# fabian-sp/GGLasso

Measured on AMD Instinct MI355X. Metric: ADMM iters/sec on (K=32,p=500) GGL at 1/2/4/8 GPUs; eigh HBM GB/s vs peak, higher is better.
Workload: dtype f64

## Files before the change

### gglasso_amd/_lib.py

```python
import ctypes
import os

import numpy as np

_HERE = os.path.dirname(os.path.abspath(__file__))
LIB_PATH = os.path.join(_HERE, "lib", "libggl_hip.so")
DEV_LIB_PATH = os.path.join(_HERE, "lib", "libggl_hip_dev.so")

REG_SGL, REG_GGL, REG_FGL = 0, 1, 2
EIG_AUTO, EIG_JACOBI, EIG_ROCSOLVER, EIG_NEWTON_SCHULZ = 0, 1, 2, 3
CTX_STREAM_GIVEN = 1 << 16
OPTIONS = {"speculate": 1, "spec_factor": 2, "ns_mode": 3, "ns_degrees": 4, "theta_flat": 5, "rank_eig": 6, "parts": 7,
           "parts_max_tiles": 8, "symm_variant": 9, "spin_wait": 10, "fused_bounds": 11, "pipeline": 12, "fused_start": 13, "parts_small": 14, "ns_tol": 15, "cw_warm": 16, "chain": 17, "rank_l0_coarse": 18, "isolate": 19, "rank_deflate": 20, "rank_l0_deflate": 21, "fused_cw": 22, "omega_lds": 23, "early_part": 24, "part_priority": 25, "fused_w": 26, "rank_cw": 27, "bound_side": 28, "lds_pinned": 29, "join_flag": 30, "cw_rider": 31, "copy_rider": 32, "reduce_rider": 33, "parts_bias": 34, "parts_order": 35, "download_threads": 36, "group_sched": 37}


def eig_flags(method=EIG_AUTO, ns_mode=0, ns_degrees=0):
    return int(method) | ((int(ns_mode) & 0x3) << 8) | ((int(ns_degrees) & 0xf) << 12)

JACOBI_MAX_P = 128
NS_MIN_P = 8
BUF_S, BUF_OMEGA, BUF_THETA, BUF_L, BUF_X, BUF_GROUPSQ, BUF_NORMS, BUF_OMEGA_PREV = range(8)
E_ARG, E_HIP, E_SOLVER, E_ALLOC, E_COMM = -1, -2, -3, -4, -5
PHASES = ("form_W", "eig_omega", "recon_omega", "theta", "eig_L", "recon_L", "dual", "reduce", "eig_omega2", "bound",
          "allreduce_groupsq", "allreduce_norms")

_dp = ctypes.POINTER(ctypes.c_double)
_vp = ctypes.c_void_p
_i = ctypes.c_int
_d = ctypes.c_double
_ubp = ctypes.POINTER(ctypes.c_ubyte)
_ip = ctypes.POINTER(ctypes.c_int)

_SIGNATURES = {
    "ggl_version": ([], _i),
    "ggl_last_error": ([], ctypes.c_char_p),
    "ggl_device_count": ([], _i),
    "ggl_theta_limits": ([ctypes.POINTER(_i)], _i),
    "ggl_ctx_create": ([_i, _i, _i, _i, _vp, ctypes.POINTER(_vp)], _i),
    "ggl_ctx_destroy": ([_vp], _i),
    "ggl_ctx_sync": ([_vp], _i),
    "ggl_device_ptr": ([_vp, _i], _vp),
    "ggl_ctx_set_option": ([_vp, _i, _d], _i),
    "ggl_ctx_get_option": ([_vp, _i, _dp], _i),
    "ggl_set_S": ([_vp, _dp], _i),
    "ggl_set_state": ([_vp, _dp, _dp, _dp, _dp], _i),
    "ggl_set_state_ex": ([_vp, _dp, _dp, _dp, _dp, ctypes.POINTER(_i)], _i),
# ... 40 lines not shown
    "ggl_ext_batch_step": ([_vp, _d, _dp, _dp, _i, _dp, _dp], _i),
    "ggl_objective": ([_vp, _d, _d, _i, _dp], _i),
    "ggl_kkt_residual": ([_vp, _d, _d, _d, _i, _i, _dp, _dp, _dp], _i),
    "ggl_profile_enable": ([_vp, _i], _i),
    "ggl_profile_read": ([_vp, _dp, ctypes.POINTER(ctypes.c_longlong), _i], _i),
    "ggl_dev_symm": ([_i, _i, _dp, _dp, _dp, _dp, _dp, _dp, _i], _i),
    "ggl_dev_symm_bench": ([_i, _i, _i, _i, _dp], _i),
    "ggl_lds_stats": ([_vp, ctypes.POINTER(ctypes.c_longlong)], _i),
    "ggl_group_stats": ([_vp, ctypes.POINTER(ctypes.c_longlong), _dp], _i),
    "ggl_spectral_bounds": ([_vp, _dp, _dp], _i),
    "ggl_pipeline_stats": ([_vp, ctypes.POINTER(ctypes.c_longlong)], _i),
    "ggl_trace_start": ([_vp, _i], _i),
    "ggl_trace_read": ([_vp, _dp, _i], _i),
    "ggl_dev_omega_lds": ([_i, _i, _dp, _dp, _dp, _dp, _dp, _d, _i, _dp, _dp, _i, _dp], _i),
    "ggl_dev_symm_bounds": ([_i, _i, _dp, _dp, _i, _dp, _dp, _dp, _dp], _i),
    "ggl_snapshot_k": ([_vp, _i], _i),
    "ggl_snapshot_from": ([_vp, _i, _vp, _i], _i),
    "ggl_selection_stats": ([_vp, _dp], _i),
    "ggl_threshold_scan": ([_vp, _dp, _i, _dp, ctypes.POINTER(_i)], _i),
    "ggl_selection_rank": ([_vp, _d, _dp], _i),
    "ggl_finalize_L": ([_vp, _i, ctypes.POINTER(_i)], _i),
    "ggl_failed_instances": ([_vp, ctypes.POINTER(_i)], _i),
    "ggl_failed_reason": ([_vp, _i, _dp], _i),
    "ggl_debug_poison": ([_i], _i),
    "ggl_set_odd_dl": ([_i], _i),
    "ggl_reset_instance": ([_vp, _i], _i),
    "ggl_ctx_create_subset": ([_vp, ctypes.POINTER(_i), _i, ctypes.POINTER(_vp)], _i),
    "ggl_get_snapshot_k": ([_vp, _i, _dp, _dp], _i),
    "ggl_get_snapshot_state_k": ([_vp, _i, _dp, _dp], _i),
    "ggl_dev_ns_schedule": ([_d, _i, _i, ctypes.POINTER(_i), _dp, ctypes.POINTER(_i)], _i),
    "ggl_dev_ns_schedule_tol": ([_d, _i, _d, _i, ctypes.POINTER(_i), _dp, ctypes.POINTER(_i)], _i),
    "ggl_dev_group_partition": ([ctypes.POINTER(_i), _i, _i, _i, ctypes.POINTER(_i)], _i),
    "ggl_dev_ns_units": ([_d, _i, _d], _i),
    "ggl_ns_stats": ([_vp, ctypes.POINTER(ctypes.c_longlong)], _i),
    "ggl_rank_stats": ([_vp, ctypes.POINTER(ctypes.c_longlong)], _i),
    "ggl_deflate_stats": ([_vp, ctypes.POINTER(ctypes.c_longlong)], _i),
    "ggl_finalize_stats": ([_vp, ctypes.POINTER(ctypes.c_longlong)], _i),
    "ggl_eig_info": ([_vp, ctypes.POINTER(_i)], _i),
    "ggl_last_dispatch": ([_vp, ctypes.POINTER(ctypes.c_longlong)], _i),
    "ggl_eigh_batched": ([_i, _i, _dp, _dp, _dp, _i], _i),
    "ggl_phiplus": ([_i, _i, _dp, _dp, _dp, _dp], _i),
    "ggl_prox_rank_norm": ([_i, _i, _dp, _dp, _dp, _dp], _i),
    "ggl_phiplus_matrix": ([_i, _i, _dp, _dp, _dp, _i], _i),
    "ggl_rank_matrix": ([_i, _i, _dp, _dp, _dp, _i], _i),
    "ggl_rank_matrix_ex": ([_i, _i, _dp, _dp, _dp, _i, _d, ctypes.POINTER(ctypes.c_longlong)], _i),
    "ggl_rank_matrix_deflate": ([_i, _i, _dp, _dp, _dp, _i, _d, ctypes.POINTER(ctypes.c_longlong)], _i),
    "ggl_prox_od_1norm": ([_i, _dp, _d, _dp, _dp], _i),
    "ggl_prox_p": ([_i, _i, _dp, _d, _d, _i, _dp], _i),
    "ggl_prox_tv": ([_i, _i, _dp, _d, _dp], _i),
    "ggl_prox_2norm": ([_i, _i, _dp, _d, _dp], _i),
    "ggl_prox_phi": ([_i, _i, _dp, _d, _d, _i, _dp], _i),
}

_DEV_SIGNATURES = {
    "ggl_dev_i8_stages": ([_i], _i),
    "ggl_dev_symm_i8": ([_i, _i, _i, _i, _dp, _dp, _d, _d, _dp, _i, _dp], _i),
    "ggl_dev_omega_i8": ([_i, _i, _dp, _dp, _dp, ctypes.POINTER(_i), _d, _dp, _i, _dp], _i),
    "ggl_dev_mfma_f64_peak": ([_dp], _i),
    "ggl_dev_symm_timeline": ([_i, _i, ctypes.POINTER(ctypes.c_longlong), _i, ctypes.POINTER(_i)], _i),
    "ggl_dev_chain_probe": ([_i, _i, _i, _i, _i, _i, _dp], _i),
    "ggl_dev_coissue_probe": ([_dp], _i),
    "ggl_dev_mfma_lds_probe": ([_dp], _i),
    "ggl_dev_chain_run": ([_i, _i, _i, _i, _dp], _i),
    "ggl_dev_switch_bench": ([_i, _i, _i, _i, _i, _dp], _i),
    "ggl_dev_vendor_bench": ([_i, _i, _i, _i, _dp], _i),
    "ggl_dev_fill_copy_probe": ([_i, _i, _i, _i, _i, ctypes.POINTER(ctypes.c_longlong)], _i),
# ... 79 lines not shown
```

### gglasso_amd/csrc/capi_batch.hip

```cpp
#include "capi_internal.hpp"

static int sgl_fused_finish(ggl_ctx* c, const double* rho, const double* lambda1, double* out_norms);

extern "C" int ggl_sgl_batch_step(ggl_ctx* c, const double* rho, const double* lambda1, int latent, const double* mu1,
                                  double* out_norms)
{
    ARGCHK(c && rho && lambda1 && out_norms, "ctx, rho, lambda1, out_norms");
    ARGCHK(!latent || mu1, "latent needs mu1");
    HIPCHK(hipSetDevice(c->device));
    DROP_PRE(c);
    return sgl_batch_step_impl(c, rho, lambda1, latent, mu1, out_norms);
}

static int sgl_fused_finish(ggl_ctx* c, const double* rho, const double* lambda1, double* out_norms)
{
    const int K = c->K;
    c->sgl_done = false;
    c->sgl_fused_calls += 1;
    c->norms_host = true;
    double* rows = c->norms_h;
    {
        const unsigned long long want = c->seq_wait;
        const volatile unsigned long long* sq = c->seq_h;
        const auto t0 = std::chrono::steady_clock::now();
// ... 443 lines not shown
    HIPCHK(hipSetDevice(c->device));
    DROP_PRE(c);
    const size_t pp = (size_t)c->p * c->p, off = (size_t)k * pp;
    double* ident[] = {c->S + off, c->Om[0] + off, c->Om[1] + off, c->Theta + off};
    double* zero[] = {c->L + off, c->X + off, c->W + off};
    for (double* z : zero) HIPCHK(hipMemsetAsync(z, 0, pp * sizeof(double), c->stream));
    for (double* a : ident) launch_set_identity(c->stream, a, 1, c->p);
    for (double* lam : c->Lam)
        if (lam) launch_set_identity(c->stream, lam + off, 1, c->p);
    if (c->X1) HIPCHK(hipMemsetAsync(c->X1 + off, 0, pp * sizeof(double), c->stream));
    HIPCHK(hipGetLastError());
    c->spec_have = false;
    c->cw_have = false;
    c->cwL_have = false;
    return GGL_OK;
}

extern "C" int ggl_ctx_create_subset(ggl_ctx* src, const int* idx, int m, ggl_ctx** out)
{
    ARGCHK(src && idx && out, "ctx, idx, out");
    ARGCHK(m >= 1 && m <= src->K, "1 <= m <= K");
    for (int i = 0; i < m; ++i) ARGCHK(idx[i] >= 0 && idx[i] < src->K, "instance index");
    HIPCHK(hipSetDevice(src->device));
    { int rc_ = drop_prelaunch(src); if (rc_) return rc_; }
    ggl_ctx* c = nullptr;
    int rc = ggl_ctx_create(src->device, m, src->p, src->flags & ~GGL_CTX_STREAM_GIVEN, nullptr, &c);
    if (rc) return rc;
    c->spec_enable = src->spec_enable; c->spec_factor = src->spec_factor; c->ns_force = src->ns_force;
    c->ns_degrees = src->ns_degrees; c->theta_flat = src->theta_flat; c->rank_eig = src->rank_eig;
    c->rank_ns = c->omega_ns && !c->rank_eig; c->ns_parts = src->ns_parts; c->parts_max_tiles = src->parts_max_tiles;
    c->symm_variant = src->symm_variant; c->spin_wait = src->spin_wait; c->fused_bounds = src->fused_bounds;
    c->pipeline = src->pipeline; c->fused_start = src->fused_start; c->parts_small = src->parts_small; c->download_threads = src->download_threads; c->ns_tol = src->ns_tol;
    c->cw_warm = src->cw_warm; c->rank_l0 = src->rank_l0; c->rank_l0_coarse = src->rank_l0_coarse;
    c->group_sched = src->group_sched;
    c->isolate = src->isolate; c->lds_omega = src->lds_omega; c->lds_waves = src->lds_waves; c->early_part = src->early_part; c->rank_deflate = src->rank_deflate; c->rank_l0_deflate = src->rank_l0_deflate;
    int* didx = nullptr;
    hipError_t e = hipMalloc(&didx, m * sizeof(int));
    if (e == hipSuccess) e = hipMemcpyAsync(didx, idx, m * sizeof(int), hipMemcpyHostToDevice, src->stream);
    if (e != hipSuccess) { ggl_ctx_destroy(c); return fail(GGL_E_HIP, "subset: %s", hipGetErrorString(e)); }
    const size_t pp = (size_t)src->p * src->p;
    const double* from[] = {src->S, src->Om[src->cur], src->Om[src->cur ^ 1], src->Theta, src->L, src->X};
    double* to[] = {c->S, c->Om[0], c->Om[1], c->Theta, c->L, c->X};
    for (int i = 0; i < 6; ++i) launch_copy_instances(src->stream, to[i], from[i], didx, m, pp, false);
    c->cur = 0;
    c->state_symmetric = src->state_symmetric;
    c->S_symmetric = src->S_symmetric;
    c->fused_w = src->fused_w;
#ifdef GGL_DEV
    c->parts_bias = src->parts_bias; c->parts_order = src->parts_order; c->chain_mode = src->chain_mode; c->fused_cw = src->fused_cw;
    c->rank_cw = src->rank_cw; c->bound_side = src->bound_side;
#endif
    c->lds_pinned = src->lds_pinned;
    c->join_flag = src->join_flag;
    c->cw_rider = src->cw_rider;
    c->copy_rider = src->copy_rider;
    c->red_rider = src->red_rider;
    c->step_latent = src->step_latent;
    c->nk_valid = false;
    if (src->l_ns && src->Ckeep && src->Ckeep_beta) {
        e = hipMalloc(&c->Ckeep_alloc, c->n * sizeof(double) + STACK_SLACK);
        if (e != hipSuccess) { (void)hipFree(didx); ggl_ctx_destroy(c); return fail(GGL_E_HIP, "subset: %s", hipGetErrorString(e)); }
        c->Ckeep = c->Ckeep_alloc;
        c->Ckeep_beta = (double*)malloc(m * sizeof(double));
        for (int i = 0; i < m; ++i) c->Ckeep_beta[i] = src->Ckeep_beta[idx[i]];
        launch_copy_instances(src->stream, c->Ckeep, src->Ckeep, didx, m, pp, false);
        c->l_ns = true;
    }
// ... 27 lines not shown
```

### gglasso_amd/csrc/capi_ctx.hip

```cpp
#include "capi_internal.hpp"

static thread_local char g_err[512] = "";

int fail(int code, const char* fmt, ...)
{
    va_list ap;
    va_start(ap, fmt);
    vsnprintf(g_err, sizeof(g_err), fmt, ap);
    va_end(ap);
    return code;
}

void prof_collect(ggl_ctx* c)
{
    if (!c->prof_on) return;
    for (int ph = 0; ph < GGL_NPHASE; ++ph) {
        if (!c->ev_used[ph]) continue;
        float ms = 0.f;
        if (hipEventElapsedTime(&ms, c->ev[ph][0], c->ev[ph][1]) == hipSuccess) {
            c->ph_ms[ph] += ms;
            c->ph_cnt[ph] += 1;
        }
        c->ev_used[ph] = false;
    }
// ... 294 lines not shown
{
    int rcd = drop_prelaunch(c);
    if (rcd) return rcd;
    switch (opt) {
        case GGL_OPT_SPECULATE: c->spec_enable = v != 0.0; break;
        case GGL_OPT_SPEC_FACTOR:
            if (!(v > 0.0)) return fail(GGL_E_ARG, "bad argument: GGL_OPT_SPEC_FACTOR must be positive");
            c->spec_factor = v;
            break;
        case GGL_OPT_NS_MODE:
            if (v != 0.0 && v != 1.0 && v != 2.0) return fail(GGL_E_ARG, "bad argument: GGL_OPT_NS_MODE is 0, 1 or 2");
            c->ns_force = (int)v;
            break;
        case GGL_OPT_NS_DEGREES: c->ns_degrees = v >= 9 ? 9 : (v >= 5 ? 5 : 3); break;
        case GGL_OPT_THETA_FLAT: c->theta_flat = (v == 2.0) ? 2 : (v != 0.0 ? 1 : 0); break;
        case GGL_OPT_RANK_EIG: c->rank_eig = v != 0.0; c->rank_ns = c->omega_ns && !c->rank_eig; break;
        case GGL_OPT_PARTS: c->ns_parts = std::min(std::max((int)v, 1), (int)ggl_ctx::MAX_PARTS); break;
        case GGL_OPT_PARTS_MAX_TILES: c->parts_max_tiles = (long)v; break;
        case GGL_OPT_SYMM_VARIANT:
            if (v >= 0 && !symm_variant_built((int)v))
                return fail(GGL_E_ARG, "bad argument: product-kernel variant not in this build");
            c->symm_variant = (int)v;
            break;
        case GGL_OPT_SPIN_WAIT: c->spin_wait = v != 0.0; break;
        case GGL_OPT_FUSED_BOUNDS: c->fused_bounds = v != 0.0; break;
        case GGL_OPT_PIPELINE: c->pipeline = v != 0.0; break;
        case GGL_OPT_FUSED_START: c->fused_start = v != 0.0; break;
        case GGL_OPT_PARTS_SMALL: c->parts_small = (int)v; break;
        case GGL_OPT_GROUP_SCHED:
            if (v != 0.0 && v != 1.0 && v != 2.0 && v != 3.0 && v != 12.0 && v != 13.0)
                return fail(GGL_E_ARG, "bad argument: GGL_OPT_GROUP_SCHED is 0, 1, 2, 3, 12 or 13");
            c->group_sched = (int)v;
            break;
#ifdef GGL_DEV
        case GGL_OPT_PARTS_BIAS: c->parts_bias = (int)v; break;
        case GGL_OPT_PARTS_ORDER: c->parts_order = (int)v; break;
        case GGL_OPT_CHAIN: c->chain_mode = (v == 2.0) ? 2 : (v != 0.0 ? 1 : 0); break;
        case GGL_OPT_FUSED_CW: c->fused_cw = v != 0.0; break;
        case GGL_OPT_RANK_CW: c->rank_cw = v != 0.0; break;
        case GGL_OPT_BOUND_SIDE: c->bound_side = (int)v; break;
#else
        case GGL_OPT_PARTS_BIAS: case GGL_OPT_PARTS_ORDER: case GGL_OPT_CHAIN: case GGL_OPT_FUSED_CW: case GGL_OPT_RANK_CW:
        case GGL_OPT_BOUND_SIDE: case GGL_OPT_PART_PRIORITY:
            if (v == 0.0) break;
            return fail(GGL_E_ARG, "bad argument: option %d is a measured-and-rejected alternative that only the development "
                        "library (libggl_hip_dev.so, python -m gglasso_amd.build --dev) carries", opt);
#endif
        case GGL_OPT_DOWNLOAD_THREADS: c->download_threads = std::min(std::max((int)v, 1), 64); break;
        case GGL_OPT_CW_WARM: c->cw_warm = v != 0.0; break;
        case GGL_OPT_ISOLATE: c->isolate = v != 0.0; break;
        case GGL_OPT_OMEGA_LDS: c->lds_omega = v != 0.0; c->lds_waves = (v == 4.0 || v == 8.0) ? (int)v : 0; break;
        case GGL_OPT_EARLY_PART: c->early_part = v != 0.0; break;
        case GGL_OPT_FUSED_W: c->fused_w = v != 0.0; break;
        case GGL_OPT_LDS_PINNED: c->lds_pinned = v != 0.0; break;
        case GGL_OPT_JOIN_FLAG: c->join_flag = v != 0.0; break;
        case GGL_OPT_CW_RIDER: c->cw_rider = (int)v; break;
        case GGL_OPT_COPY_RIDER: c->copy_rider = (int)v; break;
        case GGL_OPT_REDUCE_RIDER: c->red_rider = (int)v; break;
#ifdef GGL_DEV
        case GGL_OPT_PART_PRIORITY: {
            if (v != 0.0 && v != 1.0 && v != 2.0) return fail(GGL_E_ARG, "bad argument: GGL_OPT_PART_PRIORITY is 0, 1 or 2");
            if (!c->omega_ns || (int)v == c->part_priority) break;
            int lo = 0, hi = 0;
            HIPCHK(hipSetDevice(c->device));
            HIPCHK(hipDeviceGetStreamPriorityRange(&lo, &hi));
            HIPCHK(hipStreamSynchronize(c->stream));
// ... 25 lines not shown
        default: return fail(GGL_E_ARG, "bad argument: unknown ctx option %d", opt);
    }
    c->spec_have = false;
    c->cw_have = false;
    c->cwL_have = false;
    return GGL_OK;
}

extern "C" int ggl_ctx_set_option(ggl_ctx* c, int opt, double value)
{
    ARGCHK(c, "ctx");
    return set_option(c, opt, value);
}

extern "C" int ggl_ctx_get_option(ggl_ctx* c, int opt, double* value)
{
    ARGCHK(c && value, "ctx, value");
    switch (opt) {
        case GGL_OPT_SPECULATE: *value = c->spec_enable; break;
        case GGL_OPT_SPEC_FACTOR: *value = c->spec_factor; break;
        case GGL_OPT_NS_MODE: *value = c->ns_force; break;
        case GGL_OPT_NS_DEGREES: *value = c->ns_degrees; break;
        case GGL_OPT_THETA_FLAT: *value = c->theta_flat; break;
        case GGL_OPT_RANK_EIG: *value = c->rank_eig; break;
        case GGL_OPT_PARTS: *value = c->ns_parts; break;
        case GGL_OPT_PARTS_MAX_TILES: *value = (double)c->parts_max_tiles; break;
        case GGL_OPT_SYMM_VARIANT: *value = c->symm_variant; break;
        case GGL_OPT_SPIN_WAIT: *value = c->spin_wait; break;
        case GGL_OPT_FUSED_BOUNDS: *value = c->fused_bounds; break;
        case GGL_OPT_PIPELINE: *value = c->pipeline; break;
        case GGL_OPT_FUSED_START: *value = c->fused_start; break;
        case GGL_OPT_PARTS_SMALL: *value = c->parts_small; break;
        case GGL_OPT_GROUP_SCHED: *value = c->group_sched; break;
        case GGL_OPT_PARTS_BIAS: *value = c->parts_bias; break;
        case GGL_OPT_PARTS_ORDER: *value = c->parts_order; break;
        case GGL_OPT_DOWNLOAD_THREADS: *value = c->download_threads; break;
        case GGL_OPT_NS_TOL: *value = c->ns_tol; break;
        case GGL_OPT_CW_WARM: *value = c->cw_warm; break;
        case GGL_OPT_CHAIN: *value = c->chain_mode; break;
        case GGL_OPT_RANK_L0_COARSE: *value = c->rank_l0_coarse; break;
        case GGL_OPT_ISOLATE: *value = c->isolate; break;
        case GGL_OPT_FUSED_CW: *value = c->fused_cw; break;
        case GGL_OPT_OMEGA_LDS: *value = c->lds_omega ? (c->lds_waves ? c->lds_waves : 1) : 0; break;
        case GGL_OPT_EARLY_PART: *value = c->early_part; break;
        case GGL_OPT_FUSED_W: *value = c->fused_w; break;
        case GGL_OPT_RANK_CW: *value = c->rank_cw; break;
        case GGL_OPT_BOUND_SIDE: *value = c->bound_side; break;
        case GGL_OPT_LDS_PINNED: *value = c->lds_pinned; break;
        case GGL_OPT_JOIN_FLAG: *value = c->join_flag; break;
        case GGL_OPT_CW_RIDER: *value = c->cw_rider; break;
        case GGL_OPT_COPY_RIDER: *value = c->copy_rider; break;
        case GGL_OPT_REDUCE_RIDER: *value = c->red_rider; break;
        case GGL_OPT_PART_PRIORITY: *value = c->part_priority; break;
        case GGL_OPT_RANK_DEFLATE: *value = c->rank_deflate; break;
        case GGL_OPT_RANK_L0_DEFLATE: *value = c->rank_l0_deflate; break;
        default: return fail(GGL_E_ARG, "bad argument: unknown ctx option %d", opt);
    }
    return GGL_OK;
}

#ifdef GGL_DEV
static void dev_env_options(ggl_ctx* c)
{
    static const struct { const char* name; int opt; } tab[] = {
        {"GGL_SPECULATE", GGL_OPT_SPECULATE}, {"GGL_SPEC_FACTOR", GGL_OPT_SPEC_FACTOR}, {"GGL_NS_MODE", GGL_OPT_NS_MODE},
        {"GGL_NS_DEGREES", GGL_OPT_NS_DEGREES}, {"GGL_THETA_FLAT", GGL_OPT_THETA_FLAT}, {"GGL_RANK_EIG", GGL_OPT_RANK_EIG},
// ... 339 lines not shown
```

### gglasso_amd/csrc/capi_internal.hpp

```cpp
#pragma once
#include <hip/hip_runtime.h>
#include <rocblas/rocblas.h>
#include <rocsolver/rocsolver.h>

#include <algorithm>
#include <cmath>
#include <cstdarg>
#include <cstdio>
#include <cstring>
#include <numeric>
#include <atomic>
#include <thread>
#include <mutex>
#include <chrono>
#include <vector>

#include "../../include/ggl_hip.h"
#include "kernels.hpp"
#include "ggl_comm.hpp"

using namespace ggl;


#define HIPCHK(expr)                                                                                   \
// ... 74 lines not shown
    bool flags_dirty = false;
    int step_latent = 0;
    int ns_force = 0;
    bool use_syevj = false;
    static constexpr int MAX_PARTS = 4;
    hipStream_t streamx[MAX_PARTS - 1] = {};
    hipEvent_t ev_fork = nullptr, ev_join[MAX_PARTS - 1] = {};
    GGL_DEV_OPT(int, bound_side);
    bool join_flag = true;
    int red_rider = 2;
    long long red_rides = 0;
    RedRider red_pending;
    int copy_rider = 1;
    long long copy_rides = 0;
    std::vector<double> pre0_beta;
    int cw_rider = 1;
    long long cw_rides = 0;
    bool parts_serial = false;
    unsigned long long* join_words = nullptr;
    unsigned long long join_seq = 0;
    hipEvent_t ev_bfork[MAX_PARTS] = {}, ev_bjoin[MAX_PARTS] = {};
    bool pipeline = true, pre_valid = false, pre_spec_pending = false;
    bool last_step_hint = false;
    double* pre_beta = nullptr;
    long long pre_launched = 0, pre_dropped = 0;
    int download_threads = 8;
    GGL_DEV_OPT(int, parts_order);
    GGL_DEV_OPT(int, parts_bias);
    int group_sched = 1;
    long long group_steps = 0;
    long long group_changes = 0;
    int last_groups = 1, last_group_len[MAX_PARTS] = {}, last_group_units[MAX_PARTS] = {};
    double group_units_sum[MAX_PARTS] = {};
    int parts_small = 8;
    bool fused_start = true;
    bool fused_bounds = true;
    bool lds_omega = true;
    int lds_waves = 0;
    double* lds_tab = nullptr;
    int lds_ntab = 0, lds_tab_deg = -1;
    double lds_lnq = 0.0, lds_tab_tol = -1.0;
    long long lds_calls = 0, lds_misses = 0;
    int lds_cool = 0, lds_cool_next = 4;
    bool lds_last = false;
    GGL_DEV_OPT(bool, fused_cw);
    int theta_flat = 2;
    bool state_symmetric = true;
    bool S_symmetric = false;
    bool fused_w = true, wf_ready = false;
    double* wf_beta = nullptr;
    long long wf_written = 0, wf_used = 0;
    bool spec_enable = true, spec_have = false, spec_pending = false;
    double *spec_c = nullptr, *spec_beta = nullptr;
    double *cuse = nullptr, *cuse_h = nullptr;
    double *coef_hh[2] = {nullptr, nullptr}, *cuse_hh[2] = {nullptr, nullptr};
    int plan_par = 0;
    struct EarlyA {
        bool valid = false;
        NsPlan plans[4];
        double* fused[4] = {nullptr, nullptr, nullptr, nullptr};
        double* beta = nullptr;
        int nh = 0, Kh[4] = {}, k0h[4] = {};
        bool grouped = false;
        int var_parts = -1;
    } early;
    bool early_part = true;
// ... 169 lines not shown
```

### gglasso_amd/csrc/capi_omega.hip

```cpp
#include "capi_internal.hpp"

int eig_recon(ggl_ctx* c, double* A, double* out, double* Dv, int map, const double* betaK, int ph_eig,
                     int ph_recon)
{
    c->info_dirty = true;
    if (use_jacobi(c)) {
        if (ph_eig >= 0) PB(c, ph_eig);
        HIPCHK(launch_jacobi(c->stream, A, Dv, nullptr, out, map, betaK, c->info, c->K, c->p));
        if (ph_eig >= 0) PE(c, ph_eig);
        return GGL_OK;
    }
    if (ph_eig >= 0) PB(c, ph_eig);
    {
        int rcb = blas_handle(c, &c->blas);
        if (rcb) return rcb;
    }
    if (c->use_syevj) {
        rocblas_status sj = rocsolver_dsyevj_strided_batched(c->blas, rocblas_esort_none, rocblas_evect_original,
                                                             rocblas_fill_upper, c->p, A, c->p,
                                                             (rocblas_stride)c->p * c->p, 0.0, c->E, 100,
                                                             (rocblas_int*)c->sweeps, Dv, c->p, c->info, c->K);
        if (sj != rocblas_status_success) return fail(GGL_E_SOLVER, "rocsolver_dsyevj_strided_batched: status %d", (int)sj);
        if (ph_eig >= 0) PE(c, ph_eig);
        if (ph_recon >= 0) PB(c, ph_recon);
// ... 175 lines not shown
{
    c->lds_misses += 1;
    c->lds_cool = c->lds_cool_next;
    c->lds_cool_next = std::min(2 * c->lds_cool_next, 64);
    c->lds_last = false;
}

int trace_lane(const ggl_ctx* c, hipStream_t st)
{
    if (st == c->stream) return 0;
    for (int i = 0; i < ggl_ctx::MAX_PARTS - 1; ++i)
        if (st == c->streamx[i]) return i + 1;
    return -1;
}
void trace_mark(ggl_ctx* c, hipStream_t st, int tag)
{
    ggl_ctx::Trace& t = c->trace;
    if (!t.on || t.n >= t.cap) return;
    if (hipEventRecord(t.ev[t.n], st) != hipSuccess) return;
    t.tag[t.n] = tag;
    t.lane[t.n] = trace_lane(c, st);
    t.n += 1;
}
void trace_host(ggl_ctx* c, int tag)
{
    ggl_ctx::Trace& t = c->trace;
    if (!t.on || t.nhost >= t.cap) return;
    t.host_us[t.nhost] = std::chrono::duration<double, std::micro>(std::chrono::steady_clock::now() - t.t0).count();
    t.host_tag[t.nhost] = tag;
    t.nhost += 1;
}
void trace_symm_hook(hipStream_t st, int kind, void* arg) { trace_mark((ggl_ctx*)arg, st, 10 + kind); }

static int omega_groups(const ggl_ctx* c, const double* cb, const double* beta_h, int K, int* Kh, int* k0h, int* gunits)
{
    if (!c->group_sched || K < 2 || c->ns_force == 2 || c->chain_mode || c->comm) return 1;
    {
        const double I = 2.5e-14 * (double)c->p * c->p * c->p, F = 6.5e-6;
        if (c->group_sched < 10 && (double)K * 1e-7 > 0.01 * 7.0 * (F + K * I)) return 1;
    }
    std::vector<int> u(K);
    for (int k = 0; k < K; ++k) {
        double ck = cb[k] * (1.0 + 1e-10);
        if (!(ck > 0.0) || !std::isfinite(ck) || !(beta_h[k] > 0.0)) return 1;
        if (ck < 4.0 * beta_h[k]) ck = 4.0 * beta_h[k];
        u[k] = ns_units_query(std::sqrt(4.0 * beta_h[k] / ck), c->ns_degrees, c->ns_tol);
        if (u[k] < 0) return 1;
    }
    int len[ggl_ctx::MAX_PARTS];
    const bool force = c->group_sched >= 10;
    const int gmax = force ? c->group_sched - 10 : (c->group_sched >= 2 ? c->group_sched : 3);
    const int G = ns_group_partition(u.data(), K, force ? 20000 : c->p, std::min(gmax, (int)ggl_ctx::MAX_PARTS - 1), len);
    if (G <= 1) return 1;
    for (int g = 0, k0 = 0; g < G; ++g) {
        Kh[g] = len[g];
        k0h[g] = k0;
        gunits[g] = 0;
        for (int k = k0; k < k0 + len[g]; ++k) gunits[g] = std::max(gunits[g], u[k]);
        k0 += len[g];
    }
    return G;
}

static void note_groups(ggl_ctx* c, int G, const int* Kh, const NsPlan* plans)
{
    const int G_prev = c->last_groups;
// ... 10 lines not shown
    }
}

int omega_step(ggl_ctx* c, int latent, CopySegs* pending, bool allow_spec, bool only_spec)
{
    int rc;
    const double* beta = c->par;
    const int nxt = c->cur ^ 1;
    c->step_latent = latent;
    if (latent && !c->pre0_beta.empty()) std::fill(c->pre0_beta.begin(), c->pre0_beta.end(), std::nan(""));
    CopySegs first;
    if (pending) first = *pending;
    else if (c->par0_stale) first.add(c->par, c->par_h, 8 * (size_t)c->K * sizeof(double));
    c->par0_stale = false;
    if (c->omega_ns) {
        const int K = c->K;
        const bool want_A = c->early_request;
        c->early_request = false;
        bool w_ready = c->wf_ready && want_A && !latent;
        for (int k = 0; w_ready && k < K; ++k) w_ready = (c->par_h[k] == c->wf_beta[k]);
        c->wf_ready = false;
        bool resume = c->early.valid && allow_spec && !latent && !want_A && c->spec_enable;
        for (int k = 0; resume && k < K; ++k) resume = (c->par_h[k] == c->early.beta[k]);
        c->early.valid = false;
        if (!resume) {
            c->plan_par ^= 1;
            c->coef_h = c->coef_hh[c->plan_par];
            c->cuse_h = c->cuse_hh[c->plan_par];
        }
        double* pre = c->coef_h + (size_t)(NS_MAX_LAUNCHES - 2) * NS_SLOT(K);
        for (int k = 0; !resume && k < K; ++k) {
            double* o0 = pre + (size_t)k * NS_NCOEF;
            double* o1 = pre + NS_SLOT(K) + (size_t)k * NS_NCOEF;
            o0[0] = 4.0 * c->par_h[k]; o0[1] = 1.0; o0[2] = o0[3] = o0[4] = o0[5] = 0.0;
            o1[0] = 0.0; o1[1] = 1.0; o1[2] = o1[3] = o1[4] = o1[5] = 0.0;
        }
        double* pre_d = c->coef + (size_t)(NS_MAX_LAUNCHES - 2) * NS_SLOT(K);
        const long t64 = (c->p + 63) / 64;
        const long ntile = t64 * (t64 + 1) / 2 * K;
        int nh = (K >= 16 && ntile >= 600 && ntile <= c->parts_max_tiles) ? std::min(c->ns_parts, K / 8) : 1;
        if (nh == 1 && c->parts_small && K >= c->parts_small && K < 16 && c->p >= 384 && c->ns_parts >= 2) nh = 2;
        nh = std::max(nh, 1);
        bool spec = allow_spec && c->spec_enable && c->spec_have && !latent && c->spec_cool == 0;
        if (allow_spec && !only_spec && c->spec_cool > 0) c->spec_cool -= 1;
        for (int k = 0; spec && k < K; ++k) spec = (c->par_h[k] == c->spec_beta[k]);
        if (resume) spec = true;
        int Kh[ggl_ctx::MAX_PARTS], k0h[ggl_ctx::MAX_PARTS];
        bool grouped = false;
        int gunits[ggl_ctx::MAX_PARTS] = {};
        if (resume) {
            nh = c->early.nh;
            grouped = c->early.grouped;
            for (int h = 0; h < nh; ++h) { Kh[h] = c->early.Kh[h]; k0h[h] = c->early.k0h[h]; }
        } else {
            for (int h = 0, k0 = 0; h < nh; ++h) {
                Kh[h] = K / nh + (h < K % nh ? 1 : 0);
                if (nh == 2 && c->parts_bias && std::abs(c->parts_bias) < K / 2) Kh[h] += h == 0 ? c->parts_bias : -c->parts_bias;
                k0h[h] = k0;
                k0 += Kh[h];
            }
            if (spec && nh == 1) {
                std::vector<double> cb(K);
                for (int k = 0; k < K; ++k) cb[k] = c->spec_c[k] * c->spec_factor;
                const int G = omega_groups(c, cb.data(), c->par_h, K, Kh, k0h, gunits);
                if (G > 1) { nh = G; grouped = true; }
            }
        }
        const size_t pp = (size_t)c->p * c->p;
// ... 66 lines not shown
                if (as_spec) {
                    c->spec_pending = !fused;
                    c->cw_pending = false;
                    c->dvo_valid = false;
                    c->cur = nxt;
                    return GGL_OK;
                }
                HIPCHK(hipStreamSynchronize(c->stream));
                if (c->spec_flag_h[0] == 0) {
                    sanitize_bounds(c, c->bounds_h, c->par_h, 4.0);
                    for (int k = 0; k < K; ++k) { c->spec_c[k] = c->bounds_h[k]; c->spec_beta[k] = c->par_h[k]; }
                    c->spec_have = true;
                    c->lds_cool_next = 4;
                    c->dvo_valid = false;
                    c->cur = nxt;
                    return GGL_OK;
                }
                c->par0_stale = false;
                lds_missed(c);
                HIPCHK(hipMemsetAsync(c->spec_flag, 0, ggl_ctx::MAX_PARTS * sizeof(int), c->stream));
                for (int h = 0; h < ggl_ctx::MAX_PARTS; ++h) c->spec_flag_h[h] = 0;
            }
        }
#ifdef GGL_DEV
        if (spec && !want_A && !resume && c->chain_mode && c->fused_start && c->fused_bounds && (c->symm_variant < 0 || c->symm_variant == 17) &&
            chain_tile(K, c->p, c->chain_mode == 2) == 64) {
            if (!c->nsNX) HIPCHK(malloc_filled(&c->nsNX, 2 * c->n * sizeof(double) + STACK_SLACK, c->stream));
            if (!c->chain_cnt) HIPCHK(hipMalloc(&c->chain_cnt, (size_t)K * CHAIN_CNT_STRIDE * sizeof(unsigned)));
            for (int k = 0; k < K; ++k) c->cuse_h[k] = c->spec_c[k] * c->spec_factor;
            NsPlan& pl = plans[0];
            SymmOp ops[CHAIN_MAX_OPS];
            int nops = 0;
            const int bT = (c->p + 63) / 64;
            if (ns_plan(c->cuse_h, c->par_h, K, c->coef_h, start_base_h, &pl, c->ns_force, c->ns_degrees, c->ns_tol) == 0 &&
                !pl.stable) {
                double* f0 = nullptr;
                for (int k = 0; k < K; ++k)
                    f0 = ns_fused_start(pl, start_base_h + 5 * (size_t)k, c->nsYP[1], c->nsT, (size_t)K * pp,
                                        pre + NS_SLOT(K) + (size_t)k * NS_NCOEF + 3);
                if (f0)
                    nops = ns_chain_ops(pl, pre_d, pre_d + NS_SLOT(K), c->coef, c->W, c->nsYP[0], c->nsYP[1], c->nsNX, c->nsT,
                                        c->Om[nxt], K, c->p, 0, f0, c->rowpart, c->fropart, ops, CHAIN_MAX_OPS);
            }
            if (nops > 0) {
                CopySegs sg = first;
                sg.add(pre_d, pre, (size_t)K * NS_NCOEF * sizeof(double));
                sg.add(pre_d + NS_SLOT(K), pre + NS_SLOT(K), (size_t)K * NS_NCOEF * sizeof(double));
                sg.add(c->spec_flag, nullptr, 2 * sizeof(int));
                sg.add(c->spec_flag + ggl_ctx::MAX_PARTS - 1, nullptr, sizeof(int));
                c->spec_flag_h[0] = c->spec_flag_h[1] = c->spec_flag_h[ggl_ctx::MAX_PARTS - 1] = 0;
                const int nb_launch = pl.products - 2;
                if (nb_launch > 0) sg.add(c->coef, c->coef_h, (size_t)nb_launch * NS_SLOT(K) * sizeof(double));
                sg.add(c->cuse, c->cuse_h, (size_t)K * sizeof(double));
                if (c->info_dirty) sg.add(c->info, nullptr, K * sizeof(int));
                sg.add(c->chain_cnt, nullptr, (size_t)K * CHAIN_CNT_STRIDE * sizeof(unsigned));
                launch_copy_small(c->stream, sg);
                PB(c, GGL_PH_FORM_W);
                launch_form_W_sym(c->stream, c->W, c->Theta, nullptr, c->X, c->S, beta, K, c->p);
                PE(c, GGL_PH_FORM_W);
                PB(c, GGL_PH_EIG_OMEGA);
                ChainProg P;
                P.nops = nops; P.K = K; P.p = c->p; P.ntiles = bT * (bT + 1) / 2;
                P.begin[0] = 0;
                for (int i = 0; i < nops; ++i) { P.op[i] = ops[i]; P.begin[i + 1] = P.begin[i] + P.ntiles * (ops[i].pair ? 2 : 1); }
                if (launch_omega_chain(c->stream, P, c->chain_cnt, c->spec_flag + 1, c->spec_flag_h + 1) < 0)
                    return fail(GGL_E_HIP, "k_omega_chain: launch failed (%s)", hipGetErrorString(hipGetLastError()));
                launch_bound_rows(c->stream, c->rowpart, bT, K, c->p, c->nbrow, c->infpart);
                launch_cw_final(c->stream, c->nsYP[0] + c->n, c->nbrow, K, c->p, c->infpart, c->fropart, bT * (bT + 1) / 2,
                                c->cwmax, c->cwcnt, c->bounds_h, c->cuse, c->spec_flag, c->spec_flag_h, 0,
                                (c->cw_warm && c->cw_have) ? c->cwvec[c->cw_cur] : nullptr,
                                c->cw_warm ? c->cwvec[c->cw_cur ^ 1] : nullptr);
                PE(c, GGL_PH_EIG_OMEGA);
                HIPCHK(hipGetLastError());
                c->last_parts = 1;
                c->last_variant = 40;
                c->chain_calls += 1;
                c->ns_launches_total += pl.products;
                c->ns_units_frac += pl.units;
                c->ns_steps_frac += pl.steps;
                c->ns_units_total = (long long)(c->ns_units_frac + 0.5);
                c->ns_steps_total = (long long)(c->ns_steps_frac + 0.5);
                c->ns_calls += 1;
                c->spec_calls += 1;
                c->spec_pending = true;
                c->cw_pending = c->cw_warm;
                if (c->info_dirty) { memset(c->info_h, 0, K * sizeof(int)); c->info_dirty = false; }
                c->dvo_valid = false;
                c->cur = nxt;
                return GGL_OK;
            }
        }
#endif
        if (resume) {
            for (int h = 0; h < nh; ++h) { plans[h] = c->early.plans[h]; fused[h] = c->early.fused[h]; }
            c->early_used += 1;
        } else if (spec) {
            for (int k = 0; k < K; ++k) c->cuse_h[k] = c->spec_c[k] * c->spec_factor;
            sanitize_bounds(c, c->cuse_h, c->par_h, 4.0);
            for (int h = 0; spec && h < nh; ++h) {
                const int k0 = k0h[h];
                const int prc = ns_plan(c->cuse_h + k0, c->par_h + k0, Kh[h], c->coef_h + h * region,
                                        start_base_h + 5 * k0, &plans[h], c->ns_force, c->ns_degrees, c->ns_tol);
                spec = (prc == 0) && !plans[h].stable;
                for (int k = k0; spec && c->fused_start && k < k0 + Kh[h]; ++k) {
                    fused[h] = ns_fused_start(plans[h], start_base_h + 5 * (size_t)k, c->nsYP[1] + k0 * pp, c->nsT + k0 * pp,
                                              nh > 1 ? c->n : (size_t)K * pp, pre + NS_SLOT(K) + (size_t)k * NS_NCOEF + 3);
                }
            }
        }
        if (only_spec && !spec) return GGL_NOT_LAUNCHED;
        if (nh > 1 && !c->parts_probed) {
            rc = probe_part_streams(c);
            if (rc) return rc;
        }
        if (nh > 1 && !resume) {
            HIPCHK(hipEventRecord(c->ev_fork, c->stream));
            for (int h = 1; h < nh; ++h) HIPCHK(hipStreamWaitEvent(c->streamx[h - 1], c->ev_fork, 0));
        }
        for (int hh = 0; hh < nh; ++hh) {
            const int h = (c->parts_order && nh == 2 && c->prof_on == 0) ? nh - 1 - hh : hh;
            hipStream_t sh = h == 0 ? c->stream : c->streamx[h - 1];
            const int k0 = k0h[h];
            if (!want_A) {
                c->spec_flag_h[h] = 0;
                if (h == 0 && nh < ggl_ctx::MAX_PARTS) c->spec_flag_h[ggl_ctx::MAX_PARTS - 1] = 0;
            }
            double* Ap = c->nsYP[0] + k0 * pp;
            double* Bp = c->nsYP[0] + c->n + k0 * pp;
            const int btile = c->fused_bounds ? symm_bounds_tile(Kh[h], c->p, var_parts) : 0;
            const int bT = btile ? (c->p + btile - 1) / btile : 0;
            double* rowp = btile ? c->rowpart + (size_t)k0 * bT * c->p : nullptr;
            double* frop = btile ? c->fropart + (size_t)k0 * (bT * (bT + 1) / 2) : nullptr;
            if (!resume) {
            bool ride_copy = (c->copy_rider == 2 || (c->copy_rider == 1 && nh == 1)) && first.n == 0 && !latent && btile != 0 &&
                             !c->chain_mode && c->prof_on != 1;
            for (int k = k0; ride_copy && k < k0 + Kh[h]; ++k) ride_copy = (c->pre0_beta[k] == c->par_h[k]);
            CopySegs sg = first;
            if (!ride_copy) {
                sg.add(pre_d + NS_NCOEF * (size_t)k0, pre + NS_NCOEF * (size_t)k0, (size_t)Kh[h] * NS_NCOEF * sizeof(double));
// ... 11 lines not shown
                sg.add(c->cuse + k0, c->cuse_h + k0, (size_t)Kh[h] * sizeof(double));
                if (h == 0 && c->info_dirty) sg.add(c->info, nullptr, K * sizeof(int));
            }
            if (h == 0 && c->red_pending.nblk > 0) {
                if (w_ready && (c->red_rider == 2 || nh == 1)) {
                    symm_set_reduce_rider(c->red_pending);
                    c->red_rides += 1;
                } else {
                    launch_reduce_partials(sh, c->red_pending.partials, 1, c->red_pending.nblk, c->red_pending.nv, c->red_pending.out,
                                           c->red_pending.seq, c->red_pending.seq_val);
                    trace_mark(c, sh, 21);
                }
                c->red_pending = RedRider{};
            }
            if (ride_copy) {
                symm_set_copy_rider(sg);
                c->copy_rides += 1;
            } else {
                launch_copy_small(sh, sg);
                trace_mark(c, sh, 1);
            }
            if (h == 0) PB(c, GGL_PH_FORM_W);
            if (!w_ready) {
                launch_form_W_sym(sh, c->W + k0 * pp, c->Theta + k0 * pp, latent ? c->L + k0 * pp : nullptr, c->X + k0 * pp,
                                  c->S + k0 * pp, beta + k0, Kh[h], c->p);
                trace_mark(c, sh, 2);
            } else if (h == 0) c->wf_used += 1;
            const bool early_ev = want_A && h == 0 && c->prof_on == 2;
            if (early_ev) {
                c->ev_early_par ^= 1;
                (void)hipEventRecord(c->ev_early[c->ev_early_par][0], c->stream);
            } else if (h == 0 && !want_A) { PE(c, GGL_PH_FORM_W); PB(c, GGL_PH_EIG_OMEGA); }
            ns_prepare(sh, pre_d + NS_NCOEF * (size_t)k0, pre_d + NS_SLOT(K) + NS_NCOEF * (size_t)k0, c->W + k0 * pp, Ap, Bp, Kh[h], c->p,
                       var_parts, spec ? fused[h] : nullptr, rowp, frop);
            symm_flush_rider(sh);
            if (early_ev) {
                (void)hipEventRecord(c->ev_early[c->ev_early_par][1], c->stream);
                c->ev_early_used[c->ev_early_par] = true;
            }
            }
            if (want_A) continue;
            if (resume && h == 0) PB(c, GGL_PH_EIG_OMEGA);
            hipStream_t sb = sh;
            hipEvent_t bfree = nullptr;
            const int side_slot = nh + h - 1;
            const bool side_on = c->bound_side == 1 || (c->bound_side == 2 && nh > 1 && K >= 16);
            if (side_on && spec && btile && !c->fused_cw && side_slot < ggl_ctx::MAX_PARTS - 1 && c->streamx[side_slot]) {
                if (!c->ev_bfork[h]) {
                    HIPCHK(hipEventCreateWithFlags(&c->ev_bfork[h], hipEventDisableTiming));
                    HIPCHK(hipEventCreateWithFlags(&c->ev_bjoin[h], hipEventDisableTiming));
                }
                sb = c->streamx[side_slot];
                HIPCHK(hipEventRecord(c->ev_bfork[h], sh));
                HIPCHK(hipStreamWaitEvent(sb, c->ev_bfork[h], 0));
                bfree = c->ev_bjoin[h];
            }
            const bool ride = c->cw_rider && spec && btile && !c->fused_cw && sb == sh && c->cw_warm && c->cw_have;
            if (ride) {
                CwRider r;
                r.B = Bp; r.rowpart = rowp; r.fropart = frop;
                r.dprev = c->cwvec[c->cw_cur] + (size_t)k0 * c->p;
                r.dnext = c->cwvec[c->cw_cur ^ 1] + (size_t)k0 * c->p;
                r.d_out = c->nbrow + (size_t)k0 * c->p;
                r.cwmax = c->cwmax + k0; r.cnt = c->cwcnt + k0; r.out = c->bounds_h + k0; r.cuse = c->cuse + k0;
                r.flag = c->spec_flag; r.flag_host = c->spec_flag_h; r.flag_slot = h;
                r.T = bT; r.ntile = bT * (bT + 1) / 2; r.p = c->p; r.K = Kh[h]; r.nbx = (c->p + 15) / 16;
                symm_set_rider(r);
// ... 4 lines not shown
                if (c->fused_cw) {
                    launch_bound_cw(sh, Bp, rowp, bT, Kh[h], c->p, c->nbrow + (size_t)k0 * c->p, frop, bT * (bT + 1) / 2,
                                    c->cwmax + k0, c->cwcnt + k0, c->bounds_h + k0, spec ? c->cuse + k0 : nullptr,
                                    spec ? c->spec_flag : nullptr, spec ? c->spec_flag_h : nullptr, h,
                                    (c->cw_warm && c->cw_have) ? c->cwvec[c->cw_cur] + (size_t)k0 * c->p : nullptr,
                                    c->cw_warm ? c->cwvec[c->cw_cur ^ 1] + (size_t)k0 * c->p : nullptr);
                } else {
                const int nib = bound_rows_blocks(c->p);
                launch_bound_rows(sb, rowp, bT, Kh[h], c->p, c->nbrow + (size_t)k0 * c->p, c->infpart + (size_t)k0 * nib);
                trace_mark(c, sb, 3);
                launch_cw_final(sb, Bp, c->nbrow + (size_t)k0 * c->p, Kh[h], c->p, c->infpart + (size_t)k0 * nib, frop,
                                bT * (bT + 1) / 2, c->cwmax + k0, c->cwcnt + k0, c->bounds_h + k0, spec ? c->cuse + k0 : nullptr,
                                spec ? c->spec_flag : nullptr, spec ? c->spec_flag_h : nullptr, h,
                                (c->cw_warm && c->cw_have) ? c->cwvec[c->cw_cur] + (size_t)k0 * c->p : nullptr,
                                c->cw_warm ? c->cwvec[c->cw_cur ^ 1] + (size_t)k0 * c->p : nullptr);
                trace_mark(c, sb, 4);
                }
                cw_written = c->cw_warm;
            } else {
                double* nb2 = c->nbpart + 2 * (size_t)k0 * nbb;
                double* nbc = c->nbpart + 2 * (size_t)K * nbb + (size_t)k0 * nbb;
                launch_norm_bounds(sh, Bp, Kh[h], c->p, nb2, c->nbrow + (size_t)k0 * c->p);
                launch_cw_bounds(sh, Bp, c->nbrow + (size_t)k0 * c->p, Kh[h], c->p, nbc);
                launch_bound_final(sh, nb2, nbc, nbb, Kh[h], c->bounds_h + k0, 0, spec ? c->cuse + k0 : nullptr,
                                   spec ? c->spec_flag + h : nullptr, spec ? c->spec_flag_h + h : nullptr);
            }
            if (bfree) HIPCHK(hipEventRecord(bfree, sb));
            if (spec) {
                ns_run(sh, plans[h], c->coef + h * region, start_base_d + 5 * k0, c->W + k0 * pp, c->nsYP[0] + k0 * pp,
                       c->nsYP[1] + k0 * pp, c->nsT + k0 * pp, c->Om[nxt] + k0 * pp, Kh[h], c->p,
                       var_parts, nh > 1 ? c->n : 0, fused[h] != nullptr, bfree);
                symm_flush_rider(sh);
                c->ns_launches_total += plans[h].products;
                const double frac = (double)Kh[h] / K;
                c->ns_units_frac += frac * plans[h].units;
                c->ns_steps_frac += frac * plans[h].steps;
            }
            if (h == 0 && !spec) PE(c, GGL_PH_EIG_OMEGA);
        }
        HIPCHK(hipGetLastError());
        if (want_A) {
            for (int h = 0; h < nh; ++h) { c->early.plans[h] = plans[h]; c->early.fused[h] = fused[h]; c->early.Kh[h] = Kh[h]; c->early.k0h[h] = k0h[h]; }
            c->early.nh = nh;
            c->early.grouped = grouped;
            c->early.var_parts = var_parts;
            memcpy(c->early.beta, c->par_h, K * sizeof(double));
            c->early.valid = true;
            c->early_launched += 1;
            return GGL_OK;
        }
        if (spec) {
            if (nh > 1 && c->join_flag && !c->parts_serial) {
                c->join_seq += 1;
                for (int h = 1; h < nh; ++h) launch_set_flag(c->streamx[h - 1], c->join_words + h, c->join_seq);
                launch_wait_flags(c->stream, c->join_words + 1, nh - 1, c->join_seq, c->spec_flag, c->spec_flag_h, 0, 200.0);
                HIPCHK(hipGetLastError());
            } else {
                for (int h = 1; h < nh; ++h) {
                    HIPCHK(hipEventRecord(c->ev_join[h - 1], c->streamx[h - 1]));
                    HIPCHK(hipStreamWaitEvent(c->stream, c->ev_join[h - 1], 0));
                }
            }
            PE(c, GGL_PH_EIG_OMEGA);
            c->ns_units_total = (long long)(c->ns_units_frac + 0.5);
            c->ns_steps_total = (long long)(c->ns_steps_frac + 0.5);
            c->ns_calls += 1;
            c->spec_calls += 1;
            note_groups(c, grouped ? nh : 1, Kh, plans);
            c->spec_pending = true;
            c->cw_pending = cw_written;
            if (c->info_dirty) { memset(c->info_h, 0, K * sizeof(int)); c->info_dirty = false; }
            c->dvo_valid = false;
            c->cur = nxt;
            return GGL_OK;
        }
        for (int h = 0; h < nh; ++h) HIPCHK(hipStreamSynchronize(h == 0 ? c->stream : c->streamx[h - 1]));
        sanitize_bounds(c, c->bounds_h, c->par_h, 4.0);
        for (int k = 0; k < K; ++k) { c->spec_c[k] = c->bounds_h[k]; c->spec_beta[k] = c->par_h[k]; }
        c->spec_have = true;
        if (cw_written) { c->cw_cur ^= 1; c->cw_have = true; }
        bool any_stable = false;
        size_t region_b = region;
        int var_b = var_parts;
        if (nh == 1) {
            const int G = omega_groups(c, c->bounds_h, c->par_h, K, Kh, k0h, gunits);
            if (G > 1) {
                nh = G;
                grouped = true;
                region_b = (size_t)(NS_MAX_LAUNCHES - 4) / nh * NS_SLOT(K);
                var_b = var_grouped;
                if (!c->parts_probed) {
                    rc = probe_part_streams(c);
                    if (rc) return rc;
                }
            }
        }
        for (int h = 0; h < nh; ++h) {
            const int k0 = k0h[h];
            const int prc = ns_plan(c->bounds_h + k0, c->par_h + k0, Kh[h], c->coef_h + h * region_b, start_base_h + 5 * k0,
                                    &plans[h], c->ns_force, c->ns_degrees, c->ns_tol);
            if (prc == -1) return fail(GGL_E_SOLVER, "Newton-Schulz Omega-step: non-finite W (diverged iterate?)");
            if (prc == -2) {
                c->ns_eigh_fallbacks += 1;
                rc = eig_recon(c, c->W, c->Om[nxt], c->DvO, MAP_PHIPLUS, beta, -1, GGL_PH_RECON_OMEGA);
                if (rc) return rc;
                c->dvo_valid = true;
                c->cur = nxt;
                return GGL_OK;
            }
            any_stable = any_stable || plans[h].stable;
        }
        if (nh > 1 && any_stable) {
            const int prc = ns_plan(c->bounds_h, c->par_h, K, c->coef_h, start_base_h, &plans[0], c->ns_force, c->ns_degrees, c->ns_tol);
            if (prc != 0) return fail(GGL_E_SOLVER, "Newton-Schulz Omega-step: plan failed (%d)", prc);
        }
        const int nrun = (nh > 1 && !any_stable) ? nh : 1;
        if (nrun == 1) { Kh[0] = K; k0h[0] = 0; }
        c->last_parts = nrun;
        c->last_variant = symm_effective_variant((nrun > 1 && var_b >= 0) ? var_b
                          : (c->symm_variant >= 0 ? c->symm_variant : symm_auto_variant(Kh[0], c->p)), c->p);
        note_groups(c, (grouped && nrun > 1) ? nrun : 1, Kh, plans);
        PB(c, GGL_PH_EIG_OMEGA2);
        for (int h = 0; h < nrun; ++h) {
            const int Kr = Kh[h], k0 = k0h[h];
            hipStream_t sh = h == 0 ? c->stream : c->streamx[h - 1];
            CopySegs up;
            up.add(start_base_d + 5 * (size_t)k0, start_base_h + 5 * (size_t)k0, (size_t)Kr * 5 * sizeof(double));
            const int nb_launch = plans[h].products - 2;
            if (nb_launch > 0)
                up.add(c->coef + h * region_b, c->coef_h + h * region_b, (size_t)nb_launch * NS_SLOT(Kr) * sizeof(double));
            if (h == 0 && c->info_dirty) up.add(c->info, nullptr, K * sizeof(int));
            launch_copy_small(sh, up);
            ns_run(sh, plans[h], c->coef + h * region_b, start_base_d + 5 * k0,
                   c->W + k0 * pp, c->nsYP[0] + k0 * pp, c->nsYP[1] + k0 * pp, c->nsT + k0 * pp, c->Om[nxt] + k0 * pp, Kr,
                   c->p,
                   nrun > 1 ? var_b : c->symm_variant, nrun > 1 ? c->n : 0);
            c->ns_stable_calls += plans[h].stable ? 1 : 0;
            c->ns_launches_total += plans[h].products;
            const double frac = (double)Kr / K;
            c->ns_units_frac += frac * plans[h].units;
            c->ns_steps_frac += frac * plans[h].steps;
        }
        for (int h = 1; h < nrun; ++h) {
            HIPCHK(hipEventRecord(c->ev_join[h - 1], c->streamx[h - 1]));
            HIPCHK(hipStreamWaitEvent(c->stream, c->ev_join[h - 1], 0));
        }
        PE(c, GGL_PH_EIG_OMEGA2);
        HIPCHK(hipGetLastError());
        c->ns_units_total = (long long)(c->ns_units_frac + 0.5);
        c->ns_steps_total = (long long)(c->ns_steps_frac + 0.5);
        c->ns_calls += 1;
        c->dvo_valid = false;
        if (c->info_dirty) { memset(c->info_h, 0, K * sizeof(int)); c->info_dirty = false; }
        c->cur = nxt;
        return GGL_OK;
    }
    if (only_spec) return GGL_NOT_LAUNCHED;
    launch_copy_small(c->stream, first);
    PB(c, GGL_PH_FORM_W);
    launch_form_W(c->stream, c->W, c->Theta, latent ? c->L : nullptr, c->X, c->S, beta, c->K, c->p);
    PE(c, GGL_PH_FORM_W);
    HIPCHK(hipGetLastError());
    rc = eig_recon(c, c->W, c->Om[nxt], c->DvO, MAP_PHIPLUS, beta, GGL_PH_EIG_OMEGA, GGL_PH_RECON_OMEGA);
    if (rc) return rc;
    c->dvo_valid = true;
    c->cur = nxt;
    return GGL_OK;
}

extern "C" int ggl_step_group_partial(ggl_ctx* c, double rho, double lambda1)
{
// ... 336 lines not shown
```

### gglasso_amd/csrc/capi_ops.hip

```cpp
#include "capi_internal.hpp"

static int eig_common(int K, int p, const double* A, const double* beta, double* D, double* Q, double* out, int map,
                      int eig_method)
{
    ARGCHK(K >= 1 && p >= 1 && A, "K, p, A");
    ARGCHK(eig_method != GGL_EIG_JACOBI || jacobi_fits(p), "GGL_EIG_JACOBI needs p <= GGL_JACOBI_MAX_P");
    const bool jac = (eig_method == GGL_EIG_JACOBI) || (eig_method == GGL_EIG_AUTO && jacobi_fits(p));
    const size_t n = (size_t)K * p * p, kp = (size_t)K * p;
    DevBuf dA, dD, dR, dO, dB, dE, dS;
    int* dinfo = nullptr;
    HIPCHK(dA.alloc(n));
    HIPCHK(dD.alloc(kp));
    HIPCHK(dB.alloc(K));
    HIPCHK(hipMalloc(&dinfo, K * sizeof(int)));
    struct InfoFree { int* p; ~InfoFree() { (void)hipFree(p); } } infofree{dinfo};
    UP(dA.p, A, n);
    if (beta) UP(dB.p, beta, K);
    if (out) HIPCHK(dO.alloc(n));
    std::vector<int> info(K);
    if (jac) {
        if (Q) HIPCHK(dR.alloc(n));
        HIPCHK(launch_jacobi(nullptr, dA.p, dD.p, dR.p, dO.p, map, beta ? dB.p : nullptr, dinfo, K, p));
        HIPCHK(hipDeviceSynchronize());
        HIPCHK(hipMemcpy(info.data(), dinfo, K * sizeof(int), hipMemcpyDeviceToHost));
// ... 686 lines not shown
    HIPCHK(dC.alloc(n));
    HIPCHK(dcoef.alloc(coef.size()));
    HIPCHK(dT.alloc((size_t)nb * 5));
    UP(dA.p, h.data(), n);
    UP(dB.p, h.data(), n);
    UP(dcoef.p, coef.data(), coef.size());
    HIPCHK(hipMemset(dT.p, 0, (size_t)nb * 5 * sizeof(double)));
    for (int i = 0; i < 3; ++i) launch_symm(nullptr, dA.p, dB.p, dC.p, nullptr, nullptr, dcoef.p, K, p, 0);
    launch_symm(nullptr, dA.p, dB.p, dC.p, nullptr, nullptr, dcoef.p, K, p, 10, dT.p);
    HIPCHK(hipGetLastError());
    HIPCHK(hipDeviceSynchronize());
    HIPCHK(hipMemcpy(out, dT.p, (size_t)nb * 5 * sizeof(long long), hipMemcpyDeviceToHost));
    *nblocks_out = nb;
    return GGL_OK;
}

#endif

extern "C" int ggl_dev_ns_schedule(double l, int degrees, int max_steps, int* deg_out, double* coef_out, int* units_out)
{
    ARGCHK(deg_out && coef_out && units_out, "output pointers");
    ARGCHK(l > 0.0 && l <= 1.0, "l must be in (0,1]");
    const int n = ns_schedule_query(l, degrees, max_steps, deg_out, coef_out, units_out);
    if (n < 0) return fail(GGL_E_ARG, "no schedule within %d steps", max_steps);
    return n;
}

extern "C" int ggl_dev_group_partition(const int* units, int K, int p, int max_groups, int* len_out)
{
    ARGCHK(units && len_out && K >= 1 && p >= 1 && max_groups >= 1 && max_groups <= 3, "units, len_out, K, p, 1 <= max_groups <= 3");
    return ns_group_partition(units, K, p, max_groups, len_out);
}
extern "C" int ggl_dev_ns_units(double l, int degrees, double tol) { return ns_units_query(l, degrees, tol); }

extern "C" int ggl_dev_ns_schedule_tol(double l, int degrees, double tol, int max_steps, int* deg_out, double* coef_out,
                                       int* units_out)
{
    ARGCHK(deg_out && coef_out && units_out, "output pointers");
    ARGCHK(l > 0.0 && l <= 1.0, "l must be in (0,1]");
    ARGCHK(tol >= 0.0 && tol <= 1e-6, "tol in [0, 1e-6]");
    const int n = ns_schedule_query(l, degrees, max_steps, deg_out, coef_out, units_out, std::max(tol, NS_TOL_EXACT));
    if (n < 0) return fail(GGL_E_ARG, "no schedule within %d steps", max_steps);
    return n;
}

#ifdef GGL_DEV
extern "C" int ggl_dev_coissue_probe(double* out12)
{
    ARGCHK(out12, "out");
    DevBuf d;
    HIPCHK(d.alloc((size_t)512 * 512));
    coissue_probe(nullptr, d.p, out12);
    HIPCHK(hipGetLastError());
    return GGL_OK;
}

extern "C" int ggl_dev_mfma_lds_probe(double* out6)
{
    ARGCHK(out6, "out");
    DevBuf d;
    HIPCHK(d.alloc((size_t)2048 * 256));
    mfma_lds_probe(nullptr, d.p, out6);
    HIPCHK(hipGetLastError());
    return GGL_OK;
}

// ... 221 lines not shown
```

### gglasso_amd/csrc/capi_stats.hip

```cpp
#include "capi_internal.hpp"

extern "C" int ggl_scale_X(ggl_ctx* c, double factor)
{
    ARGCHK(c, "ctx");
    HIPCHK(hipSetDevice(c->device));
    DROP_PRE(c);
    launch_scale(c->stream, c->X, factor, c->n);
    HIPCHK(hipGetLastError());
    return GGL_OK;
}

extern "C" int ggl_profile_enable(ggl_ctx* c, int on)
{
    ARGCHK(c, "ctx");
    HIPCHK(hipSetDevice(c->device));
    if (on && !c->ev[0][0]) {
        for (int ph = 0; ph < GGL_NPHASE; ++ph)
            for (int e = 0; e < 2; ++e) HIPCHK(hipEventCreate(&c->ev[ph][e]));
        for (int q = 0; q < 2; ++q)
            for (int e = 0; e < 2; ++e) HIPCHK(hipEventCreate(&c->ev_early[q][e]));
    }
    c->prof_on = (on == 2) ? 2 : (on != 0 ? 1 : 0);
    return GGL_OK;
}

extern "C" int ggl_ns_stats(ggl_ctx* c, long long out[16])
{
    ARGCHK(c && out, "ctx, out");
    long long lds[4] = {0, 0, 0, 0};
    if (c->lds_calls) { int rc_ = ggl_lds_stats(c, lds); if (rc_) return rc_; }
    out[0] = c->ns_calls;
    out[1] = c->ns_steps_total + (lds[3] + c->K / 2) / c->K;
    out[2] = c->ns_stable_calls;
    out[3] = c->ns_units_total + (lds[2] + c->K / 2) / c->K;
    out[4] = c->ns_launches_total;
    out[5] = c->rank_calls;
    out[6] = c->rank_retries;
    out[7] = c->rank_fallbacks;
    out[8] = c->rank_launches;
    out[9] = c->spec_calls;
    out[10] = c->spec_misses;
    out[11] = c->spin_timeouts;
    out[12] = c->last_parts;
    out[13] = c->last_variant;
    out[14] = c->ns_eigh_fallbacks;
    out[15] = c->pre_dropped;
    return GGL_OK;
}

extern "C" int ggl_group_stats(ggl_ctx* c, long long out[11], double* units_sum)
{
    ARGCHK(c && out, "ctx, out");
    out[10] = c->group_changes;
    out[0] = c->group_steps;
    out[1] = c->last_groups;
    for (int g = 0; g < 4; ++g) {
        out[2 + g] = c->last_groups > 1 ? c->last_group_len[g] : 0;
        out[6 + g] = c->last_groups > 1 ? c->last_group_units[g] : 0;
        if (units_sum) units_sum[g] = c->group_units_sum[g];
    }
    return GGL_OK;
}

extern "C" int ggl_spectral_bounds(ggl_ctx* c, double* c_out, double* beta_out)
{
    ARGCHK(c && c_out && beta_out, "ctx, c_out, beta_out");
    if (!c->omega_ns || !c->spec_have) return 0;
    for (int k = 0; k < c->K; ++k) { c_out[k] = c->spec_c[k]; beta_out[k] = c->spec_beta[k]; }
    return 1;
}

extern "C" int ggl_lds_stats(ggl_ctx* c, long long out[4])
{
    ARGCHK(c && out, "ctx, out");
    out[0] = c->lds_calls;
    out[1] = c->lds_misses;
    out[2] = out[3] = 0;
    if (c->lds_tab) {
        HIPCHK(hipSetDevice(c->device));
        unsigned long long cnt[2] = {0, 0};
        HIPCHK(hipStreamSynchronize(c->stream));
        HIPCHK(hipMemcpy(cnt, c->lds_tab + (size_t)OMEGA_LDS_MAXTAB * OMEGA_LDS_ENT, sizeof(cnt), hipMemcpyDeviceToHost));
// ... 126 lines not shown
```

### gglasso_amd/csrc/gemm_sym.hip

```cpp
#include <algorithm>
#include <initializer_list>
#include <mutex>
#include <unordered_map>
#include <type_traits>

#include "common.hpp"
#include "kernels.hpp"

namespace ggl {

typedef double v4d __attribute__((ext_vector_type(4)));

__device__ __forceinline__ double c2val(double dC, double v, double dE, double e) { return __builtin_fma(dE, e, dC * v); }

template <int BM, int BK, int WM, int WN, bool LM>
struct SymCfg {
    static constexpr int NWR = BM / WM, NWC = BM / WN, NW = NWR * NWC, NT = NW * 64;
    static constexpr int TI = WM / 16, TJ = WN / 16;
    static constexpr int LDS_LD = BM + 16;
    static constexpr int SLAB = BK * LDS_LD;
    static constexpr int CLD = BM + 1;
    static constexpr int LDS_DOUBLES = (!LM || 2 * SLAB > BM * CLD) ? 2 * SLAB : BM * CLD;
    static constexpr int LPT = (BK * BM) / NT;
    static_assert((BK * BM) % NT == 0, "slab must divide evenly over the threads");
    static_assert(NT % BM == 0, "a row of the slab must be covered by whole thread rows");
};

constexpr int sym_nt(int BM, int WM, int WN) { return (BM / WM) * (BM / WN) * 64; }

static constexpr int NXCD = 8;
__host__ __device__ inline int xcd_share(int K) { return (K == 1 || K == 2 || K == 4) ? NXCD / K : 0; }
__host__ __device__ inline int xcd_grid_small(int ntiles, int K)
{
    const int g = xcd_share(K);
    return g ? NXCD * ((ntiles + g - 1) / g) : NXCD * ((ntiles * K + NXCD - 1) / NXCD);
}
__host__ __device__ inline int xcd_grid(int ntiles, int K)
{
    if (K < NXCD) return xcd_grid_small(ntiles, K);
    const int r = K % NXCD;
    return NXCD * (K / NXCD) * ntiles + (r ? xcd_grid_small(ntiles, r) : 0);
}
__device__ __forceinline__ bool decode_block_small(int ntiles, int K, int& k, int& tile, int L)
{
    const int g = xcd_share(K);
    if (g) {
        const int xcd = L % NXCD, slot = L / NXCD;
        k = xcd / g;
        tile = slot * g + xcd % g;
        return tile < ntiles;
    }
    k = L / ntiles;
    tile = L % ntiles;
    return k < K;
}
__device__ __forceinline__ bool decode_block_xcd(int ntiles, int K, int& k, int& tile, int L)
{
    if (K < NXCD) return decode_block_small(ntiles, K, k, tile, L);
    const int nfull = NXCD * (K / NXCD) * ntiles;
    if (L < nfull) {
        const int xcd = L % NXCD, slot = L / NXCD;
        k = (slot / ntiles) * NXCD + xcd;
        tile = slot % ntiles;
        return true;
    }
    const bool ok = decode_block_small(ntiles, K % NXCD, k, tile, L - nfull);
    k += (K / NXCD) * NXCD;
    return ok;
}
__device__ __forceinline__ bool decode_block_xcd(int ntiles, int K, int& k, int& tile)
{
    return decode_block_xcd(ntiles, K, k, tile, (int)blockIdx.x);
}

template <int BM, int BK, int WM, int WN, bool LM, int ABL = 0>
__global__ __launch_bounds__(sym_nt(BM, WM, WN)) void k_symm_tn(
    const double* __restrict__ A, const double* __restrict__ B, double* __restrict__ C, double* __restrict__ C2,
    const double* __restrict__ E, const double* __restrict__ coef, int K, int p, const double* __restrict__ A1,
    const double* __restrict__ B1, double* __restrict__ C1, int K1, double* __restrict__ maxdev)
{
    using Cfg = SymCfg<BM, BK, WM, WN, LM>;
    __shared__ __attribute__((aligned(16))) double smem[Cfg::LDS_DOUBLES];
    double* As = smem;
    double* Bs = smem + Cfg::SLAB;
    const int T = (p + BM - 1) / BM;
    int k, b;
    if (!decode_block_xcd(T * (T + 1) / 2, K + K1, k, b)) return;
    const bool second = k >= K;
    const int kk = second ? k - K : k;
    int I = 0;
    while (b >= T - I) { b -= T - I; ++I; }
    const int J = I + b;
    const int I0 = I * BM, J0 = J * BM;
    const int tid = threadIdx.x, lane = tid & 63, wave = tid >> 6;
    const int wr = (wave / Cfg::NWC) * WM, wc = (wave % Cfg::NWC) * WN;
    const size_t pp = (size_t)p * p;
    const double* Ak = (second ? A1 : A) + (size_t)kk * pp;
    const double* Bk = (second ? B1 : B) + (size_t)kk * pp;

#ifdef GGL_DEV
    long long t_start = 0, t_loop = 0, t_loop_end = 0;
    if (ABL == 3) t_start = clock64();
#endif

    v4d acc[Cfg::TI][Cfg::TJ];
#pragma unroll
    for (int i = 0; i < Cfg::TI; ++i)
#pragma unroll
        for (int j = 0; j < Cfg::TJ; ++j) acc[i][j] = (v4d){0.0, 0.0, 0.0, 0.0};

    constexpr int RSTEP = Cfg::NT / BM;
    constexpr int NST = 1;
// ... 43 lines not shown
                    acc[i][j] = __builtin_amdgcn_mfma_f64_16x16x4f64(af[kk][i], bf[kk][j], acc[i][j], 0, 0, 0);
                }
        }
    };

    const bool dead_wave = (I == J) && (wr >= wc + WN);
#pragma unroll
    for (int s = 0; s < NST; ++s) fetch(s * BK, ra[s], rb[s]);
#ifdef GGL_DEV
    if (ABL == 3) t_loop = clock64();
#endif
    for (int m0 = 0; m0 < p; m0 += NST * BK) {
#pragma unroll
        for (int s = 0; s < NST; ++s) {
            const int ms = m0 + s * BK;
            if (ms < p) {
                if (ABL != 4) stage(ms, ra[s], rb[s]);
                if (ABL != 4 && ABL != 5) __syncthreads();
                fetch(ms + NST * BK, ra[s], rb[s]);
                if (!dead_wave) compute(min(BK / 4, (p - ms + 3) / 4));
                if (ABL != 4 && ABL != 5) __syncthreads();
            }
        }
    }

#ifdef GGL_DEV
    if (ABL == 3) t_loop_end = clock64();
#endif
    const double cI = coef[k * NS_NCOEF + 0], cAcc = coef[k * NS_NCOEF + 1], cE = coef[k * NS_NCOEF + 2];
    const double dI = coef[k * NS_NCOEF + 3], dC = coef[k * NS_NCOEF + 4], dE = coef[k * NS_NCOEF + 5];
    double* Ck = (second ? C1 : C) + (size_t)kk * pp;
    double* C2k = (C2 && !second) ? C2 + (size_t)kk * pp : nullptr;
    const double* Ek = (E && !second) ? E + (size_t)kk * pp : nullptr;
#pragma unroll
    for (int ti = 0; ti < Cfg::TI; ++ti)
#pragma unroll
        for (int tj = 0; tj < Cfg::TJ; ++tj)
#pragma unroll
            for (int r = 0; r < 4; ++r) {
                const int row = wr + ti * 16 + (lane >> 4) + 4 * r;
                const int col = wc + tj * 16 + (lane & 15);
                const int gi = I0 + row, gj = J0 + col;
                double v = cAcc * acc[ti][tj][r];
                const bool in = gi < p && gj < p;
                if (in && (I != J || gi <= gj)) {
                    if (gi == gj) v += cI;
                    const double e0 = Ek ? Ek[(size_t)gi * p + gj] : 0.0;
                    v += cE * e0;
                    Ck[(size_t)gi * p + gj] = v;
                    if (C2k) C2k[(size_t)gi * p + gj] = c2val(dC, v, dE, e0) + (gi == gj ? dI : 0.0);
                    if ((I == J && gi != gj) || (!LM && I != J)) {
                        Ck[(size_t)gj * p + gi] = v;
                        if (C2k) C2k[(size_t)gj * p + gi] = c2val(dC, v, dE, e0);
                    }
                }
                if (LM && I != J) smem[row * Cfg::CLD + col] = v;
            }
    if (maxdev && ABL != 3) {
        double dev = 0.0;
#pragma unroll
        for (int ti = 0; ti < Cfg::TI; ++ti)
#pragma unroll
            for (int tj = 0; tj < Cfg::TJ; ++tj)
#pragma unroll
                for (int r = 0; r < 4; ++r) {
                    const int gi = I0 + wr + ti * 16 + (lane >> 4) + 4 * r;
                    const int gj = J0 + wc + tj * 16 + (lane & 15);
                    if (gi < p && gj < p && (I != J || gi <= gj)) {
                        double v = cAcc * acc[ti][tj][r] + (gi == gj ? cI - 1.0 : 0.0);
                        if (Ek) v += cE * Ek[(size_t)gi * p + gj];
                        dev = fmax(dev, fabs(v));
                    }
                }
        dev = wave_max(dev);
        if (lane == 0 && dev > 0.0)
            atomicMax(reinterpret_cast<unsigned long long*>(maxdev + k), (unsigned long long)__double_as_longlong(dev));
    }
    if (LM && I != J) {
        __syncthreads();
        for (int e = tid; e < BM * BM; e += Cfg::NT) {
            const int a = e / BM, c = e % BM;
            if (J0 + a < p && I0 + c < p) {
                const double v = smem[c * Cfg::CLD + a];
                Ck[(size_t)(J0 + a) * p + I0 + c] = v;
                if (C2k) {
                    const double e0 = (dE != 0.0 && Ek) ? Ek[(size_t)(J0 + a) * p + I0 + c] : 0.0;
                    C2k[(size_t)(J0 + a) * p + I0 + c] = c2val(dC, v, dE, e0);
                }
            }
        }
    }
#ifdef GGL_DEV
    if (ABL == 3 && tid == 0) {
        asm volatile("s_waitcnt vmcnt(0)" ::: "memory");
        long long* tl = reinterpret_cast<long long*>(maxdev) + (size_t)blockIdx.x * 5;
        unsigned xcc = 0;
        asm volatile("s_getreg_b32 %0, hwreg(HW_REG_XCC_ID)" : "=s"(xcc));
        tl[0] = t_start; tl[1] = t_loop; tl[2] = t_loop_end; tl[3] = clock64(); tl[4] = (long long)xcc;
    }
#endif
}

template <int BM, int BK, int WM, int WN, bool LM>
static void launch_cfg(hipStream_t st, const double* A, const double* B, double* C, double* C2, const double* E,
                       const double* coef, int K, int p, const double* A1 = nullptr, const double* B1 = nullptr,
                       double* C1 = nullptr, int K1 = 0, double* maxdev = nullptr)
{
    using Cfg = SymCfg<BM, BK, WM, WN, LM>;
    const int T = (p + BM - 1) / BM;
    hipLaunchKernelGGL((k_symm_tn<BM, BK, WM, WN, LM>), dim3(xcd_grid(T * (T + 1) / 2, K + K1)), dim3(Cfg::NT), 0, st, A,
                       B, C, C2, E, coef, K, p, A1, B1, C1, K1, maxdev);
}

typedef __attribute__((address_space(1))) const void* gptr_t;
typedef __attribute__((address_space(3))) void* lptr_t;

template <int N> __device__ __forceinline__ void wait_vmcnt()
{
    static_assert(N >= 0 && N <= 63, "vmcnt range");
    if constexpr (N == 0) asm volatile("s_waitcnt vmcnt(0)" ::: "memory");
    else if constexpr (N == 2) asm volatile("s_waitcnt vmcnt(2)" ::: "memory");
    else if constexpr (N == 4) asm volatile("s_waitcnt vmcnt(4)" ::: "memory");
    else if constexpr (N == 6) asm volatile("s_waitcnt vmcnt(6)" ::: "memory");
    else if constexpr (N == 8) asm volatile("s_waitcnt vmcnt(8)" ::: "memory");
    else if constexpr (N == 12) asm volatile("s_waitcnt vmcnt(12)" ::: "memory");
    else if constexpr (N == 16) asm volatile("s_waitcnt vmcnt(16)" ::: "memory");
    else if constexpr (N == 24) asm volatile("s_waitcnt vmcnt(24)" ::: "memory");
    else static_assert(N == 0, "add the immediate");
}

template <int AUX> __device__ __forceinline__ double ld_pol(const double* p)
{
    if constexpr (AUX == 0) return *p;
    else return __hip_atomic_load(p, __ATOMIC_RELAXED, __HIP_MEMORY_SCOPE_AGENT);
}

template <int BK, int NSTG, int ABL, int BM, int NW, int AUX = 0>
__device__ __forceinline__ void symm_dl_tile(const double* __restrict__ A, const double* __restrict__ B,
                                             double* __restrict__ C, double* __restrict__ C2,
                                             const double* __restrict__ E, const double* __restrict__ coef, int K,
                                             int p, const double* __restrict__ A1, const double* __restrict__ B1,
                                             double* __restrict__ C1, int K1, double* __restrict__ maxdev,
                                             double* __restrict__ rowpart, double* __restrict__ fropart, int k, int b,
                                             double* smem)
{
    constexpr int NT = NW * 64;
    constexpr int WM = BM / (NW / 2), WN = BM / 2, TI = WM / 16, TJ = WN / 16;
    constexpr int RPI = 128 / BM;
    constexpr int LPR = 64 / RPI;
    constexpr int SLAB = BK * BM;
    constexpr int IPW = BK / (NW * RPI);
    constexpr int RPW = BK / NW;
    static_assert(NW == 4 || NW == 8, "waves per workgroup");
    static_assert(TI >= 1 && TJ >= 1, "wave tile");
    static_assert(BM == 64 || BM == 32, "tile edge");
    static_assert(IPW >= 1, "k-slab too shallow for this tile");
    static_assert(NSTG * 2 * SLAB >= BM * BM, "the mirror tile reuses the slab storage");
    const int T = (p + BM - 1) / BM;
    const int blockTile = b;
    const bool second = k >= K;
    const int kk = second ? k - K : k;
    int I = 0;
    while (b >= T - I) { b -= T - I; ++I; }
    const int J = I + b;
    const int I0 = I * BM, J0 = J * BM;
    const int tid = threadIdx.x, lane = tid & 63;
    const int wave = __builtin_amdgcn_readfirstlane(tid >> 6);
    const int wr = (wave >> 1) * WM, wc = (wave & 1) * WN;
    const size_t pp = (size_t)p * p;
    const double* Ak = (second ? A1 : A) + (size_t)kk * pp;
    const double* Bk = (second ? B1 : B) + (size_t)kk * pp;

    v4d acc[TI][TJ];
// ... 120 lines not shown
            __builtin_amdgcn_s_setprio(0);
#endif
        }
    };
    auto stages = [&](const int s0, auto... bufs) {
        (void)std::initializer_list<int>{((s0 + (int)decltype(bufs)::value < S) ? (slab(s0 + (int)decltype(bufs)::value, bufs), 0) : 0)...};
    };
    static_assert(NSTG == 2 || NSTG == 3 || NSTG == 4 || NSTG == 6, "stage counts with an unrolled slab loop");
    for (int s0 = 0; s0 < S; s0 += NSTG) {
        if constexpr (NSTG == 2) stages(s0, std::integral_constant<int, 0>{}, std::integral_constant<int, 1>{});
        else if constexpr (NSTG == 3) stages(s0, std::integral_constant<int, 0>{}, std::integral_constant<int, 1>{}, std::integral_constant<int, 2>{});
        else if constexpr (NSTG == 4) stages(s0, std::integral_constant<int, 0>{}, std::integral_constant<int, 1>{}, std::integral_constant<int, 2>{}, std::integral_constant<int, 3>{});
        else stages(s0, std::integral_constant<int, 0>{}, std::integral_constant<int, 1>{}, std::integral_constant<int, 2>{}, std::integral_constant<int, 3>{}, std::integral_constant<int, 4>{}, std::integral_constant<int, 5>{});
    }
    __syncthreads();
#if defined(GGL_EXP_SETPRIO) && GGL_EXP_SETPRIO == 2
    __builtin_amdgcn_s_setprio(2);
#endif
    if (ABL == 4) {
        double keepalive = 0.0;
#pragma unroll
        for (int i = 0; i < TI; ++i)
#pragma unroll
            for (int j = 0; j < TJ; ++j) keepalive += acc[i][j][0] + acc[i][j][1] + acc[i][j][2] + acc[i][j][3];
        if (keepalive == 1234.5678) C[0] = keepalive;
        return;
    }

    const double cI = coef[k * NS_NCOEF + 0], cAcc = coef[k * NS_NCOEF + 1], cE = coef[k * NS_NCOEF + 2];
    const double dI = coef[k * NS_NCOEF + 3], dC = coef[k * NS_NCOEF + 4], dE = coef[k * NS_NCOEF + 5];
    double* Ck = (second ? C1 : C) + (size_t)kk * pp;
    double* C2k = (C2 && !second) ? C2 + (size_t)kk * pp : nullptr;
    const double* Ek = (E && !second) ? E + (size_t)kk * pp : nullptr;
    double dev = 0.0;
    const bool wide = (I != J) && ABL != 1;
    if (wide) {
#pragma unroll
        for (int ti = 0; ti < TI; ++ti)
#pragma unroll
            for (int tj = 0; tj < TJ; ++tj)
#pragma unroll
                for (int r = 0; r < 4; ++r) {
                    const int row = wr + ti * 16 + (lane >> 4) + 4 * r;
                    const int col = wc + tj * 16 + (lane & 15);
                    smem[row * BM + (col ^ row)] = cAcc * acc[ti][tj][r];
                }
        __syncthreads();
        auto ld2 = [](const double* q) { return *reinterpret_cast<const double2*>(q); };
        auto lde2 = [&](const double* q) {
            if constexpr (AUX == 0) return *reinterpret_cast<const double2*>(q);
            else { double2 e; e.x = ld_pol<AUX>(q); e.y = ld_pol<AUX>(q + 1); return e; }
        };
        for (int e2 = tid; e2 < BM * BM / 2; e2 += NT) {
            const int row = e2 / (BM / 2), c2 = (e2 % (BM / 2)) * 2;
            const int gi = I0 + row, gj = J0 + c2;
            double2 t = ld2(smem + row * BM + ((c2 ^ row) & ~1));
            if (row & 1) { const double h = t.x; t.x = t.y; t.y = h; }
            if (gi < p && gj + 1 < p) {
                double2 e = {0.0, 0.0};
                if (Ek) e = lde2(Ek + (size_t)gi * p + gj);
                double2 v;
                v.x = t.x + cE * e.x;
                v.y = t.y + cE * e.y;
                dev = fmax(dev, fmax(fabs(v.x), fabs(v.y)));
                *reinterpret_cast<double2*>(Ck + (size_t)gi * p + gj) = v;
                if (C2k) {
                    double2 w;
                    w.x = c2val(dC, v.x, dE, e.x);
                    w.y = c2val(dC, v.y, dE, e.y);
                    *reinterpret_cast<double2*>(C2k + (size_t)gi * p + gj) = w;
                }
                if (rowpart) {
                    if (row & 1) { const double h = v.x; v.x = v.y; v.y = h; }
                    *reinterpret_cast<double2*>(smem + row * BM + ((c2 ^ row) & ~1)) = v;
                }
            } else if (gi < p && gj < p) {
                const double e0 = Ek ? ld_pol<AUX>(Ek + (size_t)gi * p + gj) : 0.0;
                const double v0 = t.x + cE * e0;
                dev = fmax(dev, fabs(v0));
                Ck[(size_t)gi * p + gj] = v0;
                if (C2k) C2k[(size_t)gi * p + gj] = c2val(dC, v0, dE, e0);
                if (rowpart) {
                    double2 v = {v0, 0.0};
                    if (row & 1) { v.x = 0.0; v.y = v0; }
                    *reinterpret_cast<double2*>(smem + row * BM + ((c2 ^ row) & ~1)) = v;
                }
            } else if (rowpart) {
                *reinterpret_cast<double2*>(smem + row * BM + ((c2 ^ row) & ~1)) = double2{0.0, 0.0};
            }
        }
    } else {
    if (REBAL && I == J && rowpart && ABL != 1) {
        for (int e = tid; e < 6 * 256; e += NT) {
            const int blk = e >> 8, br = (blk < 1) ? 1 : (blk < 3 ? 2 : 3), bc = blk - (br == 1 ? 0 : (br == 2 ? 1 : 3));
            const int row = br * 16 + ((e >> 4) & 15), col = bc * 16 + (e & 15);
            smem[row * BM + (col ^ row)] = 0.0;
        }
    }
#pragma unroll
    for (int ti = 0; ti < TI; ++ti)
#pragma unroll
        for (int tj = 0; tj < TJ; ++tj) {
            if (REBAL && ((ti != tj && tj == 0 && nval <= 3) || ((ti | tj) != 0 && nval <= 1))) continue;
#pragma unroll
            for (int r = 0; r < 4; ++r) {
                const int row = rbk[ti] + (lane >> 4) + 4 * r;
                const int col = cbk[tj] + (lane & 15);
                const int gi = I0 + row, gj = J0 + col;
                double v = cAcc * acc[ti][tj][r];
                const bool keep = gi < p && gj < p && (I != J || gi <= gj);
                if (keep) {
                    if (gi == gj) v += cI;
                    const double e0 = Ek ? ld_pol<AUX>(Ek + (size_t)gi * p + gj) : 0.0;
                    v += cE * e0;
                    dev = fmax(dev, fabs(v - (gi == gj ? 1.0 : 0.0)));
                    Ck[(size_t)gi * p + gj] = v;
                    if (C2k) C2k[(size_t)gi * p + gj] = c2val(dC, v, dE, e0) + (gi == gj ? dI : 0.0);
                    if (I == J && gi != gj) {
                        Ck[(size_t)gj * p + gi] = v;
                        if (C2k) C2k[(size_t)gj * p + gi] = c2val(dC, v, dE, e0);
                    }
                }
                if ((I != J || rowpart) && ABL != 1) smem[row * BM + (col ^ row)] = (rowpart && !keep) ? 0.0 : v;
            }
        }
    }
    if (maxdev) {
        dev = wave_max(dev);
        if (lane == 0 && dev > 0.0)
            atomicMax(reinterpret_cast<unsigned long long*>(maxdev + k), (unsigned long long)__double_as_longlong(dev));
    }
    if (((I != J && !wide) || rowpart) && ABL != 1) __syncthreads();
    if (rowpart && ABL != 1 && tid < 2 * BM) {
        const int t = tid & (BM - 1);
        const bool second = tid >= BM;
        const size_t slot_stride = (size_t)p;
        double rs = 0.0, sq = 0.0;
        if (!second) {
#pragma unroll 8
            for (int c = 0; c < BM; ++c) { const double x = smem[t * BM + (c ^ t)]; rs += fabs(x); sq += x * x; }
        }
        if (second || I == J) {
            double cs = 0.0;
#pragma unroll 8
            for (int r = 0; r < BM; ++r) cs += fabs(smem[r * BM + (t ^ r)]);
            if (I == J) {
                if (!second) {
                    const double dg = smem[t * BM];
                    rs = (rs + cs) - fabs(dg);
                    sq = 2.0 * sq - dg * dg;
                }
            } else {
                rs = cs;
            }
        } else {
            sq *= 2.0;
        }
        if (I != J || !second) {
            const int T2 = (p + BM - 1) / BM;
            const int slot = second ? I : J, gi = (second ? J0 : I0) + t;
            if (gi < p) rowpart[((size_t)k * T2 + slot) * slot_stride + gi] = rs;
        }
        if (tid < 64) {
            sq = wave_sum((tid < BM) ? sq : 0.0);
            if (tid == 0) fropart[(size_t)k * (T * (T + 1) / 2) + blockTile] = sq;
        }
    }
    if (wide) {
        auto lde2 = [&](const double* q) {
            if constexpr (AUX == 0) return *reinterpret_cast<const double2*>(q);
            else { double2 e; e.x = ld_pol<AUX>(q); e.y = ld_pol<AUX>(q + 1); return e; }
        };
        for (int e2 = tid; e2 < BM * BM / 2; e2 += NT) {
            const int a = e2 / (BM / 2), c2 = (e2 % (BM / 2)) * 2;
            if (J0 + a < p && I0 + c2 + 1 < p) {
                double2 v;
                v.x = smem[c2 * BM + (a ^ c2)];
                v.y = smem[(c2 + 1) * BM + (a ^ (c2 + 1))];
                double2 e = {0.0, 0.0};
                const bool need_e = Ek && (!rowpart || (C2k && dE != 0.0));
                if (need_e) e = lde2(Ek + (size_t)(J0 + a) * p + I0 + c2);
                if (!rowpart) { v.x += cE * e.x; v.y += cE * e.y; }
                *reinterpret_cast<double2*>(Ck + (size_t)(J0 + a) * p + I0 + c2) = v;
                if (C2k) {
                    double2 w;
                    w.x = c2val(dC, v.x, dE, e.x);
                    w.y = c2val(dC, v.y, dE, e.y);
                    *reinterpret_cast<double2*>(C2k + (size_t)(J0 + a) * p + I0 + c2) = w;
                }
            } else if (J0 + a < p && I0 + c2 < p) {
                double v0 = smem[c2 * BM + (a ^ c2)];
                const bool need_e = Ek && (!rowpart || (C2k && dE != 0.0));
                const double e0 = need_e ? ld_pol<AUX>(Ek + (size_t)(J0 + a) * p + I0 + c2) : 0.0;
                if (!rowpart) v0 += cE * e0;
                Ck[(size_t)(J0 + a) * p + I0 + c2] = v0;
                if (C2k) C2k[(size_t)(J0 + a) * p + I0 + c2] = c2val(dC, v0, dE, e0);
            }
        }
    }
}

__device__ __forceinline__ void cw_rider_body(const CwRider& r, int idx, double* sh)
{
    const int k = idx / r.nbx, bx = idx - k * r.nbx;
    if (k >= r.K) return;
    const int p = r.p;
    const int lane = threadIdx.x & 63, wave = threadIdx.x >> 6;
    double mxd = 0.0;
    for (int j = threadIdx.x; j < p; j += 256) {
        const double* rp = r.rowpart + (size_t)k * r.T * p + j;
        double v = 0.0;
        for (int s2 = 0; s2 < r.T; ++s2) v += rp[(size_t)s2 * p];
        mxd = fmax(mxd, v);
        if (bx == 0 && r.d_out) r.d_out[(size_t)k * p + j] = v;
    }
    mxd = wave_max(mxd);
    if (lane == 0) sh[wave] = mxd;
    __syncthreads();
    const double inf0 = fmax(fmax(sh[0], sh[1]), fmax(sh[2], sh[3]));
    __syncthreads();
    const double scale = 1.0 / inf0;
    const double* dk = r.dprev + (size_t)k * p;
    const int r0 = bx * 16 + wave * 4;
    const double* w = r.B + (size_t)k * p * p;
    double a[4] = {0.0, 0.0, 0.0, 0.0};
    size_t ro[4];
    bool ok[4];
#pragma unroll
    for (int q = 0; q < 4; ++q) {
// ... 79 lines not shown
#pragma unroll
                for (int v = 0; v < 8; ++v)
                    if (v < nv) acc[v] += t[u][v];
            }
        }
    }
#pragma unroll
    for (int v = 0; v < 8; ++v) {
        if (v < nv) {
            const double s = wave_sum(acc[v]);
            if (lane == 0) sh[wid][v] = s;
        }
    }
    __syncthreads();
    if ((int)threadIdx.x <= nv) {
        const double s = (int)threadIdx.x == nv ? (double)r.seq_val
                                                : (sh[0][threadIdx.x] + sh[1][threadIdx.x]) + (sh[2][threadIdx.x] + sh[3][threadIdx.x]);
        __hip_atomic_store(r.out + threadIdx.x, s, __ATOMIC_RELAXED, __HIP_MEMORY_SCOPE_SYSTEM);
        asm volatile("s_waitcnt vmcnt(0)" ::: "memory");
    }
    __syncthreads();
    if (threadIdx.x == 0) __hip_atomic_store(r.seq, r.seq_val, __ATOMIC_RELAXED, __HIP_MEMORY_SCOPE_SYSTEM);
}

__global__ __launch_bounds__(256) void k_cw_rider(const CwRider rider)
{
    __shared__ __attribute__((aligned(16))) double sh[8 + 256];
    cw_rider_body(rider, (int)blockIdx.x, sh);
}

template <int BK, int NSTG, int ABL = 0, int BM = 64, int NW = 4>
__global__ __launch_bounds__(NW * 64) void k_symm_dl(const double* __restrict__ A, const double* __restrict__ B,
                                                 double* __restrict__ C, double* __restrict__ C2,
                                                 const double* __restrict__ E, const double* __restrict__ coef, int K,
                                                 int p, const double* __restrict__ A1, const double* __restrict__ B1,
                                                 double* __restrict__ C1, int K1, double* __restrict__ maxdev,
                                                 double* __restrict__ rowpart, double* __restrict__ fropart, const CwRider rider,
                                                 const CopySegs cps, const RedRider red)
{
    __shared__ __attribute__((aligned(16))) double smem[NSTG * 2 * BK * BM];
    const int T = (p + BM - 1) / BM;
    int bid = (int)blockIdx.x;
    if constexpr (NW == 4) {
        if (red.nblk > 0) {
            if (bid < NXCD) {
                if (bid == 0) red_rider_body(red, smem);
                return;
            }
            bid -= NXCD;
        }
        const int base = xcd_grid(T * (T + 1) / 2, K + K1);
        if (bid >= base) {
            const int idx = bid - base, ncw = rider.K * rider.nbx;
            if (idx < ncw) cw_rider_body(rider, idx, smem);
            else {
                int blk = idx - ncw;
                for (int sgi = 0; sgi < cps.n; ++sgi) {
                    const int nb = (int)((cps.words[sgi] + 1023u) / 1024u);
                    if (blk < nb) {
                        unsigned* d = (unsigned*)cps.dst[sgi];
                        const unsigned* src = (const unsigned*)cps.src[sgi];
                        const unsigned i0 = (unsigned)blk * 1024u + threadIdx.x;
#pragma unroll
                        for (int e = 0; e < 4; ++e) {
                            const unsigned i = i0 + 256u * e;
                            if (i < cps.words[sgi]) d[i] = src ? src[i] : 0u;
                        }
                        break;
                    }
                    blk -= nb;
                }
            }
            return;
        }
    }
    int k, b;
    if (!decode_block_xcd(T * (T + 1) / 2, K + K1, k, b, bid)) return;
    symm_dl_tile<BK, NSTG, ABL, BM, NW>(A, B, C, C2, E, coef, K, p, A1, B1, C1, K1, maxdev, rowpart, fropart, k, b, smem);
}

#ifdef GGL_DEV
template <int SPLIT> __device__ __forceinline__ bool sk_decode(int ntiles, int K, int L, int& k, int& tile, int& part)
{
    auto small = [&](int Ks, int Ls) {
        const int g = xcd_share(Ks);
        if (g) {
            const int xcd = Ls % NXCD, slot = Ls / NXCD;
            k = xcd / g;
            tile = (slot / SPLIT) * g + xcd % g;
            part = slot % SPLIT;
            return tile < ntiles;
        }
        const int u = Ls % (ntiles * SPLIT);
        k = Ls / (ntiles * SPLIT);
        tile = u / SPLIT;
        part = u % SPLIT;
        return k < Ks;
    };
    if (K < NXCD) return small(K, L);
    const int nfull = NXCD * (K / NXCD) * ntiles * SPLIT;
    if (L < nfull) {
        const int xcd = L % NXCD, slot = L / NXCD, u = slot % (ntiles * SPLIT);
        k = (slot / (ntiles * SPLIT)) * NXCD + xcd;
        tile = u / SPLIT;
        part = u % SPLIT;
        return true;
    }
    const bool ok = small(K % NXCD, L - nfull);
    k += (K / NXCD) * NXCD;
    return ok;
}
// ... 292 lines not shown
                    ++s;
                }
                sh_step[i] = (unsigned char)s;
            }
            sh_job[0] = jk; sh_job[1] = js; sh_job[2] = jb;
        }
        __syncthreads();
        const int jk = __builtin_amdgcn_readfirstlane(sh_job[0]);
        const int js = __builtin_amdgcn_readfirstlane(sh_job[1]);
        int jb = __builtin_amdgcn_readfirstlane(sh_job[2]);
        __syncthreads();
#ifdef GGL_DEV
        if (jk == -2 && P.prof && threadIdx.x == 0) {
            long long* o = P.prof + (size_t)blockIdx.x * 8;
            o[0] = t_claim; o[1] = t_idle; o[2] = t_tile; o[3] = n_tile; o[4] = t_first; o[5] = wall_clock64(); o[6] = x; o[7] = clock64() - c_first;
        }
#endif
        if (jk == -2) return;
        if (jk == -1) {
            for (unsigned q = 0; q < backoff; ++q) __builtin_amdgcn_s_sleep(8);
            backoff = min(backoff * 2u, 64u);
#ifdef GGL_DEV
            { const long long t = wall_clock64(); t_idle += t - t_prev; t_prev = t; }
#endif
            continue;
        }
        backoff = 4;
#ifdef GGL_DEV
        { const long long t = wall_clock64(); t_claim += t - t_prev; t_prev = t; }
#endif
        const SymmOp& o = P.op[js];
        int kk = jk;
        if (o.pair && jb >= P.ntiles) { kk = P.K + jk; jb -= P.ntiles; }
        symm_dl_tile<BK, NSTG, 0, BM, 4, AUX>(o.A, o.B, o.C, o.C2, o.E, o.coef, P.K, P.p, o.A1, o.B1, o.C1, o.pair ? P.K : 0,
                                               nullptr, o.rowpart, o.fropart, kk, jb, smem);
        asm volatile("s_waitcnt vmcnt(0)" ::: "memory");
        __syncthreads();
        if (threadIdx.x == 0)
            __hip_atomic_fetch_add(state + (size_t)jk * CHAIN_CNT_STRIDE, 1u, __ATOMIC_RELAXED, __HIP_MEMORY_SCOPE_WORKGROUP);
#ifdef GGL_DEV
        { const long long t = wall_clock64(); t_tile += t - t_prev; t_prev = t; n_tile += 1; }
#endif
    }
}

__global__ __launch_bounds__(64) void k_chain_check(const unsigned* __restrict__ state, int K, unsigned total,
                                                    int* __restrict__ flag, int* __restrict__ flag_h)
{
    bool bad = false;
    for (int k = threadIdx.x; k < K; k += 64) bad = bad || (state[(size_t)k * CHAIN_CNT_STRIDE] != total);
    if (__any(bad) && threadIdx.x == 0) { *flag = 1; *flag_h = 1; }
}

int chain_tile(int K, int p, bool force)
{
    if ((p & 1) != 0 || K < NXCD || K > NXCD * CHAIN_MAX_INST) return 0;
    const long T = (p + 63) / 64;
    return (force || T * (T + 1) / 2 * K >= 1100) ? 64 : 0;
}

int launch_omega_chain(hipStream_t st, const ChainProg& P, unsigned* state, int* flag, int* flag_h, int aux)
{
    static int slots = 0;
    if (!slots) {
        int dev = 0, per_cu = 0;
        hipDeviceProp_t prop;
        if (hipGetDevice(&dev) != hipSuccess || hipGetDeviceProperties(&prop, dev) != hipSuccess) return -1;
// ... 40 lines not shown
        long spins = 0;
        while (__hip_atomic_load(bar, __ATOMIC_RELAXED, __HIP_MEMORY_SCOPE_AGENT) < phase * NXCD) {
            __builtin_amdgcn_s_sleep(1);
            if (++spins > (1L << 22)) {
                __hip_atomic_store(bar + 1, 1u, __ATOMIC_RELAXED, __HIP_MEMORY_SCOPE_AGENT);
                break;
            }
        }
        __builtin_amdgcn_fence(__ATOMIC_ACQUIRE, "agent");
    }
    __syncthreads();
}

template <int BK, int NSTG, int BM>
__global__ __launch_bounds__(256) void k_symm_chain_probe(double* X0, double* X1, const double* coef, int K, int p,
                                                          int nprod, unsigned* bar, unsigned* err, int two_level)
{
    __shared__ __attribute__((aligned(16))) double smem[NSTG * 2 * BK * BM];
    const int T = (p + BM - 1) / BM, ntiles = T * (T + 1) / 2;
    const int total = xcd_grid(ntiles, K);
    unsigned xcd = blockIdx.x % NXCD;
    if (two_level) {
        unsigned xcc;
        asm volatile("s_getreg_b32 %0, hwreg(HW_REG_XCC_ID)" : "=s"(xcc));
        if ((xcc & 0xf) != xcd && threadIdx.x == 0)
            __hip_atomic_store(err, 2u, __ATOMIC_RELAXED, __HIP_MEMORY_SCOPE_AGENT);
    }
    for (int j = 0; j < nprod; ++j) {
        const double* src = (j & 1) ? X1 : X0;
        double* dst = (j & 1) ? X0 : X1;
        for (int L = blockIdx.x; L < total; L += gridDim.x) {
            int k, b;
            if (decode_block_xcd(ntiles, K, k, b, L))
                symm_dl_tile<BK, NSTG, 0, BM, 4>(src, src, dst, nullptr, nullptr, coef, K, p, nullptr, nullptr, nullptr, 0,
                                                 nullptr, nullptr, nullptr, k, b, smem);
            __syncthreads();
        }
        if (j + 1 < nprod) {
            if (two_level) grid_barrier_xcd(bar, (unsigned)(j + 1), gridDim.x / NXCD, xcd);
            else grid_barrier(bar, (unsigned)(j + 1) * gridDim.x, err);
        }
    }
}

int launch_chain_probe(hipStream_t st, double* X0, double* X1, const double* coef, int K, int p, int nprod, int variant,
                       unsigned* bar, unsigned* err, int two_level)
{
    const void* fn = nullptr;
    int BM = 64;
    if (variant == 16) fn = (const void*)k_symm_chain_probe<16, 2, 64>;
    else if (variant == 17) fn = (const void*)k_symm_chain_probe<16, 3, 64>;
    else if (variant == 20) { fn = (const void*)k_symm_chain_probe<32, 2, 32>; BM = 32; }
    else return 0;
    int per_cu = 0, dev = 0;
    hipDeviceProp_t prop;
    if (hipGetDevice(&dev) != hipSuccess || hipGetDeviceProperties(&prop, dev) != hipSuccess) return -1;
    if (hipOccupancyMaxActiveBlocksPerMultiprocessor(&per_cu, fn, 256, 0) != hipSuccess || per_cu < 1) return -1;
    const int T = (p + BM - 1) / BM;
    const int total = xcd_grid(T * (T + 1) / 2, K);
    if (per_cu > 4) per_cu = 4;
    int grid = per_cu * prop.multiProcessorCount;
    if (grid > total) grid = total;
    grid -= grid % NXCD;
    if (grid < NXCD) return -1;
    void* args[] = {&X0, &X1, &coef, &K, &p, &nprod, &bar, &err, &two_level};
    if (hipLaunchCooperativeKernel(fn, dim3(grid), dim3(256), args, 0, st) != hipSuccess) return -1;
    return grid;
}
#endif

static thread_local CwRider g_rider;
static thread_local CopySegs g_copy_rider;
static thread_local RedRider g_red_rider;
void symm_set_reduce_rider(const RedRider& r) { g_red_rider = r; }
void symm_set_rider(const CwRider& r) { g_rider = r; }
void symm_set_copy_rider(const CopySegs& sg) { g_copy_rider = sg; }
void symm_flush_rider(hipStream_t st)
{
    if (g_red_rider.nblk > 0) {
        launch_reduce_partials(st, g_red_rider.partials, 1, g_red_rider.nblk, g_red_rider.nv, g_red_rider.out, g_red_rider.seq,
                               g_red_rider.seq_val);
        g_red_rider = RedRider{};
    }
    if (g_copy_rider.n > 0) {
        launch_copy_small(st, g_copy_rider);
        g_copy_rider = CopySegs{};
    }
    if (g_rider.K <= 0) return;
    hipLaunchKernelGGL(k_cw_rider, dim3(g_rider.K * g_rider.nbx), dim3(256), 0, st, g_rider);
    g_rider = CwRider{};
}

static void launch_dl(hipStream_t st, const double* A, const double* B, double* C, double* C2, const double* E,
                      const double* coef, int K, int p, const double* A1, const double* B1, double* C1, int K1,
                      double* maxdev, int dl_cfg = 0, double* rowpart = nullptr, double* fropart = nullptr)
{
    const bool eight = dl_cfg == 6 || dl_cfg == 7;
    const CwRider rider = (g_rider.K > 0 && !eight) ? g_rider : CwRider{};
    if (rider.K > 0) g_rider = CwRider{};
    const CopySegs cps = (g_copy_rider.n > 0 && !eight) ? g_copy_rider : CopySegs{};
    if (cps.n > 0) g_copy_rider = CopySegs{};
    const RedRider red = (g_red_rider.nblk > 0 && !eight) ? g_red_rider : RedRider{};
    if (red.nblk > 0) g_red_rider = RedRider{};
    int ncopy = red.nblk > 0 ? NXCD : 0;
    for (int i = 0; i < cps.n; ++i) ncopy += (int)((cps.words[i] + 1023u) / 1024u);
    const int nride = rider.K * rider.nbx + ncopy;
#define GGL_DL(...) hipLaunchKernelGGL((k_symm_dl<__VA_ARGS__>), grid, dim3(256), 0, st, A, B, C, C2, E, coef, K, p, A1, B1, C1, K1, maxdev, rowpart, fropart, rider, cps, red)
    if (dl_cfg == 4 || (dl_cfg >= 8 && dl_cfg <= 13) || (dl_cfg >= 18 && dl_cfg <= 21)) {
        const int T32 = (p + 31) / 32;
        const dim3 grid(xcd_grid(T32 * (T32 + 1) / 2, K + K1) + nride);
        if (dl_cfg == 4) GGL_DL(32, 2, 0, 32);
#ifdef GGL_DEV
        else if (dl_cfg == 8) GGL_DL(16, 4, 0, 32);
        else if (dl_cfg == 9) GGL_DL(32, 3, 0, 32);
        else if (dl_cfg == 10) GGL_DL(16, 6, 0, 32);
        else if (dl_cfg == 11) GGL_DL(32, 4, 0, 32);
        else if (dl_cfg == 12) GGL_DL(16, 2, 0, 32);
        else if (dl_cfg == 13) GGL_DL(16, 3, 0, 32);
        else if (dl_cfg == 18) GGL_DL(32, 2, 2, 32);
        else if (dl_cfg == 19) GGL_DL(32, 2, 3, 32);
        else if (dl_cfg == 20) GGL_DL(32, 2, 4, 32);
        else if (dl_cfg == 21) GGL_DL(32, 2, 5, 32);
#endif
        return;
    }
    const int T = (p + 63) / 64;
    const dim3 grid(xcd_grid(T * (T + 1) / 2, K + K1) + nride);
#ifdef GGL_DEV
    if (dl_cfg == 6 || dl_cfg == 7) {
#define GGL_DL8(...) hipLaunchKernelGGL((k_symm_dl<__VA_ARGS__>), grid, dim3(512), 0, st, A, B, C, C2, E, coef, K, p, A1, B1, C1, K1, maxdev, rowpart, fropart, rider, cps, red)
        if (dl_cfg == 6) GGL_DL8(16, 4, 0, 64, 8);
        else GGL_DL8(32, 3, 0, 64, 8);
#undef GGL_DL8
        return;
    }
#endif
    if (dl_cfg == 1) GGL_DL(16, 3);
#ifdef GGL_DEV
    else if (dl_cfg == 2) GGL_DL(16, 4);
    else if (dl_cfg == 3) GGL_DL(32, 2);
    else if (dl_cfg == 5) GGL_DL(16, 2, 1);
    else if (dl_cfg == 14) GGL_DL(16, 3, 2);
    else if (dl_cfg == 15) GGL_DL(16, 3, 3);
    else if (dl_cfg == 16) GGL_DL(16, 3, 4);
    else if (dl_cfg == 17) GGL_DL(16, 3, 5);
    else if (dl_cfg == 22) GGL_DL(8, 4);
    else if (dl_cfg == 23) GGL_DL(8, 6);
#endif
    else GGL_DL(16, 2);
#undef GGL_DL
}

template <int BM, int BK, int WM, int WN>
__global__ __launch_bounds__(sym_nt(BM, WM, WN)) void k_gemm_nt_right(const double* __restrict__ A,
                                                                      const double* __restrict__ T,
                                                                      double* __restrict__ C,
                                                                      const double* __restrict__ scal, int nbatch, int K, int p)
{
    constexpr int NWC = BM / WN, NT = sym_nt(BM, WM, WN), TI = WM / 16, TJ = WN / 16;
    constexpr int LDA = BK + 2;
    constexpr int LDB = BM + 16;
    __shared__ __attribute__((aligned(16))) double smem[BM * LDA + BK * LDB];
    double* As = smem;
// ... 294 lines not shown
    SymmHookAtExit hook{st, 1};
    if (variant < 0) variant = symm_auto_variant(2 * K, p);
    if (variant >= 41 && variant <= 50) variant = 20;
    switch (variant) {
        case 16: case 17: case 18: case 19: case 20: case 22: case 23: case 24: case 25: case 26: case 27: case 28: case 29: case 30: case 31: case 32: case 33: case 34: case 35: case 36: case 37: case 38: case 39:
            if (symm_dl_serves(p)) {
                launch_dl(st, A, B, C, nullptr, nullptr, coef2K, K, p, A1, B1, C1, K, nullptr, variant - 16);
                break;
            }
            if (variant == 20 || variant >= 24) launch_cfg<32, 32, 16, 16, true>(st, A, B, C, nullptr, nullptr, coef2K, K, p, A1, B1, C1, K);
            else launch_cfg<64, 16, 32, 32, true>(st, A, B, C, nullptr, nullptr, coef2K, K, p, A1, B1, C1, K);
            break;
        case 9: launch_cfg<32, 32, 16, 16, true>(st, A, B, C, nullptr, nullptr, coef2K, K, p, A1, B1, C1, K); break;
#ifdef GGL_DEV
        case 1: launch_cfg<64, 32, 32, 32, true>(st, A, B, C, nullptr, nullptr, coef2K, K, p, A1, B1, C1, K); break;
        case 3: launch_cfg<128, 16, 32, 64, false>(st, A, B, C, nullptr, nullptr, coef2K, K, p, A1, B1, C1, K); break;
        case 4: launch_cfg<64, 16, 32, 32, false>(st, A, B, C, nullptr, nullptr, coef2K, K, p, A1, B1, C1, K); break;
        case 8: launch_cfg<32, 16, 16, 16, true>(st, A, B, C, nullptr, nullptr, coef2K, K, p, A1, B1, C1, K); break;
#endif
        default: launch_cfg<64, 16, 32, 32, true>(st, A, B, C, nullptr, nullptr, coef2K, K, p, A1, B1, C1, K); break;
    }
}

int symm_bounds_tile(int K, int p, int variant)
{
    if (variant < 0) variant = symm_auto_variant(K, p);
    if (!symm_dl_serves(p)) return 0;
    if (variant == 20 || (variant >= 24 && variant <= 29) || (variant >= 34 && variant <= 37) || (variant >= 41 && variant <= 50)) return 32;
    if ((variant >= 16 && variant <= 19) || variant == 22 || variant == 23 || (variant >= 30 && variant <= 33) || variant == 38 || variant == 39) return 64;
    return 0;
}

void launch_symm(hipStream_t st, const double* A, const double* B, double* C, double* C2, const double* E,
                 const double* coef, int K, int p, int variant, double* maxdev, double* rowpart, double* fropart)
{
    SymmHookAtExit hook{st, 0};
    if (variant < 0) variant = symm_auto_variant(K, p);
#define GGL_TN(BM, BK, WM, WN, LM) \
    launch_cfg<BM, BK, WM, WN, LM>(st, A, B, C, C2, E, coef, K, p, nullptr, nullptr, nullptr, 0, maxdev)
#ifdef GGL_DEV
    if (variant >= 41 && variant <= 50) {
        if ((p & 1) == 0 && p >= 2) { launch_sk(st, A, B, C, C2, E, coef, K, p, maxdev, rowpart, fropart, variant); return; }
        variant = 9;
    }
#endif
    switch (variant) {
        case 16: case 17: case 18: case 19: case 20: case 21: case 22: case 23: case 24: case 25: case 26: case 27: case 28: case 29: case 30: case 31: case 32: case 33: case 34: case 35: case 36: case 37: case 38: case 39:
            if (symm_dl_serves(p)) {
                launch_dl(st, A, B, C, C2, E, coef, K, p, nullptr, nullptr, nullptr, 0, maxdev, variant - 16, rowpart, fropart);
                break;
            }
            if (variant == 20 || variant >= 24) GGL_TN(32, 32, 16, 16, true);
            else GGL_TN(64, 16, 32, 32, true);
            break;
        case 9: GGL_TN(32, 32, 16, 16, true); break;
#ifdef GGL_DEV
        case 1: GGL_TN(64, 32, 32, 32, true); break;
        case 2: GGL_TN(128, 16, 64, 64, false); break;
        case 3: GGL_TN(128, 16, 32, 64, false); break;
        case 4: GGL_TN(64, 16, 32, 32, false); break;
        case 5: GGL_TN(128, 32, 64, 64, false); break;
        case 8: GGL_TN(32, 16, 16, 16, true); break;
        case 11: GGL_TN(64, 16, 16, 32, true); break;
        case 12: GGL_TN(64, 32, 16, 32, true); break;
        case 13: GGL_TN(64, 16, 32, 16, true); break;
        case 6: case 7: case 10: case 14: case 15: {
            const int T = (p + 63) / 64;
            const dim3 grid(xcd_grid(T * (T + 1) / 2, K));
            double* md = (variant == 10) ? maxdev : nullptr;
#define GGL_ABL(N) hipLaunchKernelGGL((k_symm_tn<64, 16, 32, 32, true, N>), grid, dim3(256), 0, st, A, B, C, C2, E, coef, K, p, nullptr, nullptr, nullptr, 0, md)
            if (variant == 6) GGL_ABL(1); else if (variant == 7) GGL_ABL(2); else if (variant == 10) GGL_ABL(3);
            else if (variant == 14) GGL_ABL(4); else GGL_ABL(5);
#undef GGL_ABL
            break;
        }
#endif
        default: GGL_TN(64, 16, 32, 32, true); break;
    }
#undef GGL_TN
}

}
```

### gglasso_amd/csrc/kernels.hpp

```cpp
#pragma once
#include <hip/hip_runtime.h>
#include <stddef.h>

#define GGL_NNORM 5

namespace ggl {

enum EigMap {
    MAP_PHIPLUS = 0,
    MAP_RANK = 1,
    MAP_IDENT = 2
};

int elementwise_blocks(int p);
void launch_form_W(hipStream_t st, double* W, const double* Theta, const double* L, const double* X,
                   const double* S, const double* betaK, int K, int p);
void launch_theta_sgl(hipStream_t st, double* Theta, double* X, double* C, const double* Omega,
                      const double* OmegaPrev, const double* L, const double* l1K,
                      const double* mask, const double* invrhoK, int latent, double* partials, int K, int p, const int* skip = nullptr,
                      const int* pk = nullptr, size_t mask_stride = 0);
void launch_dual_update(hipStream_t st, double* X, const double* Omega, const double* OmegaPrev,
                        const double* Theta, const double* L, double* partials, int K, int p);
void launch_reduce_partials(hipStream_t st, const double* partials, int K, int nblk, int nv, double* out,
                            unsigned long long* seq = nullptr, unsigned long long seq_val = 0, unsigned* arrive = nullptr);
// ... 122 lines not shown
    int nS1 = 0, nS2 = 0;
    size_t sstride1 = 0, sstride2 = 0;
    int* flag = nullptr;
    int K = 0, p = 0, P = 0;
};
bool launch_symm_i8_op(hipStream_t st, const I8Op& op, int SA, int SB, int dmax);
static constexpr int I8_NSLICES = 59;
static constexpr int I8_MAXPROD = 8;
struct I8Omega {
    int K = 0, p = 0, P = 0;
    size_t sl = 0;
    int8_t* slab = nullptr;
    double *par = nullptr, *par_h = nullptr;
    double *wscale = nullptr, *wscale_h = nullptr;
    int* flag = nullptr;
};
struct I8Cfg { int s_full = 7, s_f2 = 4, s_gf2 = 3, s_ye = 5, d_ye = 4; };
struct I8Bufs { const double* W; double *Ap, *Bp, *Y1, *F, *F2, *Om; };
struct I8Prog {
    struct Prod { I8Op op; int SA, SB, dmax; } prod[I8_MAXPROD];
    int nprod = 0, units = 0, k0 = 0, Kp = 0, S_W = 7;
};
int i8_omega_alloc(I8Omega* w, int K, int p);
void i8_omega_free(I8Omega* w);
int i8_omega_plan(I8Omega* w, const double* cuse_h, const double* beta_h, int k0, int Kp, double tol, int degrees,
                  const I8Cfg& cfg, const I8Bufs& bufs, I8Prog* prog);
bool i8_omega_run(hipStream_t st, I8Omega* w, const I8Prog& prog, const double* W);
hipError_t launch_jacobi(hipStream_t st, const double* A, double* D, double* R, double* out, int map,
                         const double* betaK, int* info, int K, int p);

void launch_recon(hipStream_t st, double* out, const double* R, const double* D, const double* betaK,
                  int map, int K, int p, double* scale_work);

static constexpr int NS_NCOEF = 6;
int symm_variants();
bool symm_variant_built(int v);
bool symm_dl_serves(int p);
void symm_set_odd_dl(bool on);
int symm_effective_variant(int variant, int p);
int symm_auto_variant(int nprod, int p);
void launch_symm(hipStream_t st, const double* A, const double* B, double* C, double* C2, const double* E,
                 const double* coef, int K, int p, int variant, double* maxdev = nullptr, double* rowpart = nullptr,
                 double* fropart = nullptr);
int symm_bounds_tile(int K, int p, int variant);
void symm_release_workspace(hipStream_t st);

struct SymmOp {
    const double *A, *B, *E, *A1, *B1;
    double *C, *C2, *C1;
    const double* coef;
    double *rowpart, *fropart;
    int pair, pad_;
};
static constexpr int CHAIN_MAX_OPS = 16;
struct ChainProg {
    int nops, K, p, ntiles;
    int begin[CHAIN_MAX_OPS + 1];
    SymmOp op[CHAIN_MAX_OPS];
    long long* prof = nullptr;
};
int chain_tile(int K, int p, bool force = false);
static constexpr int CHAIN_CNT_STRIDE = 32;
static constexpr int CHAIN_MAX_INST = 64;
static_assert(CHAIN_MAX_OPS + 1 <= CHAIN_CNT_STRIDE, "one line holds the completion word and the ticket words");
int launch_omega_chain(hipStream_t st, const ChainProg& P, unsigned* state, int* flag, int* flag_h, int aux = 16);

#ifdef GGL_DEV
int launch_chain_probe(hipStream_t st, double* X0, double* X1, const double* coef, int K, int p, int nprod, int variant,
                       unsigned* bar, unsigned* err, int two_level);
#endif
#ifdef GGL_DEV
void coissue_probe(hipStream_t st, double* scratch, double* out);
void mfma_lds_probe(hipStream_t st, double* scratch, double* out);
#endif
double mfma_f64_peak_tflops(hipStream_t st, double* scratch, int blocks, int iters, int nacc);
double mfma_valu_mix_tflops(hipStream_t st, double* scratch, int blocks, int iters, int nv);
void launch_gemm_right(hipStream_t st, const double* A, const double* T, double* C, const double* scal,
                       int nbatch, int K, int p, int variant);


struct CwRider {
// ... 7 lines not shown
    unsigned* cnt = nullptr;
    double* out = nullptr;
    const double* cuse = nullptr;
    int* flag = nullptr;
    int* flag_host = nullptr;
    int flag_slot = 0;
    int T = 0, ntile = 0, p = 0, K = 0;
    int nbx = 0;
};
void symm_set_copy_rider(const CopySegs& sg);
struct RedRider {
    const double* partials = nullptr;
    double* out = nullptr;
    unsigned long long* seq = nullptr;
    unsigned long long seq_val = 0;
    int nblk = 0, nv = 0;
};
void symm_set_reduce_rider(const RedRider& r);
void symm_set_rider(const CwRider& r);
void symm_flush_rider(hipStream_t st);
void symm_set_launch_hook(void (*fn)(hipStream_t, int, void*), void* arg);
void launch_symm_pair(hipStream_t st, const double* A, const double* B, double* C, const double* A1, const double* B1,
                      double* C1, const double* coef2K, int K, int p, int variant);

static constexpr double NS_TOL_EXACT = 4e-16;
static constexpr double NS_TOL_DEFAULT = 2e-12;
static constexpr int NS_MAX_STEPS = 24;
static constexpr int NS_RANK_MAX_STEPS = 40;
static constexpr int NS_MAX_LAUNCHES = 2 * NS_RANK_MAX_STEPS + 1 + 3;
static inline size_t NS_SLOT(int K) { return (size_t)K * 2 * NS_NCOEF; }
static constexpr double NS_SYM_KAPPA_MAX = 300.0;
static constexpr double NS_KAPPA_LIMIT = 1e12;
struct NsPlan {
    int steps = 0; int products = 0; bool stable = false; double kappa = 0.0; int units = 0;
    double check = 5e-5;
    unsigned char deg[NS_RANK_MAX_STEPS] = {};
};
int form_W_tiles(int p);
void launch_form_W_sym(hipStream_t st, double* W, const double* Theta, const double* L, const double* X,
                       const double* S, const double* betaK, int K, int p);
int ns_plan(const double* cbound_h, const double* beta_h, int K, double* coef_h, double* start_h, NsPlan* plan,
            int force_mode, int degrees = 9, double tol = NS_TOL_EXACT);
int ns_schedule_query(double l, int degrees, int max_steps, int* deg, double* coef, int* units, double tol = NS_TOL_EXACT);
int ns_units_query(double l, int degrees, double tol);
int ns_group_partition(const int* units, int K, int p, int max_groups, int* len_out);
void ns_prepare(hipStream_t st, const double* pre0_d, const double* pre1_d, const double* W, double* Ap, double* Bp,
                int K, int p, int variant, double* start2 = nullptr, double* rowpart = nullptr, double* fropart = nullptr);
void ns_run(hipStream_t st, const NsPlan& plan, const double* coef_d, const double* start_d, const double* W,
            double* AB, double* YP, double* Tb, double* out, int K, int p, int variant, size_t pstride = 0,
            bool fused_start = false, hipEvent_t bprime_free = nullptr);
int ns_chain_ops(const NsPlan& plan, const double* pre0_d, const double* pre1_d, const double* coef_d, const double* W,
                 double* AB, double* YP, double* NX, double* Tb, double* out, int K, int p, size_t pstride, double* start2,
                 double* rowpart, double* fropart, SymmOp* ops, int max_ops);
double* ns_fused_start(const NsPlan& plan, const double* start_hk, double* YP, double* Tb, size_t n1, double out3[3]);

int norm_bounds_blocks(int p);
void launch_norm_bounds(hipStream_t st, const double* W, int K, int p, double* part, double* rowsum = nullptr);
void launch_cw_bounds(hipStream_t st, const double* W, const double* rowsum, int K, int p, double* part);
void launch_bound_final(hipStream_t st, const double* part2, const double* cwpart, int nbb, int K, double* out, int mode,
                        const double* cuse = nullptr, int* flag = nullptr, int* flag_host = nullptr);
int bound_rows_blocks(int p);
void launch_bound_rows(hipStream_t st, const double* rowpart, int T, int K, int p, double* d, double* infpart);
void launch_bound_cw(hipStream_t st, const double* B, const double* rowpart, int T, int K, int p, double* d_out,
                     const double* fropart, int ntile, unsigned long long* cwmax, unsigned* cnt, double* out,
                     const double* cuse, int* flag, int* flag_host, int flag_slot, const double* dprev, double* dnext);
void launch_cw_final(hipStream_t st, const double* B, const double* d, int K, int p, const double* infpart,
                     const double* fropart, int ntile, unsigned long long* cwmax, unsigned* cnt, double* out,
                     const double* cuse, int* flag, int* flag_host, int flag_slot, const double* dprev = nullptr,
                     double* dnext = nullptr);
int rank_ns_plan(const double* cnorm_h, const double* mu_h, int K, double l0, double* coef_h, NsPlan* plan,
                 int degrees = 9);
double rank_ns_image(double l0, int degrees, double x);
double rank_trace_tolerance(double l0, int p);
int rank_ns_plan_continue(const double* mu_h, int m, double lp, double* coef_h, NsPlan* plan, int degrees, size_t slot);
void rank_ns_steps(hipStream_t st, const NsPlan& plan, const double* coef_d, const double* C, double* X, double* Xn, double* Tb,
                   double* P2, double* out, double* maxdev, int K, int p, int variant, size_t cs);
void rank_ns_run(hipStream_t st, const NsPlan& plan, const double* coef_d, const double* C, double* Xa, double* Xb,
                 double* Tb, double* P2, double* out, double* maxdev, int K, int p, int variant, size_t cslot = 0,
                 bool t0_ready = false);
void launch_bound_sqrt_inf_fro(hipStream_t st, const double* infpart, int ninf, const double* fropart, int ntile, int K,
                               double* out);
void launch_rank_t0(hipStream_t st, double* P, const double* C, const double* coef_d, int K, int p);

}
```

### gglasso_amd/csrc/newton_schulz.hip

```cpp
#include <cmath>
#include <vector>
#include <unordered_map>

#include <functional>
#include "common.hpp"
#include "kernels.hpp"

namespace ggl {

static constexpr int FT = 32, FTY = 8, FQ = FT / FTY;

template <bool HAS_L>
__global__ __launch_bounds__(256) void k_form_W_sym(double* __restrict__ W, const double* __restrict__ Theta,
                                                    const double* __restrict__ L, const double* __restrict__ X,
                                                    const double* __restrict__ S, const double* __restrict__ betaK,
                                                    int p)
{
    __shared__ double tile[FT][FT + 1];
    const int k = blockIdx.y;
    const int T = (p + FT - 1) / FT;
    int I = 0, b = blockIdx.x;
    while (b >= T - I) { b -= T - I; ++I; }
    const int J = I + b;
    const int I0 = I * FT, J0 = J * FT;
// ... 294 lines not shown
        NsKey q = q0;
        int d = bd;
        bool done = false;
        for (int i = 0; i < NS_RANK_MAX_STEPS; ++i) {
            const NsStep& s = step(q, d);
            best.deg[i] = (unsigned char)d;
            best.st[i] = s;
            best.n = i + 1;
            if (converged(s)) { done = true; break; }
            q = ns_quantise(s.lnew);
            d = best_from(q, i + 1).d;
        }
        if (!done) best.cost = 1 << 30;
        return plans.emplace(q0.key, best).first->second;
    }
};

static const NsSeq& ns_mixed_schedule(double l, int degrees, double tol)
{
    static thread_local NsPlanner planners[3] = {{3, 0}, {5, 0}, {9, 0}};
    NsPlanner& pl = planners[degrees >= 9 ? 2 : (degrees >= 5 ? 1 : 0)];
    pl.set_tol(std::fmin(std::fmax(tol, NS_TOL_EXACT), 1e-6));
    return pl.plan(l);
}

static const NsSeq& ns_sign_schedule(double l, int degrees, double tol = NS_TOL_EXACT)
{
    static thread_local NsPlanner planners[3] = {{3, 1}, {5, 1}, {9, 1}};
    NsPlanner& pl = planners[degrees >= 9 ? 2 : (degrees >= 5 ? 1 : 0)];
    pl.set_tol(std::fmin(std::fmax(tol, NS_TOL_EXACT), 1e-6));
    return pl.plan(l);
}

int ns_schedule_query(double l, int degrees, int max_steps, int* deg, double* coef, int* units, double tol)
{
    if (!(l > 0.0) || !(l <= 1.0)) return -1;
    const NsSeq& sq = (degrees >= 100) ? ns_sign_schedule(l, degrees - 100, tol) : ns_mixed_schedule(l, degrees, tol);
    if (sq.n < 1 || sq.n > max_steps || sq.cost >= (1 << 29)) return -1;
    for (int i = 0; i < sq.n; ++i) {
        deg[i] = sq.deg[i];
        for (int j = 0; j < 5; ++j) coef[6 * i + j] = sq.st[i].t[j];
        coef[6 * i + 5] = sq.st[i].lnew;
    }
    *units = (degrees >= 100) ? sq.cost : 2 + sq.cost;
    return sq.n;
}

int ns_units_query(double l, int degrees, double tol)
{
    if (!(l > 0.0) || !(l <= 1.0) || 1.0 / (l * l) > NS_SYM_KAPPA_MAX) return -1;
    const NsSeq& sq = ns_mixed_schedule(l, degrees, tol);
    if (sq.n < 1 || sq.n > NS_MAX_STEPS || sq.cost >= (1 << 29)) return -1;
    return 2 + sq.cost;
}

int ns_group_partition(const int* units, int K, int p, int max_groups, int* len_out)
{
    len_out[0] = K;
    if (K < 2 || max_groups < 2) return 1;
    int umin = units[0], umax = units[0];
    for (int k = 1; k < K; ++k) { umin = std::min(umin, units[k]); umax = std::max(umax, units[k]); }
    if (umin <= 0 || umin == umax) return 1;
    const double I = 2.5e-14 * (double)p * p * p, F = 6.5e-6;
    if (3.0 * K * K * 4e-9 > 0.02 * umax * (F + K * I)) return 1;
    const int G = std::min(max_groups, 3);
    const double INF = 1e300;
// ... 17 lines not shown
        if (best[(size_t)g * (K + 1) + K] < best[(size_t)gbest * (K + 1) + K]) gbest = g;
    if (gbest == 1 || !(best[(size_t)gbest * (K + 1) + K] <= 0.94 * whole)) return 1;
    int j = K;
    for (int g = gbest; g >= 1; --g) {
        const int i = from[(size_t)g * (K + 1) + j];
        len_out[g - 1] = j - i;
        j = i;
    }
    return gbest;
}

__global__ __launch_bounds__(256) void k_ns_start(double* __restrict__ Y1, double* __restrict__ Z1,
                                                  const double* __restrict__ Ap, const double* __restrict__ Bp,
                                                  const double* __restrict__ W, const double* __restrict__ st, int p,
                                                  int mode)
{
    const int k = blockIdx.y;
    const size_t pp = (size_t)p * p, base = (size_t)k * pp;
    const double y1a = st[k * 5 + 0], y1b = st[k * 5 + 1], z1i = st[k * 5 + 2], z1a = st[k * 5 + 3], h = st[k * 5 + 4];
    size_t i = (size_t)blockIdx.x * 1024 + threadIdx.x;
#pragma unroll
    for (int e = 0; e < 4; ++e, i += 256) {
        if (i < pp) {
            const double a = Ap[base + i], b2 = Bp[base + i];
            const int r = (int)(i / p), c = (int)(i - (size_t)r * p);
            if (mode == 2) {
                Z1[base + i] = __builtin_fma(z1a, a, y1b * b2) + (r == c ? z1i : 0.0);
                continue;
            }
            if (mode == 3) {
                Y1[base + i] = __builtin_fma(y1a, a, y1b * b2) + (r == c ? z1i : 0.0);
                continue;
            }
            const double y = y1a * a + y1b * b2;
            if (mode == 1) {
                Y1[base + i] = 0.5 * W[base + i] + h * y;
            } else {
                Y1[base + i] = y;
                Z1[base + i] = z1a * a + (r == c ? z1i : 0.0);
            }
        }
    }
}

static void launch_ns_start(hipStream_t st, double* Y1, double* Z1, const double* Ap, const double* Bp, const double* W,
                            const double* stt, int K, int p, int mode)
{
    dim3 grid((unsigned)(((size_t)p * p + 1023) / 1024), K);
    hipLaunchKernelGGL(k_ns_start, grid, dim3(256), 0, st, Y1, Z1, Ap, Bp, W, stt, p, mode);
}

int ns_plan(const double* cbound_h, const double* beta_h, int K, double* coef_h, double* start_h, NsPlan* plan,
            int force_mode, int degrees, double tol)
{
    std::vector<double> c(K);
    double kappa = 1.0;
    for (int k = 0; k < K; ++k) {
        c[k] = cbound_h[k] * (1.0 + 1e-10);
        if (!(c[k] > 0.0) || !std::isfinite(c[k]) || !(beta_h[k] > 0.0)) return -1;
        if (c[k] < 4.0 * beta_h[k]) c[k] = 4.0 * beta_h[k];
        kappa = std::fmax(kappa, c[k] / (4.0 * beta_h[k]));
    }
    const bool stable = (force_mode == 2) || (force_mode == 0 && kappa > NS_SYM_KAPPA_MAX);
    if (kappa > NS_KAPPA_LIMIT) return -2;
    const double lmin = 1.0 / std::sqrt(kappa);
    plan->stable = stable;
    plan->kappa = kappa;
    auto put = [&](int g, int k, double cI, double cAcc, double cE, double dI = 0.0, double dC = 0.0, double dE = 0.0) {
        double* o = coef_h + (size_t)g * NS_SLOT(K) + (size_t)k * NS_NCOEF;
        o[0] = cI; o[1] = cAcc; o[2] = cE; o[3] = dI; o[4] = dC; o[5] = dE;
    };
    if (!stable) {
        const NsSeq& sq = ns_mixed_schedule(lmin, degrees, tol);
        if (sq.n < 1 || sq.n > NS_MAX_STEPS || sq.cost >= (1 << 29)) return -2;
        const int n = sq.n;
        plan->steps = n;
        plan->units = 2 + sq.cost;
        int g = 0;
        for (int it = 0; it < n; ++it) plan->deg[it] = sq.deg[it];
        for (int k = 0; k < K; ++k) {
            const double ck = c[k], sc = std::sqrt(ck);
            double* s = start_h + (size_t)k * 5;
            const double* t = sq.st[0].t;
            g = 0;
            if (sq.deg[0] == 3) {
                s[0] = t[0] / ck; s[1] = t[1] / (ck * ck); s[2] = t[0]; s[3] = t[1] / ck; s[4] = 0.5 * sc;
            } else {
                if (sq.deg[0] == 5) {
                    s[0] = 0.0; s[1] = t[2] / (ck * ck); s[2] = t[0]; s[3] = t[1] / ck; s[4] = 0.0;
                } else {
                    s[0] = t[3] / ck; s[1] = t[4] / (ck * ck); s[2] = t[2]; s[3] = 0.0; s[4] = 0.0;
                    put(g++, k, t[0], 1.0 / (ck * ck), t[1] / ck);
                }
                if (n == 1) put(g++, k, 0.0, 0.5 * sc / ck, 0.5);
                else put(g++, k, 0.0, 1.0 / ck, 0.0);
            }
            for (int it = 1; it < n; ++it) {
                t = sq.st[it].t;
                if (sq.deg[it] == 3) {
                    put(g++, k, t[0], t[1], 0.0);
                } else if (sq.deg[it] == 5) {
                    put(g++, k, 0.0, 1.0, 0.0);
                    put(g++, k, t[0], t[2], t[1]);
                } else {
// ... 20 lines not shown
        n = std::max(n, (int)al[k].size());
    }
    plan->steps = n;
    plan->products = 2 + 2 * (n - 1);
    plan->units = (n == 1) ? 2 : 5 * n - 6;
    for (int it = 0; it < n && it < NS_MAX_STEPS; ++it) plan->deg[it] = 3;
    for (int k = 0; k < K; ++k) {
        auto a_of = [&](int it) { return it < (int)al[k].size() ? al[k][it] : 1.0; };
        const double sc = std::sqrt(c[k]);
        double a = a_of(0);
        double* s = start_h + (size_t)k * 5;
        s[0] = 1.5 * a / c[k];
        s[1] = -0.5 * a * a * a / (c[k] * c[k]);
        s[2] = 1.5 * a;
        s[3] = -0.5 * a * a * a / c[k];
        s[4] = 0.5 * sc;
        int g = 0;
        for (int it = 1; it < n; ++it) {
            a = a_of(it);
            put(g++, k, 1.5, -0.5 * a * a, 0.0);
            if (it == n - 1) put(g++, k, 0.0, 0.5 * sc * a, 0.5);
            else {
                double* o = coef_h + (size_t)g * NS_SLOT(K);
                o[k] = a;
                o[K + k] = a;
                ++g;
            }
        }
    }
    return 0;
}

void ns_prepare(hipStream_t st, const double* pre0_d, const double* pre1_d, const double* W, double* Ap, double* Bp, int K,
                int p, int variant, double* start2, double* rowpart, double* fropart)
{
    launch_symm(st, W, W, Ap, nullptr, nullptr, pre0_d, K, p, variant);
    symm_flush_rider(st);
    launch_symm(st, Ap, Ap, Bp, start2, start2 ? Ap : nullptr, pre1_d, K, p, variant, nullptr, rowpart, fropart);
}

double* ns_fused_start(const NsPlan& plan, const double* start_hk, double* YP, double* Tb, size_t n1, double out3[3])
{
    if (plan.stable || plan.deg[0] < 5) return nullptr;
    if (plan.deg[0] == 5) { out3[0] = start_hk[2]; out3[1] = start_hk[1]; out3[2] = start_hk[3]; return YP + n1; }
    out3[0] = start_hk[2]; out3[1] = start_hk[1]; out3[2] = start_hk[0];
    return Tb;
}

void ns_run(hipStream_t st, const NsPlan& plan, const double* coef_d, const double* start_d, const double* W,
            double* AB, double* YP, double* Tb, double* out, int K, int p, int variant, size_t pstride, bool fused_start,
            hipEvent_t bprime_free)
{
    bool bwaited = bprime_free == nullptr;
    const double* bprime = AB + (pstride ? pstride : (size_t)K * p * p);
    auto before_write = [&](const double* o1, const double* o2) {
        if (!bwaited && (o1 == bprime || o2 == bprime)) { (void)hipStreamWaitEvent(st, bprime_free, 0); bwaited = true; }
    };
    struct AtExit { std::function<void()> f; ~AtExit() { f(); } } at_exit{[&]() { before_write(bprime, nullptr); }};
    const size_t cs = NS_SLOT(K), n1 = pstride ? pstride : (size_t)K * p * p;
    const int n = plan.steps;
    int g = 0;
    double *cur = YP, *nxt = AB;
    if (plan.deg[0] >= 5 && !plan.stable) {
        if (plan.deg[0] == 5) {
            if (!fused_start)
                launch_ns_start(st, nullptr, YP + n1, AB, AB + n1, W, start_d, K, p, 2);
        } else {
            if (!fused_start)
                launch_ns_start(st, Tb, nullptr, AB, AB + n1, W, start_d, K, p, 3);
            launch_symm(st, Tb, AB + n1, YP + n1, nullptr, AB, coef_d + cs * g++, K, p, variant);
        }
        if (n == 1) {
            launch_symm(st, AB, YP + n1, out, nullptr, W, coef_d + cs * g++, K, p, variant);
            return;
        }
        launch_symm(st, AB, YP + n1, YP, nullptr, nullptr, coef_d + cs * g++, K, p, variant);
    } else {
        if (n == 1) {
            launch_ns_start(st, out, nullptr, AB, AB + n1, W, start_d, K, p, 1);
            return;
        }
        launch_ns_start(st, YP, YP + n1, AB, AB + n1, W, start_d, K, p, 0);
    }
    for (int it = 1; it < n; ++it) {
        if (plan.deg[it] == 5 && !plan.stable) {
            launch_symm(st, cur + n1, cur, nxt, nullptr, nullptr, coef_d + cs * g++, K, p, variant);
            launch_symm(st, nxt, nxt, Tb, nullptr, nxt, coef_d + cs * g++, K, p, variant);
        } else if (plan.deg[it] == 9 && !plan.stable) {
            launch_symm(st, cur + n1, cur, out, nullptr, nullptr, coef_d + cs * g++, K, p, variant);
            before_write(nxt, nxt + n1);
            launch_symm(st, out, out, nxt, nxt + n1, out, coef_d + cs * g++, K, p, variant);
            launch_symm(st, nxt, nxt + n1, Tb, nullptr, out, coef_d + cs * g++, K, p, variant);
        } else {
            launch_symm(st, cur + n1, cur, Tb, nullptr, nullptr, coef_d + cs * g++, K, p, variant);
        }
        if (it == n - 1) {
            launch_symm(st, cur, Tb, out, nullptr, W, coef_d + cs * g++, K, p, variant);
        } else if (plan.stable) {
            before_write(nxt + n1, nullptr);
            launch_gemm_right(st, cur, Tb, nxt, coef_d + cs * g++, 2 * K, K, p, 0);
            std::swap(cur, nxt);
        } else {
            before_write(nxt, nxt + n1);
            launch_symm_pair(st, cur, Tb, nxt, Tb, cur + n1, nxt + n1, coef_d + cs * g++, K, p, variant);
            std::swap(cur, nxt);
        }
    }
}

#ifdef GGL_DEV
int ns_chain_ops(const NsPlan& plan, const double* pre0_d, const double* pre1_d, const double* coef_d, const double* W,
                 double* AB, double* YP, double* NX, double* Tb, double* out, int K, int p, size_t pstride, double* start2,
                 double* rowpart, double* fropart, SymmOp* ops, int max_ops)
{
    if (plan.stable || plan.deg[0] < 5 || !start2) return 0;
    const size_t cs = NS_SLOT(K), n1 = pstride ? pstride : (size_t)K * p * p;
    const int n = plan.steps;
    int no = 0, g = 0;
    bool ok = true;
    auto add = [&](const double* A, const double* B, double* C, double* C2, const double* E, const double* coef,
                   double* rp = nullptr, double* fp = nullptr) -> SymmOp* {
        if (no >= max_ops) { ok = false; return nullptr; }
        SymmOp& o = ops[no++];
        o = SymmOp{};
        o.A = A; o.B = B; o.C = C; o.C2 = C2; o.E = E; o.coef = coef; o.rowpart = rp; o.fropart = fp;
        return &o;
    };
    double* Ap = AB;
    double* Bp = AB + n1;
    add(W, W, Ap, nullptr, nullptr, pre0_d);
    add(Ap, Ap, Bp, start2, Ap, pre1_d, rowpart, fropart);
    double *cur = YP, *nxt = NX;
    if (plan.deg[0] == 9) add(Tb, Bp, YP + n1, nullptr, Ap, coef_d + cs * g++);
    if (n == 1) {
        add(Ap, YP + n1, out, nullptr, W, coef_d + cs * g++);
        return ok ? no : 0;
    }
    add(Ap, YP + n1, YP, nullptr, nullptr, coef_d + cs * g++);
    for (int it = 1; it < n; ++it) {
        if (plan.deg[it] == 5) {
            add(cur + n1, cur, nxt, nullptr, nullptr, coef_d + cs * g++);
            add(nxt, nxt, Tb, nullptr, nxt, coef_d + cs * g++);
        } else if (plan.deg[it] == 9) {
            add(cur + n1, cur, out, nullptr, nullptr, coef_d + cs * g++);
            add(out, out, nxt, nxt + n1, out, coef_d + cs * g++);
            add(nxt, nxt + n1, Tb, nullptr, out, coef_d + cs * g++);
        } else {
            add(cur + n1, cur, Tb, nullptr, nullptr, coef_d + cs * g++);
        }
        if (it == n - 1) {
            add(cur, Tb, out, nullptr, W, coef_d + cs * g++);
        } else {
            SymmOp* o = add(cur, Tb, nxt, nullptr, nullptr, coef_d + cs * g++);
            if (o) { o->A1 = Tb; o->B1 = cur + n1; o->C1 = nxt + n1; o->pair = 1; }
            std::swap(cur, nxt);
        }
    }
    return ok ? no : 0;
}
#endif

__global__ __launch_bounds__(256) void k_norm_bounds(const double* __restrict__ W, int p, double* __restrict__ part,
// ... 535 lines not shown
```

### gglasso_amd/solver.py

```python
import math
import time
import warnings

import numpy as np

from . import _lib
from ._lib import as_c, check, ptr

_REG = {"SGL": _lib.REG_SGL, "GGL": _lib.REG_GGL, "FGL": _lib.REG_FGL}


ENGINE_OPTIONS = {}


RANK_REL_TOL = 1e-9


def latent_rank(L, rel_tol=0.0):
    a = np.abs(np.linalg.eigvalsh(L))
    return int(np.count_nonzero(a > a.max() * max(rel_tol, L.shape[0] * np.finfo(np.float64).eps)))


def _host_period(A, K=None, p=None):
    if K is not None:
# ... 357 lines not shown
                raise RuntimeError(f"ggl_ext_admm_step: unexpected return code {rc} (speculative step rejected twice)")
            check(rc)
        return self._norms

    def ext_kkt(self, rho, lambda1K, lambda2, latent, mu1):
        out = np.zeros(1)
        check(self.lib.ggl_ext_kkt_residual(self.h, rho, ptr(lambda1K), lambda2, int(latent), ptr(mu1), ptr(out)))
        return float(out[0])

    def state(self):
        shape = (self.K, self.p, self.p)
        Om, Th, L, X = (np.empty(shape) for _ in range(4))
        check(self.lib.ggl_get_state(self.h, ptr(Om), ptr(Th), ptr(L), ptr(X)))
        return {'Omega': Om, 'Theta': Th, 'L': L, 'X': X}

    def profile(self, on=1):
        check(self.lib.ggl_profile_enable(self.h, int(on)))

    def profile_read(self, reset=True):
        import ctypes
        ms = np.zeros(len(_lib.PHASES))
        cnt = (ctypes.c_longlong * len(_lib.PHASES))()
        check(self.lib.ggl_profile_read(self.h, ptr(ms), cnt, int(reset)))
        return {name: (float(ms[i]), int(cnt[i])) for i, name in enumerate(_lib.PHASES)}

    def ns_stats(self):
        import ctypes
        out = (ctypes.c_longlong * 16)()
        check(self.lib.ggl_ns_stats(self.h, out))
        return dict(zip(("calls", "steps", "stable_calls", "units", "launches", "rank_calls", "rank_retries",
                         "rank_fallbacks", "rank_launches", "spec_calls", "spec_misses", "spin_timeouts", "last_parts",
                         "last_variant", "eigh_fallbacks", "pre_dropped"), (int(v) for v in out)))

    def rank_stats(self):
        import ctypes
        out = (ctypes.c_longlong * 4)()
        check(self.lib.ggl_rank_stats(self.h, out))
        st = dict(zip(("calls", "continued_calls", "continued_instances", "eigh_fallbacks"), (int(v) for v in out)))
        d = (ctypes.c_longlong * 2)()
        check(self.lib.ggl_deflate_stats(self.h, d))
        st["deflated_calls"], st["deflated_instances"] = int(d[0]), int(d[1])
        return st

    def group_stats(self):
        import ctypes
        out = (ctypes.c_longlong * 11)()
        us = np.zeros(4)
        check(self.lib.ggl_group_stats(self.h, out, ptr(us)))
        g = int(out[1])
        return {'steps': int(out[0]), 'groups': g, 'changes': int(out[10]), 'len': [int(out[2 + i]) for i in range(g)] if g > 1 else [],
                'units': [int(out[6 + i]) for i in range(g)] if g > 1 else [], 'units_sum': us.tolist()}

    def spectral_bounds(self):
        cb, be = np.zeros(self.K), np.zeros(self.K)
        if check(self.lib.ggl_spectral_bounds(self.h, ptr(cb), ptr(be))) == 0:
            return None
        return cb, be

    def lds_stats(self):
        import ctypes
        out = (ctypes.c_longlong * 4)()
        check(self.lib.ggl_lds_stats(self.h, out))
        return dict(zip(("calls", "misses", "products", "steps"), (int(v) for v in out)))

    def pipeline_stats(self):
        import ctypes
# ... 347 lines not shown
```

### include/ggl_hip.h

```cpp
#ifndef GGL_HIP_H
#define GGL_HIP_H

#ifdef __cplusplus
extern "C" {
#endif

#define GGL_VERSION 300

#define GGL_OK 0
#define GGL_E_ARG (-1)
#define GGL_E_HIP (-2)
#define GGL_E_SOLVER (-3)
#define GGL_E_ALLOC (-4)
#define GGL_E_COMM (-5)

#define GGL_REG_SGL 0
#define GGL_REG_GGL 1
#define GGL_REG_FGL 2

#define GGL_EIG_AUTO 0
#define GGL_EIG_JACOBI 1
#define GGL_EIG_ROCSOLVER 2
#define GGL_EIG_NEWTON_SCHULZ 3
#define GGL_JACOBI_MAX_P 128
// ... 26 lines not shown
#define GGL_OPT_SPEC_FACTOR 2
#define GGL_OPT_NS_MODE 3
#define GGL_OPT_NS_DEGREES 4
#define GGL_OPT_THETA_FLAT 5
#define GGL_OPT_RANK_EIG 6
#define GGL_OPT_PARTS 7
#define GGL_OPT_PARTS_MAX_TILES 8
#define GGL_OPT_SYMM_VARIANT 9
#define GGL_OPT_SPIN_WAIT 10
#define GGL_OPT_FUSED_BOUNDS 11
#define GGL_OPT_PIPELINE 12
#define GGL_OPT_FUSED_START 13
#define GGL_OPT_PARTS_SMALL 14
#define GGL_OPT_NS_TOL 15
#define GGL_OPT_CW_WARM 16
#define GGL_OPT_CHAIN 17
#define GGL_OPT_RANK_DEFLATE 20
#define GGL_OPT_RANK_L0_DEFLATE 21
#define GGL_OPT_FUSED_CW 22
#define GGL_OPT_OMEGA_LDS 23
#define GGL_OPT_EARLY_PART 24
#define GGL_OPT_FUSED_W 26
#define GGL_OPT_RANK_CW 27
#define GGL_OPT_BOUND_SIDE 28
#define GGL_OPT_LDS_PINNED 29
#define GGL_OPT_JOIN_FLAG 30
#define GGL_OPT_CW_RIDER 31
#define GGL_OPT_COPY_RIDER 32
#define GGL_OPT_REDUCE_RIDER 33
#define GGL_OPT_PARTS_BIAS 34
#define GGL_OPT_PARTS_ORDER 35
#define GGL_OPT_DOWNLOAD_THREADS 36
#define GGL_OPT_GROUP_SCHED 37
#define GGL_OPT_PART_PRIORITY 25
#define GGL_OPT_ISOLATE 19
#define GGL_OPT_RANK_L0_COARSE 18
int ggl_ctx_set_option(ggl_ctx *ctx, int option, double value);
int ggl_ctx_get_option(ggl_ctx *ctx, int option, double *value);

int ggl_set_S(ggl_ctx *ctx, const double *S_host);
int ggl_set_state(ggl_ctx *ctx, const double *Omega, const double *Theta, const double *L,
                  const double *X);
int ggl_set_S_ex(ggl_ctx *ctx, const double *S_host, int period);
int ggl_set_state_ex(ggl_ctx *ctx, const double *Omega, const double *Theta, const double *L, const double *X,
                     const int *periods);
int ggl_get_state(ggl_ctx *ctx, double *Omega, double *Theta, double *L, double *X);
int ggl_state_snapshot(ggl_ctx *ctx, int restore);
int ggl_set_lambda1_mask(ggl_ctx *ctx, const double *lam_pp_host);

int ggl_admm_step(ggl_ctx *ctx, double rho, double lambda1, double lambda2, int reg, int latent,
                  const double *mu1, const double *nk, double out_norms[5]);
int ggl_hint_last_step(ggl_ctx *ctx);

int ggl_step_omega(ggl_ctx *ctx, double rho, int latent, const double *nk);
int ggl_step_group_partial(ggl_ctx *ctx, double rho, double lambda1);
int ggl_step_omega_spec(ggl_ctx *ctx, double rho, int latent, const double *nk);
int ggl_step_finish(ggl_ctx *ctx, double rho, double lambda1, double lambda2, int reg, int latent,
                    const double *mu1, int groupsq_ready, double out_norms[5]);
int ggl_norms_read(ggl_ctx *ctx, double out_norms[5]);

int ggl_comm_unique_id(char id_out[128]);
int ggl_comm_init(ggl_ctx *ctx, int rank, int nranks, const char id[128]);
int ggl_comm_destroy(ggl_ctx *ctx);
int ggl_comm_count(ggl_ctx *ctx, int *nranks_out);
int ggl_allreduce_groupsq(ggl_ctx *ctx);
int ggl_allreduce_norms(ggl_ctx *ctx);
// ... 51 lines not shown
int ggl_selection_rank(ggl_ctx *ctx, double rel_tol, double *out);
int ggl_finalize_L(ggl_ctx *ctx, int which, int *rank_out);
int ggl_debug_poison(int on);
int ggl_set_odd_dl(int on);
int ggl_failed_instances(ggl_ctx *ctx, int *out);
int ggl_failed_reason(ggl_ctx *ctx, int k, double out[2]);
int ggl_reset_instance(ggl_ctx *ctx, int k);
int ggl_ctx_create_subset(ggl_ctx *src, const int *idx, int m, ggl_ctx **out);
int ggl_get_snapshot_k(ggl_ctx *ctx, int k, double *Theta, double *L);
int ggl_get_snapshot_state_k(ggl_ctx *ctx, int k, double *Omega, double *X);
int ggl_objective(ggl_ctx *ctx, double lambda1, double lambda2, int reg, double out[3]);

int ggl_kkt_residual(ggl_ctx *ctx, double rho, double lambda1, double lambda2, int reg, int latent,
                     const double *mu1, const double *nk, double *out);

#define GGL_PH_FORM_W 0
#define GGL_PH_EIG_OMEGA 1
#define GGL_PH_RECON_OMEGA 2
#define GGL_PH_THETA 3
#define GGL_PH_EIG_L 4
#define GGL_PH_RECON_L 5
#define GGL_PH_DUAL 6
#define GGL_PH_REDUCE 7
#define GGL_PH_EIG_OMEGA2 8
#define GGL_PH_BOUND 9
#define GGL_PH_ALLREDUCE_GROUPSQ 10
#define GGL_PH_ALLREDUCE_NORMS 11
#define GGL_NPHASE 12
int ggl_profile_enable(ggl_ctx *ctx, int on);
int ggl_profile_read(ggl_ctx *ctx, double ms[GGL_NPHASE], long long count[GGL_NPHASE], int reset);
int ggl_ns_stats(ggl_ctx *ctx, long long out[16]);
int ggl_lds_stats(ggl_ctx *ctx, long long out[4]);
int ggl_group_stats(ggl_ctx *ctx, long long out[11], double *units_sum);
int ggl_spectral_bounds(ggl_ctx *ctx, double *c_out, double *beta_out);
int ggl_pipeline_stats(ggl_ctx *ctx, long long out[10]);
int ggl_rank_stats(ggl_ctx *ctx, long long out[4]);
int ggl_deflate_stats(ggl_ctx *ctx, long long out[2]);
int ggl_finalize_stats(ggl_ctx *ctx, long long out[2]);
int ggl_last_dispatch(ggl_ctx *ctx, long long out[4]);
int ggl_trace_start(ggl_ctx *ctx, int max_events);
int ggl_trace_read(ggl_ctx *ctx, double *out, int cap);
int ggl_eig_info(ggl_ctx *ctx, int *out);

int ggl_dev_symm(int K, int p, const double *A, const double *B, const double *E, const double *coef5K,
                 double *C, double *C2, int variant);
int ggl_dev_symm_bench(int K, int p, int variant, int iters, double *ms_out);
int ggl_dev_omega_lds(int K, int p, const double *Theta, const double *L, const double *X, const double *S, const double *beta,
                      double tol, int degrees, double *Omega, double *cbound, int iters, double *out);
int ggl_dev_symm_bounds(int K, int p, const double *A, const double *B, int variant, double *C,
                        double *rowsum_out, double *fro2_out, double *bound_out);
int ggl_dev_ns_schedule(double l, int degrees, int max_steps, int *deg_out, double *coef_out, int *units_out);
int ggl_dev_ns_schedule_tol(double l, int degrees, double tol, int max_steps, int *deg_out, double *coef_out,
                            int *units_out);
int ggl_dev_group_partition(const int *units, int K, int p, int max_groups, int *len_out);
int ggl_dev_ns_units(double l, int degrees, double tol);
#ifdef GGL_DEV
int ggl_dev_i8_stages(int n);
int ggl_dev_symm_i8(int K, int p, int S, int dmax, const double *A, const double *B, double scaleA, double scaleB, double *C,
                    int iters, double *ms_out);
int ggl_dev_omega_i8(int K, int p, const double *W, const double *beta, const double *cbound, const int *cfg5, double tol,
                     double *Omega, int iters, double *ms_out);
int ggl_dev_mfma_f64_peak(double *tflops_out);
int ggl_dev_coissue_probe(double *out12);
int ggl_dev_mfma_lds_probe(double *out6);
int ggl_dev_chain_run(int K, int p, int nprod, int iters, double *out);
int ggl_dev_switch_bench(int K, int p, int variant, int iters, int mode, double *ms_out);
int ggl_dev_vendor_bench(int K, int p, int mode, int iters, double *ms_out);
int ggl_dev_fill_copy_probe(int reps, int K, int p, int slices, int gap_us, long long out[2]);
int ggl_dev_symm_timeline(int K, int p, long long *out, int max_blocks, int *nblocks_out);
int ggl_dev_chain_probe(int K, int p, int variant, int nprod, int iters, int two_level, double *out);
#endif

int ggl_eigh_batched(int K, int p, const double *A, double *D, double *Q, int eig_method);
int ggl_phiplus(int K, int p, const double *beta, const double *D, const double *Q, double *out);
int ggl_prox_rank_norm(int K, int p, const double *beta, const double *D, const double *Q, double *out);
int ggl_phiplus_matrix(int K, int p, const double *beta, const double *W, double *out, int eig_method);
int ggl_rank_matrix(int K, int p, const double *beta, const double *C, double *out, int eig_method);
int ggl_rank_matrix_ex(int K, int p, const double *beta, const double *C, double *out, int eig_method, double l0_coarse,
                       long long stats[6]);
int ggl_rank_matrix_deflate(int K, int p, const double *beta, const double *C, double *out, int eig_method, double l0_deflate,
                            long long stats[8]);
int ggl_prox_od_1norm(int p, const double *A, double lam, const double *lam_pp, double *out);
int ggl_prox_p(int K, int p, const double *X, double l1, double l2, int reg, double *out);
int ggl_prox_tv(int n, int K, const double *Y, double lam, double *out);
int ggl_prox_2norm(int n, int K, const double *Y, double lam, double *out);
int ggl_prox_phi(int n, int K, const double *Y, double l1, double l2, int reg, double *out);

#ifdef __cplusplus
// ... 4 lines not shown
```

Baseline: 1443.

## Add direct polynomial Omega-step replacing Newton-Schulz iteration chain

Adds an 'omega_poly' mode, on by default, in which the Omega-step matrix function is evaluated by a single precomputed polynomial in W. The polynomial is applied through a Horner-like chain of fused symmetric GEMMs, instead of a multi-step Newton-Schulz schedule. The symmetric GEMM kernel gains a second epilogue addend (E2) and two extra coefficients per instance, so each product can fold in another matrix term. The aim is fewer GEMM launches per ADMM iteration, at the cost of extra epilogue memory reads and a possible accuracy risk if the polynomial fit is poor for some spectra.

```diff
diff --git a/gglasso_amd/_lib.py b/gglasso_amd/_lib.py
--- a/gglasso_amd/_lib.py
+++ b/gglasso_amd/_lib.py
@@ -11,7 +11,7 @@
 EIG_AUTO, EIG_JACOBI, EIG_ROCSOLVER, EIG_NEWTON_SCHULZ = 0, 1, 2, 3
 CTX_STREAM_GIVEN = 1 << 16
 OPTIONS = {"speculate": 1, "spec_factor": 2, "ns_mode": 3, "ns_degrees": 4, "theta_flat": 5, "rank_eig": 6, "parts": 7,
-           "parts_max_tiles": 8, "symm_variant": 9, "spin_wait": 10, "fused_bounds": 11, "pipeline": 12, "fused_start": 13, "parts_small": 14, "ns_tol": 15, "cw_warm": 16, "chain": 17, "rank_l0_coarse": 18, "isolate": 19, "rank_deflate": 20, "rank_l0_deflate": 21, "fused_cw": 22, "omega_lds": 23, "early_part": 24, "part_priority": 25, "fused_w": 26, "rank_cw": 27, "bound_side": 28, "lds_pinned": 29, "join_flag": 30, "cw_rider": 31, "copy_rider": 32, "reduce_rider": 33, "parts_bias": 34, "parts_order": 35, "download_threads": 36, "group_sched": 37}
+           "parts_max_tiles": 8, "symm_variant": 9, "spin_wait": 10, "fused_bounds": 11, "pipeline": 12, "fused_start": 13, "parts_small": 14, "ns_tol": 15, "cw_warm": 16, "chain": 17, "rank_l0_coarse": 18, "isolate": 19, "rank_deflate": 20, "rank_l0_deflate": 21, "fused_cw": 22, "omega_lds": 23, "early_part": 24, "part_priority": 25, "fused_w": 26, "rank_cw": 27, "bound_side": 28, "lds_pinned": 29, "join_flag": 30, "cw_rider": 31, "copy_rider": 32, "reduce_rider": 33, "parts_bias": 34, "parts_order": 35, "download_threads": 36, "group_sched": 37, "omega_poly": 38}
 
 
 def eig_flags(method=EIG_AUTO, ns_mode=0, ns_degrees=0):
@@ -118,6 +118,8 @@
     "ggl_dev_ns_schedule_tol": ([_d, _i, _d, _i, ctypes.POINTER(_i), _dp, ctypes.POINTER(_i)], _i),
     "ggl_dev_group_partition": ([ctypes.POINTER(_i), _i, _i, _i, ctypes.POINTER(_i)], _i),
     "ggl_dev_ns_units": ([_d, _i, _d], _i),
+    "ggl_dev_omega_poly_plan": ([_d, _d, _i, ctypes.POINTER(_i), _dp, ctypes.POINTER(_i)], _i),
+    "ggl_omega_poly_stats": ([_vp, ctypes.POINTER(ctypes.c_longlong)], _i),
     "ggl_ns_stats": ([_vp, ctypes.POINTER(ctypes.c_longlong)], _i),
     "ggl_rank_stats": ([_vp, ctypes.POINTER(ctypes.c_longlong)], _i),
     "ggl_deflate_stats": ([_vp, ctypes.POINTER(ctypes.c_longlong)], _i),
diff --git a/gglasso_amd/csrc/capi_batch.hip b/gglasso_amd/csrc/capi_batch.hip
--- a/gglasso_amd/csrc/capi_batch.hip
+++ b/gglasso_amd/csrc/capi_batch.hip
@@ -499,7 +499,7 @@
     c->symm_variant = src->symm_variant; c->spin_wait = src->spin_wait; c->fused_bounds = src->fused_bounds;
     c->pipeline = src->pipeline; c->fused_start = src->fused_start; c->parts_small = src->parts_small; c->download_threads = src->download_threads; c->ns_tol = src->ns_tol;
     c->cw_warm = src->cw_warm; c->rank_l0 = src->rank_l0; c->rank_l0_coarse = src->rank_l0_coarse;
-    c->group_sched = src->group_sched;
+    c->group_sched = src->group_sched; c->omega_poly = src->omega_poly;
     c->isolate = src->isolate; c->lds_omega = src->lds_omega; c->lds_waves = src->lds_waves; c->early_part = src->early_part; c->rank_deflate = src->rank_deflate; c->rank_l0_deflate = src->rank_l0_deflate;
     int* didx = nullptr;
     hipError_t e = hipMalloc(&didx, m * sizeof(int));
diff --git a/gglasso_amd/csrc/capi_ctx.hip b/gglasso_amd/csrc/capi_ctx.hip
--- a/gglasso_amd/csrc/capi_ctx.hip
+++ b/gglasso_amd/csrc/capi_ctx.hip
@@ -350,6 +350,10 @@
                 return fail(GGL_E_ARG, "bad argument: GGL_OPT_GROUP_SCHED is 0, 1, 2, 3, 12 or 13");
             c->group_sched = (int)v;
             break;
+        case GGL_OPT_OMEGA_POLY:
+            if (v != 0.0 && v != 1.0) return fail(GGL_E_ARG, "bad argument: GGL_OPT_OMEGA_POLY is 0 or 1");
+            c->omega_poly = (int)v;
+            break;
 #ifdef GGL_DEV
         case GGL_OPT_PARTS_BIAS: c->parts_bias = (int)v; break;
         case GGL_OPT_PARTS_ORDER: c->parts_order = (int)v; break;
@@ -441,6 +445,7 @@
         case GGL_OPT_FUSED_START: *value = c->fused_start; break;
         case GGL_OPT_PARTS_SMALL: *value = c->parts_small; break;
         case GGL_OPT_GROUP_SCHED: *value = c->group_sched; break;
+        case GGL_OPT_OMEGA_POLY: *value = c->omega_poly; break;
         case GGL_OPT_PARTS_BIAS: *value = c->parts_bias; break;
         case GGL_OPT_PARTS_ORDER: *value = c->parts_order; break;
         case GGL_OPT_DOWNLOAD_THREADS: *value = c->download_threads; break;
diff --git a/gglasso_amd/csrc/capi_internal.hpp b/gglasso_amd/csrc/capi_internal.hpp
--- a/gglasso_amd/csrc/capi_internal.hpp
+++ b/gglasso_amd/csrc/capi_internal.hpp
@@ -130,6 +130,9 @@
     long long group_changes = 0;
     int last_groups = 1, last_group_len[MAX_PARTS] = {}, last_group_units[MAX_PARTS] = {};
     double group_units_sum[MAX_PARTS] = {};
+    int omega_poly = 1;
+    long long poly_seqs = 0, poly_seqs_total = 0;
+    int poly_last_deg = 0;
     int parts_small = 8;
     bool fused_start = true;
     bool fused_bounds = true;
diff --git a/gglasso_amd/csrc/capi_omega.hip b/gglasso_amd/csrc/capi_omega.hip
--- a/gglasso_amd/csrc/capi_omega.hip
+++ b/gglasso_amd/csrc/capi_omega.hip
@@ -231,6 +231,12 @@
 }
 void trace_symm_hook(hipStream_t st, int kind, void* arg) { trace_mark((ggl_ctx*)arg, st, 10 + kind); }
 
+static void note_family(ggl_ctx* c, const NsPlan& pl)
+{
+    c->poly_seqs_total += 1;
+    if (pl.direct) { c->poly_seqs += 1; c->poly_last_deg = pl.direct; }
+}
+
 static int omega_groups(const ggl_ctx* c, const double* cb, const double* beta_h, int K, int* Kh, int* k0h, int* gunits)
 {
     if (!c->group_sched || K < 2 || c->ns_force == 2 || c->chain_mode || c->comm) return 1;
@@ -307,8 +313,8 @@
         for (int k = 0; !resume && k < K; ++k) {
             double* o0 = pre + (size_t)k * NS_NCOEF;
             double* o1 = pre + NS_SLOT(K) + (size_t)k * NS_NCOEF;
-            o0[0] = 4.0 * c->par_h[k]; o0[1] = 1.0; o0[2] = o0[3] = o0[4] = o0[5] = 0.0;
-            o1[0] = 0.0; o1[1] = 1.0; o1[2] = o1[3] = o1[4] = o1[5] = 0.0;
+            o0[0] = 4.0 * c->par_h[k]; o0[1] = 1.0; o0[2] = o0[3] = o0[4] = o0[5] = o0[6] = o0[7] = 0.0;
+            o1[0] = 0.0; o1[1] = 1.0; o1[2] = o1[3] = o1[4] = o1[5] = o1[6] = o1[7] = 0.0;
         }
         double* pre_d = c->coef + (size_t)(NS_MAX_LAUNCHES - 2) * NS_SLOT(K);
         const long t64 = (c->p + 63) / 64;
@@ -441,12 +447,12 @@
             SymmOp ops[CHAIN_MAX_OPS];
             int nops = 0;
             const int bT = (c->p + 63) / 64;
-            if (ns_plan(c->cuse_h, c->par_h, K, c->coef_h, start_base_h, &pl, c->ns_force, c->ns_degrees, c->ns_tol) == 0 &&
+            if (ns_plan(c->cuse_h, c->par_h, K, c->coef_h, start_base_h, &pl, c->ns_force, c->ns_degrees, c->ns_tol, c->omega_poly) == 0 &&
                 !pl.stable) {
                 double* f0 = nullptr;
                 for (int k = 0; k < K; ++k)
                     f0 = ns_fused_start(pl, start_base_h + 5 * (size_t)k, c->nsYP[1], c->nsT, (size_t)K * pp,
-                                        pre + NS_SLOT(K) + (size_t)k * NS_NCOEF + 3);
+                                        pre + NS_SLOT(K) + (size_t)k * NS_NCOEF);
                 if (f0)
                     nops = ns_chain_ops(pl, pre_d, pre_d + NS_SLOT(K), c->coef, c->W, c->nsYP[0], c->nsYP[1], c->nsNX, c->nsT,
                                         c->Om[nxt], K, c->p, 0, f0, c->rowpart, c->fropart, ops, CHAIN_MAX_OPS);
@@ -485,6 +491,7 @@
                 c->last_variant = 40;
                 c->chain_calls += 1;
                 c->ns_launches_total += pl.products;
+                note_family(c, pl);
                 c->ns_units_frac += pl.units;
                 c->ns_steps_frac += pl.steps;
                 c->ns_units_total = (long long)(c->ns_units_frac + 0.5);
@@ -509,11 +516,11 @@
             for (int h = 0; spec && h < nh; ++h) {
                 const int k0 = k0h[h];
                 const int prc = ns_plan(c->cuse_h + k0, c->par_h + k0, Kh[h], c->coef_h + h * region,
-                                        start_base_h + 5 * k0, &plans[h], c->ns_force, c->ns_degrees, c->ns_tol);
+                                        start_base_h + 5 * k0, &plans[h], c->ns_force, c->ns_degrees, c->ns_tol, c->omega_poly);
                 spec = (prc == 0) && !plans[h].stable;
                 for (int k = k0; spec && c->fused_start && k < k0 + Kh[h]; ++k) {
                     fused[h] = ns_fused_start(plans[h], start_base_h + 5 * (size_t)k, c->nsYP[1] + k0 * pp, c->nsT + k0 * pp,
-                                              nh > 1 ? c->n : (size_t)K * pp, pre + NS_SLOT(K) + (size_t)k * NS_NCOEF + 3);
+                                              nh > 1 ? c->n : (size_t)K * pp, pre + NS_SLOT(K) + (size_t)k * NS_NCOEF);
                 }
             }
         }
@@ -591,7 +598,7 @@
                 (void)hipEventRecord(c->ev_early[c->ev_early_par][0], c->stream);
             } else if (h == 0 && !want_A) { PE(c, GGL_PH_FORM_W); PB(c, GGL_PH_EIG_OMEGA); }
             ns_prepare(sh, pre_d + NS_NCOEF * (size_t)k0, pre_d + NS_SLOT(K) + NS_NCOEF * (size_t)k0, c->W + k0 * pp, Ap, Bp, Kh[h], c->p,
-                       var_parts, spec ? fused[h] : nullptr, rowp, frop);
+                       var_parts, spec ? fused[h] : nullptr, rowp, frop, plans[h].direct != 0);
             symm_flush_rider(sh);
             if (early_ev) {
                 (void)hipEventRecord(c->ev_early[c->ev_early_par][1], c->stream);
@@ -662,6 +669,7 @@
                        var_parts, nh > 1 ? c->n : 0, fused[h] != nullptr, bfree);
                 symm_flush_rider(sh);
                 c->ns_launches_total += plans[h].products;
+                note_family(c, plans[h]);
                 const double frac = (double)Kh[h] / K;
                 c->ns_units_frac += frac * plans[h].units;
                 c->ns_steps_frac += frac * plans[h].steps;
@@ -728,7 +736,7 @@
         for (int h = 0; h < nh; ++h) {
             const int k0 = k0h[h];
             const int prc = ns_plan(c->bounds_h + k0, c->par_h + k0, Kh[h], c->coef_h + h * region_b, start_base_h + 5 * k0,
-                                    &plans[h], c->ns_force, c->ns_degrees, c->ns_tol);
+                                    &plans[h], c->ns_force, c->ns_degrees, c->ns_tol, c->omega_poly);
             if (prc == -1) return fail(GGL_E_SOLVER, "Newton-Schulz Omega-step: non-finite W (diverged iterate?)");
             if (prc == -2) {
                 c->ns_eigh_fallbacks += 1;
@@ -741,7 +749,8 @@
             any_stable = any_stable || plans[h].stable;
         }
         if (nh > 1 && any_stable) {
-            const int prc = ns_plan(c->bounds_h, c->par_h, K, c->coef_h, start_base_h, &plans[0], c->ns_force, c->ns_degrees, c->ns_tol);
+            const int prc = ns_plan(c->bounds_h, c->par_h, K, c->coef_h, start_base_h, &plans[0], c->ns_force, c->ns_degrees, c->ns_tol,
+                                    c->omega_poly);
             if (prc != 0) return fail(GGL_E_SOLVER, "Newton-Schulz Omega-step: plan failed (%d)", prc);
         }
         const int nrun = (nh > 1 && !any_stable) ? nh : 1;
@@ -767,6 +776,7 @@
                    nrun > 1 ? var_b : c->symm_variant, nrun > 1 ? c->n : 0);
             c->ns_stable_calls += plans[h].stable ? 1 : 0;
             c->ns_launches_total += plans[h].products;
+            note_family(c, plans[h]);
             const double frac = (double)Kr / K;
             c->ns_units_frac += frac * plans[h].units;
             c->ns_steps_frac += frac * plans[h].steps;
diff --git a/gglasso_amd/csrc/capi_ops.hip b/gglasso_amd/csrc/capi_ops.hip
--- a/gglasso_amd/csrc/capi_ops.hip
+++ b/gglasso_amd/csrc/capi_ops.hip
@@ -742,6 +742,11 @@
     return ns_group_partition(units, K, p, max_groups, len_out);
 }
 extern "C" int ggl_dev_ns_units(double l, int degrees, double tol) { return ns_units_query(l, degrees, tol); }
+extern "C" int ggl_dev_omega_poly_plan(double a, double tol, int degrees, int* deg, double* out, int* units)
+{
+    ARGCHK(deg && out && units && a > 0.0 && a < 1.0, "deg, out, units, 0 < a < 1");
+    return ns_poly_query(std::sqrt(a), degrees, tol, deg, out, units, out + 16, out + 17);
+}
 
 extern "C" int ggl_dev_ns_schedule_tol(double l, int degrees, double tol, int max_steps, int* deg_out, double* coef_out,
                                        int* units_out)
diff --git a/gglasso_amd/csrc/capi_stats.hip b/gglasso_amd/csrc/capi_stats.hip
--- a/gglasso_amd/csrc/capi_stats.hip
+++ b/gglasso_amd/csrc/capi_stats.hip
@@ -48,6 +48,15 @@
     return GGL_OK;
 }
 
+extern "C" int ggl_omega_poly_stats(ggl_ctx* c, long long out[3])
+{
+    ARGCHK(c && out, "ctx, out");
+    out[0] = c->poly_seqs;
+    out[1] = c->poly_seqs_total;
+    out[2] = c->poly_last_deg;
+    return GGL_OK;
+}
+
 extern "C" int ggl_group_stats(ggl_ctx* c, long long out[11], double* units_sum)
 {
     ARGCHK(c && out, "ctx, out");
diff --git a/gglasso_amd/csrc/gemm_sym.hip b/gglasso_amd/csrc/gemm_sym.hip
--- a/gglasso_amd/csrc/gemm_sym.hip
+++ b/gglasso_amd/csrc/gemm_sym.hip
@@ -12,6 +12,11 @@
 typedef double v4d __attribute__((ext_vector_type(4)));
 
 __device__ __forceinline__ double c2val(double dC, double v, double dE, double e) { return __builtin_fma(dE, e, dC * v); }
+__device__ __forceinline__ double c2val2(double dC, double v, double dE, double e, bool has2, double dE2, double f)
+{
+    const double w = c2val(dC, v, dE, e);
+    return has2 ? __builtin_fma(dE2, f, w) : w;
+}
 
 template <int BM, int BK, int WM, int WN, bool LM>
 struct SymCfg {
@@ -77,7 +82,8 @@
 __global__ __launch_bounds__(sym_nt(BM, WM, WN)) void k_symm_tn(
     const double* __restrict__ A, const double* __restrict__ B, double* __restrict__ C, double* __restrict__ C2,
     const double* __restrict__ E, const double* __restrict__ coef, int K, int p, const double* __restrict__ A1,
-    const double* __restrict__ B1, double* __restrict__ C1, int K1, double* __restrict__ maxdev)
+    const double* __restrict__ B1, double* __restrict__ C1, int K1, double* __restrict__ maxdev,
+    const double* __restrict__ E2)
 {
     using Cfg = SymCfg<BM, BK, WM, WN, LM>;
     __shared__ __attribute__((aligned(16))) double smem[Cfg::LDS_DOUBLES];
@@ -187,6 +193,8 @@
     double* Ck = (second ? C1 : C) + (size_t)kk * pp;
     double* C2k = (C2 && !second) ? C2 + (size_t)kk * pp : nullptr;
     const double* Ek = (E && !second) ? E + (size_t)kk * pp : nullptr;
+    const double* E2k = (E2 && !second) ? E2 + (size_t)kk * pp : nullptr;
+    const double cE2 = E2k ? coef[k * NS_NCOEF + 6] : 0.0, dE2 = E2k ? coef[k * NS_NCOEF + 7] : 0.0;
 #pragma unroll
     for (int ti = 0; ti < Cfg::TI; ++ti)
 #pragma unroll
@@ -202,11 +210,13 @@
                     if (gi == gj) v += cI;
                     const double e0 = Ek ? Ek[(size_t)gi * p + gj] : 0.0;
                     v += cE * e0;
+                    const double f0 = E2k ? E2k[(size_t)gi * p + gj] : 0.0;
+                    if (E2k) v += cE2 * f0;
                     Ck[(size_t)gi * p + gj] = v;
-                    if (C2k) C2k[(size_t)gi * p + gj] = c2val(dC, v, dE, e0) + (gi == gj ? dI : 0.0);
+                    if (C2k) C2k[(size_t)gi * p + gj] = c2val2(dC, v, dE, e0, E2k != nullptr, dE2, f0) + (gi == gj ? dI : 0.0);
                     if ((I == J && gi != gj) || (!LM && I != J)) {
                         Ck[(size_t)gj * p + gi] = v;
-                        if (C2k) C2k[(size_t)gj * p + gi] = c2val(dC, v, dE, e0);
+                        if (C2k) C2k[(size_t)gj * p + gi] = c2val2(dC, v, dE, e0, E2k != nullptr, dE2, f0);
                     }
                 }
                 if (LM && I != J) smem[row * Cfg::CLD + col] = v;
@@ -224,6 +234,7 @@
                     if (gi < p && gj < p && (I != J || gi <= gj)) {
                         double v = cAcc * acc[ti][tj][r] + (gi == gj ? cI - 1.0 : 0.0);
                         if (Ek) v += cE * Ek[(size_t)gi * p + gj];
+                        if (E2k) v += cE2 * E2k[(size_t)gi * p + gj];
                         dev = fmax(dev, fabs(v));
                     }
                 }
@@ -240,7 +251,8 @@
                 Ck[(size_t)(J0 + a) * p + I0 + c] = v;
                 if (C2k) {
                     const double e0 = (dE != 0.0 && Ek) ? Ek[(size_t)(J0 + a) * p + I0 + c] : 0.0;
-                    C2k[(size_t)(J0 + a) * p + I0 + c] = c2val(dC, v, dE, e0);
+                    const double f0 = E2k ? E2k[(size_t)(J0 + a) * p + I0 + c] : 0.0;
+                    C2k[(size_t)(J0 + a) * p + I0 + c] = c2val2(dC, v, dE, e0, E2k != nullptr, dE2, f0);
                 }
             }
         }
@@ -259,12 +271,12 @@
 template <int BM, int BK, int WM, int WN, bool LM>
 static void launch_cfg(hipStream_t st, const double* A, const double* B, double* C, double* C2, const double* E,
                        const double* coef, int K, int p, const double* A1 = nullptr, const double* B1 = nullptr,
-                       double* C1 = nullptr, int K1 = 0, double* maxdev = nullptr)
+                       double* C1 = nullptr, int K1 = 0, double* maxdev = nullptr, const double* E2 = nullptr)
 {
     using Cfg = SymCfg<BM, BK, WM, WN, LM>;
     const int T = (p + BM - 1) / BM;
     hipLaunchKernelGGL((k_symm_tn<BM, BK, WM, WN, LM>), dim3(xcd_grid(T * (T + 1) / 2, K + K1)), dim3(Cfg::NT), 0, st, A,
-                       B, C, C2, E, coef, K, p, A1, B1, C1, K1, maxdev);
+                       B, C, C2, E, coef, K, p, A1, B1, C1, K1, maxdev, E2);
 }
 
 typedef __attribute__((address_space(1))) const void* gptr_t;
@@ -293,7 +305,8 @@
 template <int BK, int NSTG, int ABL, int BM, int NW, int AUX = 0>
 __device__ __forceinline__ void symm_dl_tile(const double* __restrict__ A, const double* __restrict__ B,
                                              double* __restrict__ C, double* __restrict__ C2,
-                                             const double* __restrict__ E, const double* __restrict__ coef, int K,
+                                             const double* __restrict__ E, const double* __restrict__ E2,
+                                             const double* __restrict__ coef, int K,
                                              int p, const double* __restrict__ A1, const double* __restrict__ B1,
                                              double* __restrict__ C1, int K1, double* __restrict__ maxdev,
                                              double* __restrict__ rowpart, double* __restrict__ fropart, int k, int b,
@@ -480,6 +493,8 @@
     double* Ck = (second ? C1 : C) + (size_t)kk * pp;
     double* C2k = (C2 && !second) ? C2 + (size_t)kk * pp : nullptr;
     const double* Ek = (E && !second) ? E + (size_t)kk * pp : nullptr;
+    const double* E2k = (E2 && !second) ? E2 + (size_t)kk * pp : nullptr;
+    const double cE2 = E2k ? coef[k * NS_NCOEF + 6] : 0.0, dE2 = E2k ? coef[k * NS_NCOEF + 7] : 0.0;
     double dev = 0.0;
     const bool wide = (I != J) && ABL != 1;
     if (wide) {
@@ -505,17 +520,20 @@
             double2 t = ld2(smem + row * BM + ((c2 ^ row) & ~1));
             if (row & 1) { const double h = t.x; t.x = t.y; t.y = h; }
             if (gi < p && gj + 1 < p) {
-                double2 e = {0.0, 0.0};
+                double2 e = {0.0, 0.0}, f = {0.0, 0.0};
                 if (Ek) e = lde2(Ek + (size_t)gi * p + gj);
+                if (E2k) f = lde2(E2k + (size_t)gi * p + gj);
                 double2 v;
                 v.x = t.x + cE * e.x;
                 v.y = t.y + cE * e.y;
+                if (E2k) { v.x += cE2 * f.x; v.y += cE2 * f.y; }
                 dev = fmax(dev, fmax(fabs(v.x), fabs(v.y)));
                 *reinterpret_cast<double2*>(Ck + (size_t)gi * p + gj) = v;
                 if (C2k) {
                     double2 w;
                     w.x = c2val(dC, v.x, dE, e.x);
                     w.y = c2val(dC, v.y, dE, e.y);
+                    if (E2k) { w.x = __builtin_fma(dE2, f.x, w.x); w.y = __builtin_fma(dE2, f.y, w.y); }
                     *reinterpret_cast<double2*>(C2k + (size_t)gi * p + gj) = w;
                 }
                 if (rowpart) {
@@ -524,10 +542,12 @@
                 }
             } else if (gi < p && gj < p) {
                 const double e0 = Ek ? ld_pol<AUX>(Ek + (size_t)gi * p + gj) : 0.0;
-                const double v0 = t.x + cE * e0;
+                const double f0 = E2k ? ld_pol<AUX>(E2k + (size_t)gi * p + gj) : 0.0;
+                double v0 = t.x + cE * e0;
+                if (E2k) v0 += cE2 * f0;
                 dev = fmax(dev, fabs(v0));
                 Ck[(size_t)gi * p + gj] = v0;
-                if (C2k) C2k[(size_t)gi * p + gj] = c2val(dC, v0, dE, e0);
+                if (C2k) C2k[(size_t)gi * p + gj] = c2val2(dC, v0, dE, e0, E2k != nullptr, dE2, f0);
                 if (rowpart) {
                     double2 v = {v0, 0.0};
                     if (row & 1) { v.x = 0.0; v.y = v0; }
@@ -561,12 +581,14 @@
                     if (gi == gj) v += cI;
                     const double e0 = Ek ? ld_pol<AUX>(Ek + (size_t)gi * p + gj) : 0.0;
                     v += cE * e0;
+                    const double f0 = E2k ? ld_pol<AUX>(E2k + (size_t)gi * p + gj) : 0.0;
+                    if (E2k) v += cE2 * f0;
                     dev = fmax(dev, fabs(v - (gi == gj ? 1.0 : 0.0)));
                     Ck[(size_t)gi * p + gj] = v;
-                    if (C2k) C2k[(size_t)gi * p + gj] = c2val(dC, v, dE, e0) + (gi == gj ? dI : 0.0);
+                    if (C2k) C2k[(size_t)gi * p + gj] = c2val2(dC, v, dE, e0, E2k != nullptr, dE2, f0) + (gi == gj ? dI : 0.0);
                     if (I == J && gi != gj) {
                         Ck[(size_t)gj * p + gi] = v;
-                        if (C2k) C2k[(size_t)gj * p + gi] = c2val(dC, v, dE, e0);
+                        if (C2k) C2k[(size_t)gj * p + gi] = c2val2(dC, v, dE, e0, E2k != nullptr, dE2, f0);
                     }
                 }
                 if ((I != J || rowpart) && ABL != 1) smem[row * BM + (col ^ row)] = (rowpart && !keep) ? 0.0 : v;
@@ -625,24 +647,32 @@
                 double2 v;
                 v.x = smem[c2 * BM + (a ^ c2)];
                 v.y = smem[(c2 + 1) * BM + (a ^ (c2 + 1))];
-                double2 e = {0.0, 0.0};
+                double2 e = {0.0, 0.0}, f = {0.0, 0.0};
                 const bool need_e = Ek && (!rowpart || (C2k && dE != 0.0));
                 if (need_e) e = lde2(Ek + (size_t)(J0 + a) * p + I0 + c2);
-                if (!rowpart) { v.x += cE * e.x; v.y += cE * e.y; }
+                const bool need_f = E2k && (!rowpart || (C2k && dE2 != 0.0));
+                if (need_f) f = lde2(E2k + (size_t)(J0 + a) * p + I0 + c2);
+                if (!rowpart) {
+                    v.x += cE * e.x; v.y += cE * e.y;
+                    if (E2k) { v.x += cE2 * f.x; v.y += cE2 * f.y; }
+                }
                 *reinterpret_cast<double2*>(Ck + (size_t)(J0 + a) * p + I0 + c2) = v;
                 if (C2k) {
                     double2 w;
                     w.x = c2val(dC, v.x, dE, e.x);
                     w.y = c2val(dC, v.y, dE, e.y);
+                    if (E2k) { w.x = __builtin_fma(dE2, f.x, w.x); w.y = __builtin_fma(dE2, f.y, w.y); }
                     *reinterpret_cast<double2*>(C2k + (size_t)(J0 + a) * p + I0 + c2) = w;
                 }
             } else if (J0 + a < p && I0 + c2 < p) {
                 double v0 = smem[c2 * BM + (a ^ c2)];
                 const bool need_e = Ek && (!rowpart || (C2k && dE != 0.0));
                 const double e0 = need_e ? ld_pol<AUX>(Ek + (size_t)(J0 + a) * p + I0 + c2) : 0.0;
-                if (!rowpart) v0 += cE * e0;
+                const bool need_f = E2k && (!rowpart || (C2k && dE2 != 0.0));
+                const double f0 = need_f ? ld_pol<AUX>(E2k + (size_t)(J0 + a) * p + I0 + c2) : 0.0;
+                if (!rowpart) { v0 += cE * e0; if (E2k) v0 += cE2 * f0; }
                 Ck[(size_t)(J0 + a) * p + I0 + c2] = v0;
-                if (C2k) C2k[(size_t)(J0 + a) * p + I0 + c2] = c2val(dC, v0, dE, e0);
+                if (C2k) C2k[(size_t)(J0 + a) * p + I0 + c2] = c2val2(dC, v0, dE, e0, E2k != nullptr, dE2, f0);
             }
         }
     }
@@ -788,7 +818,8 @@
 template <int BK, int NSTG, int ABL = 0, int BM = 64, int NW = 4>
 __global__ __launch_bounds__(NW * 64) void k_symm_dl(const double* __restrict__ A, const double* __restrict__ B,
                                                  double* __restrict__ C, double* __restrict__ C2,
-                                                 const double* __restrict__ E, const double* __restrict__ coef, int K,
+                                                 const double* __restrict__ E, const double* __restrict__ E2,
+                                                 const double* __restrict__ coef, int K,
                                                  int p, const double* __restrict__ A1, const double* __restrict__ B1,
                                                  double* __restrict__ C1, int K1, double* __restrict__ maxdev,
                                                  double* __restrict__ rowpart, double* __restrict__ fropart, const CwRider rider,
@@ -832,7 +863,7 @@
     }
     int k, b;
     if (!decode_block_xcd(T * (T + 1) / 2, K + K1, k, b, bid)) return;
-    symm_dl_tile<BK, NSTG, ABL, BM, NW>(A, B, C, C2, E, coef, K, p, A1, B1, C1, K1, maxdev, rowpart, fropart, k, b, smem);
+    symm_dl_tile<BK, NSTG, ABL, BM, NW>(A, B, C, C2, E, E2, coef, K, p, A1, B1, C1, K1, maxdev, rowpart, fropart, k, b, smem);
 }
 
 #ifdef GGL_DEV
@@ -1191,7 +1222,7 @@
         const SymmOp& o = P.op[js];
         int kk = jk;
         if (o.pair && jb >= P.ntiles) { kk = P.K + jk; jb -= P.ntiles; }
-        symm_dl_tile<BK, NSTG, 0, BM, 4, AUX>(o.A, o.B, o.C, o.C2, o.E, o.coef, P.K, P.p, o.A1, o.B1, o.C1, o.pair ? P.K : 0,
+        symm_dl_tile<BK, NSTG, 0, BM, 4, AUX>(o.A, o.B, o.C, o.C2, o.E, o.E2, o.coef, P.K, P.p, o.A1, o.B1, o.C1, o.pair ? P.K : 0,
                                                nullptr, o.rowpart, o.fropart, kk, jb, smem);
         asm volatile("s_waitcnt vmcnt(0)" ::: "memory");
         __syncthreads();
@@ -1298,7 +1329,7 @@
         for (int L = blockIdx.x; L < total; L += gridDim.x) {
             int k, b;
             if (decode_block_xcd(ntiles, K, k, b, L))
-                symm_dl_tile<BK, NSTG, 0, BM, 4>(src, src, dst, nullptr, nullptr, coef, K, p, nullptr, nullptr, nullptr, 0,
+                symm_dl_tile<BK, NSTG, 0, BM, 4>(src, src, dst, nullptr, nullptr, nullptr, coef, K, p, nullptr, nullptr, nullptr, 0,
                                                  nullptr, nullptr, nullptr, k, b, smem);
             __syncthreads();
         }
@@ -1359,7 +1390,8 @@
 
 static void launch_dl(hipStream_t st, const double* A, const double* B, double* C, double* C2, const double* E,
                       const double* coef, int K, int p, const double* A1, const double* B1, double* C1, int K1,
-                      double* maxdev, int dl_cfg = 0, double* rowpart = nullptr, double* fropart = nullptr)
+                      double* maxdev, int dl_cfg = 0, double* rowpart = nullptr, double* fropart = nullptr,
+                      const double* E2 = nullptr)
 {
     const bool eight = dl_cfg == 6 || dl_cfg == 7;
     const CwRider rider = (g_rider.K > 0 && !eight) ? g_rider : CwRider{};
@@ -1371,7 +1403,7 @@
     int ncopy = red.nblk > 0 ? NXCD : 0;
     for (int i = 0; i < cps.n; ++i) ncopy += (int)((cps.words[i] + 1023u) / 1024u);
     const int nride = rider.K * rider.nbx + ncopy;
-#define GGL_DL(...) hipLaunchKernelGGL((k_symm_dl<__VA_ARGS__>), grid, dim3(256), 0, st, A, B, C, C2, E, coef, K, p, A1, B1, C1, K1, maxdev, rowpart, fropart, rider, cps, red)
+#define GGL_DL(...) hipLaunchKernelGGL((k_symm_dl<__VA_ARGS__>), grid, dim3(256), 0, st, A, B, C, C2, E, E2, coef, K, p, A1, B1, C1, K1, maxdev, rowpart, fropart, rider, cps, red)
     if (dl_cfg == 4 || (dl_cfg >= 8 && dl_cfg <= 13) || (dl_cfg >= 18 && dl_cfg <= 21)) {
         const int T32 = (p + 31) / 32;
         const dim3 grid(xcd_grid(T32 * (T32 + 1) / 2, K + K1) + nride);
@@ -1394,7 +1426,7 @@
     const dim3 grid(xcd_grid(T * (T + 1) / 2, K + K1) + nride);
 #ifdef GGL_DEV
     if (dl_cfg == 6 || dl_cfg == 7) {
-#define GGL_DL8(...) hipLaunchKernelGGL((k_symm_dl<__VA_ARGS__>), grid, dim3(512), 0, st, A, B, C, C2, E, coef, K, p, A1, B1, C1, K1, maxdev, rowpart, fropart, rider, cps, red)
+#define GGL_DL8(...) hipLaunchKernelGGL((k_symm_dl<__VA_ARGS__>), grid, dim3(512), 0, st, A, B, C, C2, E, E2, coef, K, p, A1, B1, C1, K1, maxdev, rowpart, fropart, rider, cps, red)
         if (dl_cfg == 6) GGL_DL8(16, 4, 0, 64, 8);
         else GGL_DL8(32, 3, 0, 64, 8);
 #undef GGL_DL8
@@ -1755,13 +1787,15 @@
 }
 
 void launch_symm(hipStream_t st, const double* A, const double* B, double* C, double* C2, const double* E,
-                 const double* coef, int K, int p, int variant, double* maxdev, double* rowpart, double* fropart)
+                 const double* coef, int K, int p, int variant, double* maxdev, double* rowpart, double* fropart,
+                 const double* E2)
 {
     SymmHookAtExit hook{st, 0};
     if (variant < 0) variant = symm_auto_variant(K, p);
 #define GGL_TN(BM, BK, WM, WN, LM) \
-    launch_cfg<BM, BK, WM, WN, LM>(st, A, B, C, C2, E, coef, K, p, nullptr, nullptr, nullptr, 0, maxdev)
-#ifdef GGL_DEV
+    launch_cfg<BM, BK, WM, WN, LM>(st, A, B, C, C2, E, coef, K, p, nullptr, nullptr, nullptr, 0, maxdev, E2)
+#ifdef GGL_DEV
+    if (E2 && variant >= 41 && variant <= 50) variant = 20;
     if (variant >= 41 && variant <= 50) {
         if ((p & 1) == 0 && p >= 2) { launch_sk(st, A, B, C, C2, E, coef, K, p, maxdev, rowpart, fropart, variant); return; }
         variant = 9;
@@ -1770,7 +1804,7 @@
     switch (variant) {
         case 16: case 17: case 18: case 19: case 20: case 21: case 22: case 23: case 24: case 25: case 26: case 27: case 28: case 29: case 30: case 31: case 32: case 33: case 34: case 35: case 36: case 37: case 38: case 39:
             if (symm_dl_serves(p)) {
-                launch_dl(st, A, B, C, C2, E, coef, K, p, nullptr, nullptr, nullptr, 0, maxdev, variant - 16, rowpart, fropart);
+                launch_dl(st, A, B, C, C2, E, coef, K, p, nullptr, nullptr, nullptr, 0, maxdev, variant - 16, rowpart, fropart, E2);
                 break;
             }
             if (variant == 20 || variant >= 24) GGL_TN(32, 32, 16, 16, true);
@@ -1791,7 +1825,7 @@
             const int T = (p + 63) / 64;
             const dim3 grid(xcd_grid(T * (T + 1) / 2, K));
             double* md = (variant == 10) ? maxdev : nullptr;
-#define GGL_ABL(N) hipLaunchKernelGGL((k_symm_tn<64, 16, 32, 32, true, N>), grid, dim3(256), 0, st, A, B, C, C2, E, coef, K, p, nullptr, nullptr, nullptr, 0, md)
+#define GGL_ABL(N) hipLaunchKernelGGL((k_symm_tn<64, 16, 32, 32, true, N>), grid, dim3(256), 0, st, A, B, C, C2, E, coef, K, p, nullptr, nullptr, nullptr, 0, md, E2)
             if (variant == 6) GGL_ABL(1); else if (variant == 7) GGL_ABL(2); else if (variant == 10) GGL_ABL(3);
             else if (variant == 14) GGL_ABL(4); else GGL_ABL(5);
 #undef GGL_ABL
diff --git a/gglasso_amd/csrc/kernels.hpp b/gglasso_amd/csrc/kernels.hpp
--- a/gglasso_amd/csrc/kernels.hpp
+++ b/gglasso_amd/csrc/kernels.hpp
@@ -178,7 +178,7 @@
 void launch_recon(hipStream_t st, double* out, const double* R, const double* D, const double* betaK,
                   int map, int K, int p, double* scale_work);
 
-static constexpr int NS_NCOEF = 6;
+static constexpr int NS_NCOEF = 8;
 int symm_variants();
 bool symm_variant_built(int v);
 bool symm_dl_serves(int p);
@@ -187,12 +187,12 @@
 int symm_auto_variant(int nprod, int p);
 void launch_symm(hipStream_t st, const double* A, const double* B, double* C, double* C2, const double* E,
                  const double* coef, int K, int p, int variant, double* maxdev = nullptr, double* rowpart = nullptr,
-                 double* fropart = nullptr);
+                 double* fropart = nullptr, const double* E2 = nullptr);
 int symm_bounds_tile(int K, int p, int variant);
 void symm_release_workspace(hipStream_t st);
 
 struct SymmOp {
-    const double *A, *B, *E, *A1, *B1;
+    const double *A, *B, *E, *A1, *B1, *E2;
     double *C, *C2, *C1;
     const double* coef;
     double *rowpart, *fropart;
@@ -266,7 +266,7 @@
 static constexpr double NS_SYM_KAPPA_MAX = 300.0;
 static constexpr double NS_KAPPA_LIMIT = 1e12;
 struct NsPlan {
-    int steps = 0; int products = 0; bool stable = false; double kappa = 0.0; int units = 0;
+    int steps = 0; int products = 0; bool stable = false; double kappa = 0.0; int units = 0; int direct = 0;
     double check = 5e-5;
     unsigned char deg[NS_RANK_MAX_STEPS] = {};
 };
@@ -274,19 +274,21 @@
 void launch_form_W_sym(hipStream_t st, double* W, const double* Theta, const double* L, const double* X,
                        const double* S, const double* betaK, int K, int p);
 int ns_plan(const double* cbound_h, const double* beta_h, int K, double* coef_h, double* start_h, NsPlan* plan,
-            int force_mode, int degrees = 9, double tol = NS_TOL_EXACT);
+            int force_mode, int degrees = 9, double tol = NS_TOL_EXACT, int poly = 0);
+int ns_poly_query(double l, int degrees, double tol, int* deg, double* coef, int* units, double* a_out, double* err_out);
 int ns_schedule_query(double l, int degrees, int max_steps, int* deg, double* coef, int* units, double tol = NS_TOL_EXACT);
 int ns_units_query(double l, int degrees, double tol);
 int ns_group_partition(const int* units, int K, int p, int max_groups, int* len_out);
 void ns_prepare(hipStream_t st, const double* pre0_d, const double* pre1_d, const double* W, double* Ap, double* Bp,
-                int K, int p, int variant, double* start2 = nullptr, double* rowpart = nullptr, double* fropart = nullptr);
+                int K, int p, int variant, double* start2 = nullptr, double* rowpart = nullptr, double* fropart = nullptr,
+                bool start_w = false);
 void ns_run(hipStream_t st, const NsPlan& plan, const double* coef_d, const double* start_d, const double* W,
             double* AB, double* YP, double* Tb, double* out, int K, int p, int variant, size_t pstride = 0,
             bool fused_start = false, hipEvent_t bprime_free = nullptr);
 int ns_chain_ops(const NsPlan& plan, const double* pre0_d, const double* pre1_d, const double* coef_d, const double* W,
                  double* AB, double* YP, double* NX, double* Tb, double* out, int K, int p, size_t pstride, double* start2,
                  double* rowpart, double* fropart, SymmOp* ops, int max_ops);
-double* ns_fused_start(const NsPlan& plan, const double* start_hk, double* YP, double* Tb, size_t n1, double out3[3]);
+double* ns_fused_start(const NsPlan& plan, const double* start_hk, double* YP, double* Tb, size_t n1, double* row);
 
 int norm_bounds_blocks(int p);
 void launch_norm_bounds(hipStream_t st, const double* W, int K, int p, double* part, double* rowsum = nullptr);
diff --git a/gglasso_amd/csrc/newton_schulz.hip b/gglasso_amd/csrc/newton_schulz.hip
--- a/gglasso_amd/csrc/newton_schulz.hip
+++ b/gglasso_amd/csrc/newton_schulz.hip
@@ -350,6 +350,149 @@
     return pl.plan(l);
 }
 
+static constexpr double NS_POLY_EVAL = 2e-14;
+static constexpr int NS_POLY_MAXDEG = 15;
+
+static double ns_poly_fit(double a, int d, double* mono)
+{
+    constexpr int G = 1024, NM = NS_POLY_MAXDEG + 2;
+    const double m = 0.5 * (1.0 + a), h = 0.5 * (1.0 - a);
+    static thread_local double gx[G + 1], gf[G + 1], gt[G + 1][NS_POLY_MAXDEG + 1], err[G + 1];
+    for (int i = 0; i <= G; ++i) {
+        const double x = -std::cos(M_PI * i / G);
+        gx[i] = x;
+        gf[i] = std::sqrt(m + h * x);
+        gt[i][0] = 1.0;
+        gt[i][1] = x;
+        for (int j = 2; j <= d; ++j) gt[i][j] = 2.0 * x * gt[i][j - 1] - gt[i][j - 2];
+    }
+    const int n = d + 2;
+    int ref[NM];
+    for (int r = 0; r < n; ++r) ref[r] = (int)std::lround((double)G * r / (n - 1));
+    double co[NM] = {}, best[NM] = {}, ebest = 1e300;
+    for (int iter = 0; iter < 24; ++iter) {
+        double A[NM][NM + 1];
+        for (int r = 0; r < n; ++r) {
+            const int i = ref[r];
+            for (int j = 0; j <= d; ++j) A[r][j] = gt[i][j];
+            A[r][d + 1] = ((r & 1) ? -1.0 : 1.0) * gf[i];
+            A[r][n] = gf[i];
+        }
+        for (int i = 0; i < n; ++i) {
+            int pv = i;
+            for (int r = i + 1; r < n; ++r) if (std::fabs(A[r][i]) > std::fabs(A[pv][i])) pv = r;
+            for (int cc = 0; cc <= n; ++cc) std::swap(A[i][cc], A[pv][cc]);
+            for (int r = 0; r < n; ++r) {
+                if (r == i) continue;
+                const double f = A[r][i] / A[i][i];
+                for (int cc = i; cc <= n; ++cc) A[r][cc] -= f * A[i][cc];
+            }
+        }
+        for (int i = 0; i < n; ++i) co[i] = A[i][n] / A[i][i];
+        double emax = 0.0;
+        for (int i = 0; i <= G; ++i) {
+            double v = 0.0;
+            for (int j = 0; j <= d; ++j) v += co[j] * gt[i][j];
+            err[i] = (v - gf[i]) / gf[i];
+            emax = std::fmax(emax, std::fabs(err[i]));
+        }
+        const bool settled = emax > 0.999 * ebest;
+        if (emax < ebest) { ebest = emax; for (int j = 0; j <= d; ++j) best[j] = co[j]; }
+        if (settled) break;
+        int alt[G + 2], na = 0;
+        for (int i = 0; i <= G; ++i) {
+            const bool ext = (i == 0 || i == G) || ((err[i] - err[i - 1]) * (err[i + 1] - err[i]) <= 0.0);
+            if (!ext) continue;
+            if (na > 0 && (err[i] > 0.0) == (err[alt[na - 1]] > 0.0)) {
+                if (std::fabs(err[i]) > std::fabs(err[alt[na - 1]])) alt[na - 1] = i;
+            } else {
+                alt[na++] = i;
+            }
+        }
+        int lo = 0;
+        while (na - lo > n) {
+            if (std::fabs(err[alt[lo]]) < std::fabs(err[alt[na - 1]])) ++lo; else --na;
+        }
+        if (na - lo < n) break;
+        bool same = true;
+        for (int r = 0; r < n; ++r) { same = same && (ref[r] == alt[lo + r]); ref[r] = alt[lo + r]; }
+        if (same) break;
+    }
+    for (int j = 0; j <= d; ++j) co[j] = best[j];
+    double tp[NM] = {}, tc[NM] = {}, tn[NM];
+    for (int j = 0; j <= d; ++j) mono[j] = 0.0;
+    tp[0] = 1.0;
+    tc[1] = 1.0;
+    mono[0] += co[0];
+    if (d >= 1) mono[1] += co[1];
+    for (int j = 2; j <= d; ++j) {
+        for (int i = 0; i <= j; ++i) tn[i] = (i > 0 ? 2.0 * tc[i - 1] : 0.0) - tp[i];
+        for (int i = 0; i <= j; ++i) { mono[i] += co[j] * tn[i]; tp[i] = tc[i]; tc[i] = tn[i]; }
+    }
+    double E = 0.0;
+    for (int i = 0; i <= G; ++i) {
+        long double v = 0.0L;
+        for (int j = d; j >= 0; --j) v = v * (long double)gx[i] + (long double)mono[j];
+        const long double f = std::sqrt((long double)(m + h * gx[i]));
+        E = std::fmax(E, (double)std::fabs((v - f) / f));
+    }
+    return E * (1.0 + 1e-2);
+}
+
+struct NsPoly { int deg = 0; int units = 1 << 30; double a = 0.0; double err = 0.0; double co[NS_POLY_MAXDEG + 1] = {}; };
+
+static NsPoly ns_poly_plan(double l, double tol, int dmax = NS_POLY_MAXDEG)
+{
+    struct Fit { double err; double co[NS_POLY_MAXDEG + 1]; };
+    static thread_local std::unordered_map<long long, Fit> memo;
+    const double t = std::fmin(std::fmax(tol, NS_TOL_EXACT), 1e-6);
+    const NsKey q = ns_quantise(l);
+    NsPoly r;
+    r.a = q.l * q.l;
+    if (!(r.a > 0.0 && r.a < 1.0) || t <= 2.0 * NS_POLY_EVAL) return r;
+    if (memo.size() > 4096) memo.clear();
+    for (int d = 6; d <= std::min(dmax, NS_POLY_MAXDEG); d += 3) {
+        const long long id = (long long)q.key * 32 + d;
+        auto it = memo.find(id);
+        if (it == memo.end()) {
+            Fit f;
+            f.err = ns_poly_fit(r.a, d, f.co);
+            it = memo.emplace(id, f).first;
+        }
+        if (it->second.err + NS_POLY_EVAL <= t) {
+            r.deg = d;
+            r.units = 2 + d / 3;
+            r.err = it->second.err;
+            for (int j = 0; j <= d; ++j) r.co[j] = it->second.co[j];
+            break;
+        }
+    }
+    return r;
+}
+
+static int ns_poly_choice(double l, int degrees, double tol)
+{
+    if (!(l > 0.0) || !(l < 1.0) || 1.0 / (l * l) > NS_SYM_KAPPA_MAX) return 0;
+    const NsSeq& sq = ns_mixed_schedule(l, degrees, tol);
+    const int ns_units = (sq.n < 1 || sq.cost >= (1 << 29)) ? (1 << 30) : 2 + sq.cost;
+    const int dmax = ns_units > NS_POLY_MAXDEG / 3 + 2 ? NS_POLY_MAXDEG : 3 * (ns_units - 3);
+    const NsPoly pp = ns_poly_plan(l, tol, dmax);
+    return (pp.deg && pp.units < ns_units) ? pp.deg : 0;
+}
+
+int ns_poly_query(double l, int degrees, double tol, int* deg, double* coef, int* units, double* a_out, double* err_out)
+{
+    if (!(l > 0.0) || !(l <= 1.0)) return -1;
+    const NsPoly pp = ns_poly_plan(l, tol);
+    const int chosen = ns_poly_choice(l, degrees, tol);
+    *deg = pp.deg;
+    for (int j = 0; j <= NS_POLY_MAXDEG; ++j) coef[j] = j <= pp.deg ? pp.co[j] : 0.0;
+    *units = pp.deg ? pp.units : -1;
+    if (a_out) *a_out = pp.a;
+    if (err_out) *err_out = pp.err;
+    return chosen ? 1 : 0;
+}
+
 int ns_schedule_query(double l, int degrees, int max_steps, int* deg, double* coef, int* units, double tol)
 {
     if (!(l > 0.0) || !(l <= 1.0)) return -1;
@@ -433,6 +576,10 @@
                 Y1[base + i] = __builtin_fma(y1a, a, y1b * b2) + (r == c ? z1i : 0.0);
                 continue;
             }
+            if (mode == 4) {
+                Y1[base + i] = __builtin_fma(0.5, W[base + i], __builtin_fma(y1a, a, y1b * b2)) + (r == c ? z1i : 0.0);
+                continue;
+            }
             const double y = y1a * a + y1b * b2;
             if (mode == 1) {
                 Y1[base + i] = 0.5 * W[base + i] + h * y;
@@ -452,7 +599,7 @@
 }
 
 int ns_plan(const double* cbound_h, const double* beta_h, int K, double* coef_h, double* start_h, NsPlan* plan,
-            int force_mode, int degrees, double tol)
+            int force_mode, int degrees, double tol, int poly)
 {
     std::vector<double> c(K);
     double kappa = 1.0;
@@ -467,10 +614,46 @@
     const double lmin = 1.0 / std::sqrt(kappa);
     plan->stable = stable;
     plan->kappa = kappa;
-    auto put = [&](int g, int k, double cI, double cAcc, double cE, double dI = 0.0, double dC = 0.0, double dE = 0.0) {
+    plan->direct = 0;
+    auto put = [&](int g, int k, double cI, double cAcc, double cE, double dI = 0.0, double dC = 0.0, double dE = 0.0,
+                   double cE2 = 0.0, double dE2 = 0.0) {
         double* o = coef_h + (size_t)g * NS_SLOT(K) + (size_t)k * NS_NCOEF;
-        o[0] = cI; o[1] = cAcc; o[2] = cE; o[3] = dI; o[4] = dC; o[5] = dE;
+        o[0] = cI; o[1] = cAcc; o[2] = cE; o[3] = dI; o[4] = dC; o[5] = dE; o[6] = cE2; o[7] = dE2;
     };
+    const int pd = (!stable && poly) ? ns_poly_choice(lmin, degrees, tol) : 0;
+    if (pd) {
+        const NsPoly pp = ns_poly_plan(lmin, tol, pd);
+        const int J = pd / 3;
+        const double a = pp.a, m = 0.5 * (1.0 + a), h = 0.5 * (1.0 - a), u = 1.0 / (h * h * h);
+        plan->direct = pd;
+        plan->steps = 1;
+        plan->deg[0] = 0;
+        plan->units = pp.units;
+        plan->products = J + 2;
+        for (int k = 0; k < K; ++k) {
+            const double ck = c[k], hc = 0.5 * std::sqrt(ck);
+            auto digit = [&](int j, double* o3) {
+                const double a0 = pp.co[3 * j], a1 = pp.co[3 * j + 1], a2 = pp.co[3 * j + 2];
+                o3[0] = a0 - a1 * (m / h) + a2 * (m / h) * (m / h);
+                o3[1] = a1 / (ck * h) - 2.0 * a2 * m / (ck * h * h);
+                o3[2] = a2 / (ck * ck * h * h);
+            };
+            double dg[3];
+            digit(0, dg);
+            double* s = start_h + (size_t)k * 5;
+            s[0] = hc * dg[1]; s[1] = hc * dg[2]; s[2] = hc * dg[0]; s[3] = 0.0; s[4] = 0.0;
+            int g = 0;
+            digit(J - 1, dg);
+            put(g++, k, -m * m * m * u, u / (ck * ck * ck), -3.0 * m * u / (ck * ck), dg[0], pp.co[3 * J], dg[2],
+                3.0 * m * m * u / ck, dg[1]);
+            for (int j = J - 2; j >= 1; --j) {
+                digit(j, dg);
+                put(g++, k, dg[0], 1.0, dg[2], 0.0, 0.0, 0.0, dg[1]);
+            }
+            put(g++, k, 0.0, hc, 1.0);
+        }
+        return 0;
+    }
     if (!stable) {
         const NsSeq& sq = ns_mixed_schedule(lmin, degrees, tol);
         if (sq.n < 1 || sq.n > NS_MAX_STEPS || sq.cost >= (1 << 29)) return -2;
@@ -557,15 +740,22 @@
 }
 
 void ns_prepare(hipStream_t st, const double* pre0_d, const double* pre1_d, const double* W, double* Ap, double* Bp, int K,
-                int p, int variant, double* start2, double* rowpart, double* fropart)
+                int p, int variant, double* start2, double* rowpart, double* fropart, bool start_w)
 {
     launch_symm(st, W, W, Ap, nullptr, nullptr, pre0_d, K, p, variant);
     symm_flush_rider(st);
-    launch_symm(st, Ap, Ap, Bp, start2, start2 ? Ap : nullptr, pre1_d, K, p, variant, nullptr, rowpart, fropart);
-}
-
-double* ns_fused_start(const NsPlan& plan, const double* start_hk, double* YP, double* Tb, size_t n1, double out3[3])
-{
+    launch_symm(st, Ap, Ap, Bp, start2, start2 ? Ap : nullptr, pre1_d, K, p, variant, nullptr, rowpart, fropart,
+                start2 && start_w ? W : nullptr);
+}
+
+double* ns_fused_start(const NsPlan& plan, const double* start_hk, double* YP, double* Tb, size_t n1, double* row)
+{
+    double* out3 = row + 3;
+    row[7] = 0.0;
+    if (plan.direct) {
+        out3[0] = start_hk[2]; out3[1] = start_hk[1]; out3[2] = start_hk[0]; row[7] = 0.5;
+        return Tb;
+    }
     if (plan.stable || plan.deg[0] < 5) return nullptr;
     if (plan.deg[0] == 5) { out3[0] = start_hk[2]; out3[1] = start_hk[1]; out3[2] = start_hk[3]; return YP + n1; }
     out3[0] = start_hk[2]; out3[1] = start_hk[1]; out3[2] = start_hk[0];
@@ -585,6 +775,17 @@
     const size_t cs = NS_SLOT(K), n1 = pstride ? pstride : (size_t)K * p * p;
     const int n = plan.steps;
     int g = 0;
+    if (plan.direct) {
+        if (!fused_start) launch_ns_start(st, Tb, nullptr, AB, AB + n1, W, start_d, K, p, 4);
+        const int J = plan.direct / 3;
+        auto hbuf = [&](int j) { return (j & 1) ? YP + n1 : out; };
+        launch_symm(st, AB, AB + n1, YP, hbuf(J - 1), AB + n1, coef_d + cs * g++, K, p, variant, nullptr, nullptr, nullptr, AB);
+        for (int j = J - 2; j >= 1; --j)
+            launch_symm(st, hbuf(j + 1), YP, hbuf(j), nullptr, AB + n1, coef_d + cs * g++, K, p, variant, nullptr, nullptr,
+                        nullptr, AB);
+        launch_symm(st, hbuf(1), YP, out, nullptr, Tb, coef_d + cs * g++, K, p, variant);
+        return;
+    }
     double *cur = YP, *nxt = AB;
     if (plan.deg[0] >= 5 && !plan.stable) {
         if (plan.deg[0] == 5) {
@@ -638,7 +839,7 @@
                  double* AB, double* YP, double* NX, double* Tb, double* out, int K, int p, size_t pstride, double* start2,
                  double* rowpart, double* fropart, SymmOp* ops, int max_ops)
 {
-    if (plan.stable || plan.deg[0] < 5 || !start2) return 0;
+    if (plan.stable || (plan.deg[0] < 5 && !plan.direct) || !start2) return 0;
     const size_t cs = NS_SLOT(K), n1 = pstride ? pstride : (size_t)K * p * p;
     const int n = plan.steps;
     int no = 0, g = 0;
@@ -653,6 +854,22 @@
     };
     double* Ap = AB;
     double* Bp = AB + n1;
+    if (plan.direct) {
+        const int J = plan.direct / 3;
+        auto hbuf = [&](int j) { return (j & 1) ? YP + n1 : out; };
+        add(W, W, Ap, nullptr, nullptr, pre0_d);
+        SymmOp* o = add(Ap, Ap, Bp, start2, Ap, pre1_d, rowpart, fropart);
+        if (o) o->E2 = W;
+        o = add(Ap, Bp, YP, hbuf(J - 1), Bp, coef_d + cs * g++);
+        if (o) o->E2 = Ap;
+        for (int j = J - 2; j >= 1; --j) {
+            o = add(hbuf(j + 1), YP, hbuf(j), nullptr, Bp, coef_d + cs * g++);
+            if (o) o->E2 = Ap;
+        }
+        add(hbuf(1), YP, out, nullptr, start2, coef_d + cs * g++);
+        (void)NX;
+        return ok ? no : 0;
+    }
     add(W, W, Ap, nullptr, nullptr, pre0_d);
     add(Ap, Ap, Bp, start2, Ap, pre1_d, rowpart, fropart);
     double *cur = YP, *nxt = NX;
diff --git a/gglasso_amd/solver.py b/gglasso_amd/solver.py
--- a/gglasso_amd/solver.py
+++ b/gglasso_amd/solver.py
@@ -413,6 +413,12 @@
                          "rank_fallbacks", "rank_launches", "spec_calls", "spec_misses", "spin_timeouts", "last_parts",
                          "last_variant", "eigh_fallbacks", "pre_dropped"), (int(v) for v in out)))
 
+    def poly_stats(self):
+        import ctypes
+        out = (ctypes.c_longlong * 3)()
+        check(self.lib.ggl_omega_poly_stats(self.h, out))
+        return dict(zip(("seqs", "seqs_total", "last_deg"), (int(v) for v in out)))
+
     def rank_stats(self):
         import ctypes
         out = (ctypes.c_longlong * 4)()
diff --git a/include/ggl_hip.h b/include/ggl_hip.h
--- a/include/ggl_hip.h
+++ b/include/ggl_hip.h
@@ -82,6 +82,7 @@
 #define GGL_OPT_PARTS_ORDER 35
 #define GGL_OPT_DOWNLOAD_THREADS 36
 #define GGL_OPT_GROUP_SCHED 37
+#define GGL_OPT_OMEGA_POLY 38
 #define GGL_OPT_PART_PRIORITY 25
 #define GGL_OPT_ISOLATE 19
 #define GGL_OPT_RANK_L0_COARSE 18
@@ -199,6 +200,7 @@
 int ggl_ns_stats(ggl_ctx *ctx, long long out[16]);
 int ggl_lds_stats(ggl_ctx *ctx, long long out[4]);
 int ggl_group_stats(ggl_ctx *ctx, long long out[11], double *units_sum);
+int ggl_omega_poly_stats(ggl_ctx *ctx, long long out[3]);
 int ggl_spectral_bounds(ggl_ctx *ctx, double *c_out, double *beta_out);
 int ggl_pipeline_stats(ggl_ctx *ctx, long long out[10]);
 int ggl_rank_stats(ggl_ctx *ctx, long long out[4]);
@@ -221,6 +223,7 @@
                             int *units_out);
 int ggl_dev_group_partition(const int *units, int K, int p, int max_groups, int *len_out);
 int ggl_dev_ns_units(double l, int degrees, double tol);
+int ggl_dev_omega_poly_plan(double a, double tol, int degrees, int *deg, double *out, int *units);
 #ifdef GGL_DEV
 int ggl_dev_i8_stages(int n);
 int ggl_dev_symm_i8(int K, int p, int S, int dmax, const double *A, const double *B, double scaleA, double scaleB, double *C,
```

Measured after the change: 1475, median of 6. 1.02x the previous value.
